# daeheepark/TrajSDE

Measured on AMD Instinct MI355X. Metric: scenes/sec (K=6, 20 SDE steps, ~256 agents) at 1/2/4/8 MI355X; minADE match, higher is better.
Workload: dtype f32 (fp16x3 split: 22-bit operands on v_mfma_f32_16x16x32_f16, f32 accumulate)

## Files before the change

trajsde_amd/csrc/aggregator_bwd.hip:

```cpp
#include <string>
#include <unordered_map>

#include "attn_common.hpp"
#include "bwd.hpp"
#include "common.hpp"
#include "dropout.hpp"
#include "kernels.hpp"
#include "layouts.hpp"
#include "tile.hpp"

namespace tsde {

static bool rows_bwd_mm();

template <int HEADS, bool NODE>
__global__ __launch_bounds__(256) void k_gattn_bwd(const float* __restrict__ img, const int32_t* __restrict__ segptr,
                                                   const int32_t* __restrict__ src, const float* __restrict__ rel,
                                                   const float* __restrict__ q, const float* __restrict__ kn,
                                                   const float* __restrict__ vn, const float* __restrict__ agg,
                                                   const float* __restrict__ dagg, const float* __restrict__ stats, int64_t N,
                                                   float* __restrict__ DQ, float* __restrict__ DKN, float* __restrict__ DVN,
                                                   float* __restrict__ RL, float* __restrict__ SS, float* __restrict__ DAGGM,
                                                   float* __restrict__ EA, float* __restrict__ ED, float* __restrict__ UZ,
                                                   const int32_t* __restrict__ asym, DropArg drop) {
// ... 776 lines not shown
      else TS_LAUNCH_TAG("k_edge_attn_rows_bwd<8>", false, (k_edge_rows_bwd_mm<false, true>), gridf, 64 * RMMF_WAVES, rows_mmf_lds_bytes(), st, img, segptr, emb, q, agg, dagg, stats, R, DQ, RL, SS, DAGGM, EA, ED, drop, wpart, wcs);
      rq->jobs.push_back(ReduceJob{wk, nullptr, base, gridf, 1, 64, 0, 0});
      rq->jobs.push_back(ReduceJob{wv, bv, base + gridf, gridf, 1, 64, 0, 0});
      *weights_done = true;
      return TRAJSDE_OK;
    }
    const int grid = int(std::min<int64_t>(256, cdiv(R, RMM_WAVES)));
    if (drop.p > 0.f) TS_LAUNCH_TAG("k_edge_attn_rows_bwd<8>", false, (k_edge_rows_bwd_mm<true, false>), grid, 64 * RMM_WAVES, rows_mm_lds_bytes(), st, img, segptr, emb, q, agg, dagg, stats, R, DQ, RL, SS, DAGGM, EA, ED, drop, nw, nw);
    else TS_LAUNCH_TAG("k_edge_attn_rows_bwd<8>", false, (k_edge_rows_bwd_mm<false, false>), grid, 64 * RMM_WAVES, rows_mm_lds_bytes(), st, img, segptr, emb, q, agg, dagg, stats, R, DQ, RL, SS, DAGGM, EA, ED, drop, nw, nw);
  } else
    TS_LAUNCH_TAG("k_edge_attn_rows_bwd<8>", false, (k_gattn_bwd<8, false>), xcd_grid(cdiv(R, 4)), 256, 0, st, img, segptr, ns, emb, q, nf, nf, agg, dagg, stats,
                  R, DQ, nw, nw, RL, SS, DAGGM, EA, ED, nw, ns, drop);
  return TRAJSDE_OK;
}

__global__ void k_reverse_edges(const int32_t* __restrict__ segptr, const int32_t* __restrict__ src, const int32_t* __restrict__ dst,
                                int64_t E, int32_t* __restrict__ REV, int32_t* __restrict__ asym) {
  const int64_t e = int64_t(blockIdx.x) * blockDim.x + threadIdx.x;
  if (e >= E) return;
  const int i = src[e], jn = dst[e];
  const int r0 = segptr[i], r1 = segptr[i + 1];
  int lo = r0, hi = r1;
  while (lo < hi) {
    const int mid = (lo + hi) >> 1;
    if (src[mid] < jn) lo = mid + 1;
    else hi = mid;
  }
  int found = lo < r1 && src[lo] == jn ? lo : -1;
  if (found < 0)
    for (int r = r0; r < r1; ++r)
      if (src[r] == jn) { found = r; break; }
  REV[e] = found;
  if (found < 0) atomicOr(asym, 1);
}

template <int HEADS>
__global__ __launch_bounds__(256) void k_gattn_src_bwd(const int32_t* __restrict__ segptr, const int32_t* __restrict__ src,
                                                       const int32_t* __restrict__ REV, const float* __restrict__ EA,
                                                       const float* __restrict__ ED, const float* __restrict__ q,
                                                       const float* __restrict__ dagg, int64_t N, float* __restrict__ DKN,
                                                       float* __restrict__ DVN, const int32_t* __restrict__ asym) {
  const int lane = threadIdx.x & 63, h = lane / (64 / HEADS);
  const int64_t node = xcd_block() * 4 + __builtin_amdgcn_readfirstlane(threadIdx.x >> 6);
  if (node >= N || *asym != 0) return;
  float dk = 0.f, dv = 0.f;
  const int beg = segptr[node], end = segptr[node + 1];
  auto idx_at = [&](int e0, int& rv, int& sv) {
    const int ec = e0 + (lane & 15) < end ? e0 + (lane & 15) : end - 1;
    rv = REV[ec];
    sv = src[ec];
  };
  int rv_n = 0, sv_n = 0;
  if (beg < end) idx_at(beg, rv_n, sv_n);
  for (int e0 = beg; e0 < end; e0 += 16) {
    const int rv = rv_n, sv = sv_n;
    idx_at(e0 + 16 < end ? e0 + 16 : e0, rv_n, sv_n);
    float a[16], d[16], qv[16], gv[16];
#pragma unroll
    for (int u = 0; u < 16; ++u) {
      const int e = __builtin_amdgcn_readlane(rv, u), i = __builtin_amdgcn_readlane(sv, u);
      a[u] = (EA + int64_t(e) * HEADS)[h];
      d[u] = (ED + int64_t(e) * HEADS)[h];
      qv[u] = (q + int64_t(i) * 64)[lane];
      gv[u] = (dagg + int64_t(i) * 64)[lane];
    }
#pragma unroll
    for (int u = 0; u < 16; ++u)
      if (e0 + u < end) {
        dk = fmaf(d[u], qv[u], dk);
        dv = fmaf(a[u], gv[u], dv);
      }
  }
  DKN[node * 64 + lane] = dk;
  DVN[node * 64 + lane] = dv;
}

struct AggBwdWs {
  float *rel, *xn[8], *q[8], *kn[8], *vn[8], *agg[8], *x1[8], *xn2[8], *out[8];
  float* stats[8];
  float *dcur, *dnext, *dagg, *dxn, *DQ, *DKN, *DVN, *DREL, *RL, *SS, *DAGGM, *XF, *part, *cs, *varena;
  float *EA[8], *ED[8], *UZ[8];
  int32_t *REV, *asym;
  NodeBlockScratch nb;
  EdgeEmbedScratch ee;
  int64_t total, parts;
  bool ok;
  AggBwdWs(int64_t N, int64_t E, int nl, int K, void* ws, int64_t bytes) {
    Carver c(ws, bytes);
    rel = c.take<float>(E * 64 + 64);
    for (int l = 0; l < nl; ++l) {
      xn[l] = c.take<float>(N * 64); q[l] = c.take<float>(N * 64); kn[l] = c.take<float>(N * 64); vn[l] = c.take<float>(N * 64);
      agg[l] = c.take<float>(N * 64); x1[l] = c.take<float>(N * 64); xn2[l] = c.take<float>(N * 64); out[l] = c.take<float>(N * 64);
      stats[l] = c.take<float>(N * 16);
    }
    float** singles[] = {&dcur, &dnext, &dagg, &dxn, &DQ, &DKN, &DVN, &DAGGM, &XF, &nb.dx1, &nb.UPD, &nb.DGP, &nb.DS};
    for (float** p : singles) *p = c.take<float>(N * 64);
    nb.H = c.take<float>(N * 256);
    nb.DH = c.take<float>(N * 256);
    RL = c.take<float>(N * 512);
    SS = c.take<float>(N * 512);
    DREL = c.take<float>(E * 64 + 64);
    for (int l = 0; l < nl; ++l) {
      EA[l] = c.take<float>(E * 8 + 64);
      ED[l] = c.take<float>(E * 8 + 64);
      UZ[l] = c.take<float>(N * 1024);
    }
    REV = c.take<int32_t>(E + 1);
    asym = c.take<int32_t>(4);
    float** edge[] = {&ee.DEP, &ee.DSP};
    for (float** p : edge) *p = c.take<float>(E * 64 + 64);
    ee.S = rel;
    nb.vpart = ee.vpart = c.take<float>(VPART_FLOATS);
    varena = c.take<float>(VPART_ARENA_SLABS * VPART_FLOATS);
    const int64_t rows = E > N ? E : N;
    parts = wgrad_max_parts(rows, 1);
    part = c.take<float>(parts * 4096);
    cs = c.take<float>(parts * 64);
    (void)K;
    total = c.off + 256;
    ok = c.ok;
  }
};

}

using namespace tsde;

template <typename DropOf>
static int aggregator_tape(const trajsde_batch* b, const trajsde_graph* g, const float* blob_fwd, int nl, int num_heads,
                           const float* local_embed, AggBwdWs& w, DropOf drop_of, hipStream_t st) {
  const int64_t N = b->N, E = g->E_g, ntiles = (N + 15) / 16, etiles = (E + 15) / 16;
#if TSDE_SPLIT_H3
  if (E > 0 && rel_embed_fused())
    TS_LAUNCH_TAG("k_edge_embed<true>", false, k_edge_embed2, tile_grid((E + 31) / 32, 1024, edge_embed2_lds(1024)), 1024, edge_embed2_lds(1024), st,
                  blob_fwd + AggBlob::REL6G, g->g_geom, EdgeCount{E, nullptr, 0}, w.rel, 0);
  else
#endif
  if (E > 0)
    TS_LAUNCH(k_edge_embed<true>, tile_grid(etiles, 1024, EdgeL6::EMB_SIZE * 4), 1024, EdgeL6::EMB_SIZE * 4, st, blob_fwd + AggBlob::REL6,
              g->g_geom, EdgeCount{E, nullptr, 0}, w.rel, 0);
  const float* x = local_embed;
  for (int l = 0; l < nl; ++l) {
    const float* lb = blob_fwd + AggBlob::layer(l);
    TS_LAUNCH(k_node_proj<3>, tile_grid(ntiles, 512, NodeProjL<3>::SIZE * 4), 512, NodeProjL<3>::SIZE * 4, st, lb + AggLayerL::QKV, x, N,
              w.xn[l], w.q[l], w.kn[l], w.vn[l]);
    {
      const DropArg dl = drop_of(l);
      TS_REQUIRE(N < (1 << 23), "aggregator_forward_train: node rows are addressed with 32-bit byte offsets (N < 2^23)");
      if (num_heads == 8 && gattn_f32mm_enabled() && g->E_g > 0) {
        if (int rc = launch_global_attn_mf(lb + AggLayerL::ATTN, g->g_segptr, g->g_src, w.rel, w.q[l], w.kn[l], w.vn[l], N, w.agg[l], w.stats[l], dl, st)) return rc;
      } else
        TS_GLOBAL_ATTN(num_heads, false, dl, xcd_grid(cdiv(N, 4)), 256, 0, st, lb + AggLayerL::ATTN, g->g_segptr, g->g_src, w.rel, w.q[l], w.kn[l], w.vn[l], N, w.agg[l], w.stats[l]);
    }
    TS_LAUNCH(k_node_update<true>, tile_grid(ntiles, 512, UpdL6::SIZE * 4), 512, UpdL6::SIZE * 4, st, lb + AggLayerL::UPD6, w.agg[l], w.xn[l], x,
              N, w.x1[l], w.xn2[l], drop_of(l), no_merge());
    TS_LAUNCH(k_ffn6, tile_grid(ntiles, 512, FfnL6::HALF * 4), 512, FfnL6::HALF * 4, st, lb + AggLayerL::FFN6, w.x1[l], w.xn2[l], N, w.out[l],
              drop_of(l));
    x = w.out[l];
  }

  return TRAJSDE_OK;
}

extern "C" {

int64_t trajsde_aggregator_backward_ws_bytes(const trajsde_batch* b, const trajsde_graph* g, int num_layers, int num_modes) {
  if (!b || !g || num_layers < 0 || num_layers > 8) return -1;
  AggBwdWs w(b->N, g->E_g, num_layers, num_modes, nullptr, 0);
  return w.total;
}

int trajsde_aggregator_backward(const trajsde_batch* b, const trajsde_graph* g, const float* blob_fwd, const float* blob_bwd,
                                int num_layers, int num_modes, const float* local_embed, const float* d_global, void* ws,
                                int64_t ws_bytes, float* const* grads, int n_grads, float* d_local, void* stream_) {
  return trajsde_aggregator_backward_heads(b, g, blob_fwd, blob_bwd, num_layers, num_modes, 8, local_embed, d_global, ws, ws_bytes, grads,
                                           n_grads, d_local, nullptr, 0, stream_);
}

int trajsde_aggregator_forward_train(const trajsde_batch* b, const trajsde_graph* g, const float* blob_fwd, int num_layers, int num_modes,
                                     int num_heads, const float* local_embed, void* ws, int64_t ws_bytes, float* global_embed,
                                     const trajsde_dropout* dropout, void* stream_) {
  if (int rc = refuse_retired_switches()) return rc;
  TS_REQUIRE(b && g && blob_fwd && local_embed && ws && global_embed, "aggregator_forward_train: null pointer");
  TS_REQUIRE(num_heads == 8 || num_heads == 4, "aggregator_forward_train: num_heads must be 8 or 4");
  TS_REQUIRE(g->g_src && g->g_segptr, "aggregator_forward_train: graph not compacted (call trajsde_graph_compact)");
  TS_REQUIRE(g->exact, "aggregator_forward_train: needs exact list lengths (trajsde_graph_prepare, not _async)");
  TS_REQUIRE(num_layers >= 1 && num_layers <= 8 && num_modes > 0, "aggregator_forward_train: bad layer/mode count");
  TS_REQUIRE(!dropout || (dropout->p >= 0.f && dropout->p < 1.f), "aggregator_forward_train: dropout p must be in [0, 1)");
  TS_REQUIRE(!state_bf16(), "aggregator_forward_train: the training tape is fp32; switch trajsde_state_storage(0)");
  auto drop_of = [&](int layer) { return dropout ? make_drop(dropout->p, dropout->seed, 2 + layer) : no_drop(); };
  AggBwdWs w(b->N, g->E_g, num_layers, num_modes, ws, ws_bytes);
  if (!w.ok) return fail(TRAJSDE_ERR_WORKSPACE, "aggregator_forward_train: workspace too small (trajsde_aggregator_backward_ws_bytes)");
  hipStream_t st = static_cast<hipStream_t>(stream_);
  if (int rc = aggregator_tape(b, g, blob_fwd, num_layers, num_heads, local_embed, w, drop_of, st)) return rc;
  const int64_t N = b->N, ntiles = (N + 15) / 16;
  const int lds = (128 + MAT64 + 64) * 4;
  dim3 grid(tile_grid(ntiles, 512, lds), num_modes);
  TS_LAUNCH(k_mode_proj, grid, 512, lds, st, blob_fwd + AggBlob::norm(num_layers), blob_fwd + AggBlob::proj(num_layers, 0), w.out[num_layers - 1], N,
            global_embed);
  return TRAJSDE_OK;
}

int trajsde_aggregator_backward_heads(const trajsde_batch* b, const trajsde_graph* g, const float* blob_fwd, const float* blob_bwd,
                                      int num_layers, int num_modes, int num_heads, const float* local_embed, const float* d_global,
                                      void* ws, int64_t ws_bytes, float* const* grads, int n_grads, float* d_local,
                                      const trajsde_dropout* dropout, int tape_valid, void* stream_) {
  if (int rc = refuse_retired_switches()) return rc;
  TS_REQUIRE(b && g && blob_fwd && blob_bwd && local_embed && d_global && ws && grads && d_local, "aggregator_backward: null pointer");
  TS_REQUIRE(!state_bf16(), "aggregator_backward: the backward pass keeps its tape in fp32; switch trajsde_state_storage(0) for training");
  TS_REQUIRE(!dropout || (dropout->p >= 0.f && dropout->p < 1.f), "aggregator_backward: dropout p must be in [0, 1)");
  auto drop_of = [&](int layer) { return dropout ? make_drop(dropout->p, dropout->seed, 2 + layer) : no_drop(); };
  TS_REQUIRE(num_heads == 8 || num_heads == 4, "aggregator_backward: num_heads must be 8 or 4");
  TS_REQUIRE(g->g_src && g->g_segptr, "aggregator_backward: graph not compacted (call trajsde_graph_compact)");
  TS_REQUIRE(g->exact, "aggregator_backward: needs exact list lengths (trajsde_graph_prepare, not _async)");
  TS_REQUIRE(num_layers >= 1 && num_layers <= 8 && num_modes > 0, "aggregator_backward: bad layer/mode count");
  const std::vector<std::string> names = stage_param_names(TRAJSDE_STAGE_AGGREGATOR_BWD, num_layers, num_modes);
  TS_REQUIRE(n_grads == int(names.size()), "aggregator_backward: gradient count does not match trajsde_param_count(AGGREGATOR_BWD)");
  std::unordered_map<std::string, float*> slot;
  for (int i = 0; i < n_grads; ++i) {
    TS_REQUIRE(grads[i] != nullptr, "aggregator_backward: null gradient buffer " + names[i]);
    slot[names[i]] = grads[i];
  }
  bool missing = false;
  auto G = [&](const std::string& n) -> float* {
    auto it = slot.find(n);
    if (it == slot.end()) { missing = true; return nullptr; }
    return it->second;
  };
  AggBwdWs w(b->N, g->E_g, num_layers, num_modes, ws, ws_bytes);
  if (!w.ok) return fail(TRAJSDE_ERR_WORKSPACE, "aggregator_backward: workspace too small");
  hipStream_t st = static_cast<hipStream_t>(stream_);
  const int64_t N = b->N, E = g->E_g, ntiles = (N + 15) / 16, etiles = (E + 15) / 16;
  const int nl = num_layers, K = num_modes;
  const WgradCtx wc{st, w.part, w.cs, nullptr, w.parts};
  DeferredSums sums(st, w.part, w.cs, w.parts, nullptr, w.varena, VPART_ARENA_SLABS * VPART_FLOATS);

  if (!tape_valid)
    if (int rc = aggregator_tape(b, g, blob_fwd, nl, num_heads, local_embed, w, drop_of, st)) return rc;
  (void)etiles;

  if (K > 0)
    TS_LAUNCH(k_lin_t_sum, unsigned(ntiles > 0 ? (ntiles + 3) / 4 : 1), 256, 2 * MAT64 * 4, st, blob_bwd + AggBwdBlob::proj(nl, 0),
              int64_t(AggBwdBlob::proj(nl, 1) - AggBwdBlob::proj(nl, 0)), d_global, N * 64, K, N, w.dxn);
  {
    const int gp = vec_grid(ntiles, 256, ProjBwdL<0>::SIZE * 4);
    float* const vp = vpart_slab(w.nb.vpart, int64_t(gp) * 4, 128);
    TS_LAUNCH(k_node_proj_bwd<0>, gp, 256, ProjBwdL<0>::SIZE * 4, st, blob_bwd + AggBwdBlob::norm(nl), w.out[nl - 1], nullptr, w.dxn,
              nullptr, nullptr, nullptr, N, w.dcur, w.XF, vp);
    {
      ColsumBatch cb(st, gp * 4, 128);
      cb.add(vp, 64, G("norm.weight"));
      cb.add(vp + 64, 64, G("norm.bias"));
      if (int rc = cb.flush()) return rc;
    }
    float* pw = G("multihead_proj.weight");
    float* pb = G("multihead_proj.bias");
    TS_REQUIRE(!missing, "aggregator_backward: parameter table lacks norm / multihead_proj");
    WgradBatch wb(wc, N, N);
    for (int k = 0; k < K; ++k)
      if (int rc = wb.add(d_global + int64_t(k) * N * 64, 64, w.XF, 64, pw + int64_t(k) * MAT64, 64, 0, pb + 64 * k, 0)) return rc;
    if (int rc = wb.flush()) return rc;
  }

  TS_HIP(hipMemsetAsync(w.asym, 0, sizeof(int32_t), st));
  if (E > 0) TS_LAUNCH(k_reverse_edges, cdiv(E, 256), 256, 0, st, g->g_segptr, g->g_src, g->g_dst, E, w.REV, w.asym);
  float* dcur = w.dcur;
  float* dnext = w.dnext;
  for (int l = nl - 1; l >= 0; --l) {
    const std::string p = "global_interactor_layers." + std::to_string(l);
    const float* lb = blob_bwd + AggBwdBlob::layer(l);
    const float* x_in = l == 0 ? local_embed : w.out[l - 1];
    NodeBlockGrads gr{G(p + ".lin_ih.weight"), G(p + ".lin_ih.bias"), G(p + ".lin_hh.weight"), G(p + ".lin_hh.bias"),
                      G(p + ".lin_self.weight"), G(p + ".lin_self.bias"), G(p + ".out_proj.weight"), G(p + ".out_proj.bias"),
                      G(p + ".norm2.weight"), G(p + ".norm2.bias"), G(p + ".mlp.0.weight"), G(p + ".mlp.0.bias"),
                      G(p + ".mlp.3.weight"), G(p + ".mlp.3.bias")};
    float* wke = G(p + ".lin_k_edge.weight");
    float* bke = G(p + ".lin_k_edge.bias");
    float* wve = G(p + ".lin_v_edge.weight");
    float* bve = G(p + ".lin_v_edge.bias");
    float* n1g = G(p + ".norm1.weight");
    float* n1b = G(p + ".norm1.bias");
    float* qkv_w[3] = {G(p + ".lin_q_node.weight"), G(p + ".lin_k_node.weight"), G(p + ".lin_v_node.weight")};
    float* qkv_b[3] = {G(p + ".lin_q_node.bias"), G(p + ".lin_k_node.bias"), G(p + ".lin_v_node.bias")};
    TS_REQUIRE(!missing, "aggregator_backward: parameter table lacks an entry of " + p);
    const NodeBlockTape tp{w.agg[l], w.xn[l], w.x1[l], w.xn2[l]};
    WgradBatch wb(wc, N, N);
    if (int rc = node_block_backward(lb + AggLayerBwdL::NODE, tp, dcur, N, w.nb, wc, gr, w.dagg, w.dxn, st, drop_of(l), &wb)) return rc;
    if (w.DVN >= w.DKN + N * 64 && w.DVN - w.DKN < N * 64 + 1024) {
      TS_HIP(hipMemsetAsync(w.DKN, 0, size_t(w.DVN - w.DKN + N * 64) * sizeof(float), st));
    } else {
      TS_HIP(hipMemsetAsync(w.DKN, 0, size_t(N) * 64 * sizeof(float), st));
      TS_HIP(hipMemsetAsync(w.DVN, 0, size_t(N) * 64 * sizeof(float), st));
    }
    if (num_heads == 4) {
      TS_LAUNCH((k_gattn_bwd<4, true>), xcd_grid(cdiv(N, 4)), 256, 0, st, lb + AggLayerBwdL::ATTN, g->g_segptr, g->g_src, w.rel, w.q[l], w.kn[l], w.vn[l],
                w.agg[l], w.dagg, w.stats[l], N, w.DQ, w.DKN, w.DVN, w.RL, w.SS, w.DAGGM, w.EA[l], w.ED[l], w.UZ[l], w.asym, drop_of(l));
      TS_LAUNCH(k_gattn_src_bwd<4>, xcd_grid(cdiv(N, 4)), 256, 0, st, g->g_segptr, g->g_src, w.REV, w.EA[l], w.ED[l], w.q[l], w.dagg, N, w.DKN, w.DVN,
                w.asym);
    } else {
      if (rows_bwd_mm()) {
        const int grid_mm = xcd_grid(std::min<int64_t>(256, cdiv(N, GBM_WAVES)));
        const DropArg dl = drop_of(l);
        if (dl.p > 0.f)
          TS_LAUNCH_TAG("(k_gattn_bwd<8, true>)", false, (k_gattn_bwd_mm<true>), grid_mm, 64 * GBM_WAVES, gattn_bwd_mm_lds_bytes(), st, lb + AggLayerBwdL::ATTN, g->g_segptr, g->g_src, w.rel, w.q[l], w.kn[l],
                        w.vn[l], w.agg[l], w.dagg, w.stats[l], N, w.DQ, w.DKN, w.DVN, w.RL, w.SS, w.DAGGM, w.EA[l], w.ED[l], w.UZ[l], w.asym, dl);
        else
          TS_LAUNCH_TAG("(k_gattn_bwd<8, true>)", false, (k_gattn_bwd_mm<false>), grid_mm, 64 * GBM_WAVES, gattn_bwd_mm_lds_bytes(), st, lb + AggLayerBwdL::ATTN, g->g_segptr, g->g_src, w.rel, w.q[l], w.kn[l],
// ... 55 lines not shown
```

trajsde_amd/csrc/attn.hip:

```cpp
#include "common.hpp"
#include "kernels.hpp"
#include "layouts.hpp"
#include "attn_common.hpp"
#include "dropout.hpp"
#include "range.hpp"
#include "tile.hpp"

#include <type_traits>

#ifndef TSDE_SKEW_SLEEPS
#define TSDE_SKEW_SLEEPS 2
#endif

namespace tsde {


__global__ __launch_bounds__(512) void k_aa_center(const float* __restrict__ img_g, const float* __restrict__ x,
                                                   const float* __restrict__ x_fake, const float* __restrict__ rot,
                                                   const uint8_t* __restrict__ bos, const int32_t* __restrict__ orig,
                                                   int N, int Nt, int H, float* __restrict__ center,
                                                   float* __restrict__ cn, float* __restrict__ q) {
  extern __shared__ __attribute__((aligned(16))) float lds[];
  stage_blob(lds, img_g, AaCenterL::SIZE);
  using A = AaCenterL;
  const Lane L;
  const int waves = blockDim.x >> 6, wave = threadIdx.x >> 6;
  const int64_t rows = int64_t(H) * Nt, ntiles = (rows + 15) / 16;
  for (int64_t tile = int64_t(blockIdx.x) * waves + wave; tile < ntiles; tile += int64_t(gridDim.x) * waves) {
    keep_lds_reads_here();
    const int64_t row = tile * 16 + L.n, r = row < rows ? row : rows - 1;
    const int t = int(r / Nt), i = int(r - int64_t(t) * Nt), o = orig[i];
    const float* xp = i < N ? x + (int64_t(i) * H + t) * 2 : x_fake + (int64_t(i - N) * H + t) * 2;
    const f4 R = *reinterpret_cast<const f4*>(rot + 4 * o);
    const float x0 = xp[0], x1 = xp[1];
    const float r0 = x0 * R[0] + x1 * R[2], r1 = x0 * R[1] + x1 * R[3];
    f4 a[4], b[4];
    linear_in2(a, r0, r1, lds + A::W0, lds + A::B0, L.g);
    layer_norm<4>(a, lds + A::G1, lds + A::E1, L.g);
    relu<4>(a);
    linear<4, 4>(b, a, lds + A::W3, lds + A::B3, L);
    layer_norm<4>(b, lds + A::G4, lds + A::E4, L.g);
    relu<4>(b);
    linear<4, 4>(a, b, lds + A::W6, lds + A::B6, L);
    layer_norm<4>(a, lds + A::G7, lds + A::E7, L.g);
    if (bos[int64_t(o) * H + t]) load_vec<4>(a, lds + A::BOS + t * 64, L.g);
    if (row < rows) store_row(a, center, row, L.g);
    layer_norm<4>(a, lds + A::N1G, lds + A::N1B, L.g);
    if (row < rows) store_row(a, cn, row, L.g);
    linear<4, 4>(b, a, lds + A::WQ, lds + A::BQ, L);
    if (row < rows) store_row(b, q, row, L.g);
  }
}

template <bool X6>
__global__ __launch_bounds__(1024) void k_edge_kv(const float* __restrict__ img_g, const float* __restrict__ geom,
                                                 const int32_t* __restrict__ dst, const float* __restrict__ q, int64_t E,
                                                 float* __restrict__ logits, float* __restrict__ v, int heads) {
  extern __shared__ __attribute__((aligned(16))) float lds[];
  using EL = typename std::conditional<X6, EdgeL6, EdgeL>::type;
  stage_blob(lds, img_g, EL::SIZE);
  const Lane L;
  const int waves = blockDim.x >> 6, wave = threadIdx.x >> 6;
  const int64_t ntiles = (E + 15) / 16;
  if ((wave >> 2) & 1) {
    for (int i = 0; i < TSDE_SKEW_SLEEPS; ++i) __builtin_amdgcn_s_sleep(32);
  }
  for (int64_t tile = int64_t(blockIdx.x) * waves + wave; tile < ntiles; tile += int64_t(gridDim.x) * waves) {
    keep_lds_reads_here();
    const int64_t e = tile * 16 + L.n, ec = e < E ? e : E - 1;
    const f4 ge = *reinterpret_cast<const f4*>(geom + 4 * ec);
    const int d = dst[ec];
    f4 emb[4], kv[8], qv[4];
    load_row(qv, q, d, L.g);
    edge_embed<X6>(emb, ge, lds, L);
    if constexpr (X6) linear_x6<8, 4>(kv, emb, lds + EL::WKV, lds + EL::BKV, L);
    else linear<8, 4>(kv, emb, lds + EL::WKV, lds + EL::BKV, L);
    f4 k[4] = {kv[0], kv[1], kv[2], kv[3]};
    f4 vv[4] = {kv[4], kv[5], kv[6], kv[7]};
    store_logits(qv, k, logits, e, e < E, L, heads);
    if (e < E) store_row(vv, v, e, L.g);
  }
}

template <int THREADS>
__global__ __launch_bounds__(THREADS) void k_edge_kv2(const float* __restrict__ img_g, const float* __restrict__ geom,
                                                      const int32_t* __restrict__ dst, const float* __restrict__ q, int64_t E,
                                                      float* __restrict__ logits, float* __restrict__ v, int heads) {
  extern __shared__ __attribute__((aligned(16))) float lds[];
  using EL = EdgeL6;
  stage_blob(lds, img_g, EL::SIZE);
  const Lane L;
  const int waves = blockDim.x >> 6, wave = threadIdx.x >> 6;
  const int64_t npairs = (E + 31) / 32;
  if ((wave >> 2) & 1) {
    for (int i = 0; i < 2 * TSDE_SKEW_SLEEPS; ++i) __builtin_amdgcn_s_sleep(32);
  }
  for (int64_t pair = int64_t(blockIdx.x) * waves + wave; pair < npairs; pair += int64_t(gridDim.x) * waves) {
    keep_lds_reads_here();
    const int64_t e0 = pair * 32 + L.n, e1 = e0 + 16;
    const int64_t c0 = e0 < E ? e0 : E - 1, c1 = e1 < E ? e1 : E - 1;
    const f4 g0 = *reinterpret_cast<const f4*>(geom + 4 * c0);
    const f4 g1 = *reinterpret_cast<const f4*>(geom + 4 * c1);
    const int d0 = dst[c0], d1 = dst[c1];
    f4 emb0[4], emb1[4], kv0[8], kv1[8], qv[4];
    edge_embed2_x6(emb0, emb1, g0, g1, lds, L);
    load_vec<8>(kv0, lds + EL::BKV, L.g);
    load_vec<8>(kv1, lds + EL::BKV, L.g);
    linear_acc_x6_2<8, 4>(kv0, kv1, emb0, emb1, lds + EL::WKV, L.lane);
    {
      load_row(qv, q, d0, L.g);
      f4 k[4] = {kv0[0], kv0[1], kv0[2], kv0[3]};
      f4 vv[4] = {kv0[4], kv0[5], kv0[6], kv0[7]};
      store_logits(qv, k, logits, e0, e0 < E, L, heads);
      if (e0 < E) store_row(vv, v, e0, L.g);
    }
    {
      load_row(qv, q, d1, L.g);
      f4 k[4] = {kv1[0], kv1[1], kv1[2], kv1[3]};
      f4 vv[4] = {kv1[4], kv1[5], kv1[6], kv1[7]};
      store_logits(qv, k, logits, e1, e1 < E, L, heads);
      if (e1 < E) store_row(vv, v, e1, L.g);
    }
  }
}
template __global__ void k_edge_kv2<512>(const float*, const float*, const int32_t*, const float*, int64_t, float*, float*, int);
template __global__ void k_edge_kv2<768>(const float*, const float*, const int32_t*, const float*, int64_t, float*, float*, int);

#if TSDE_SPLIT_H3
#ifdef TSDE_EDGE_STAMPS
__device__ unsigned long long g_edge_stamps[16];
__device__ unsigned long long g_edge_wg[4 * 512];
struct PhaseStamps {
  unsigned long long last, real0, acc[12];
  __device__ __forceinline__ void start() {
#pragma unroll
    for (int i = 0; i < 12; ++i) acc[i] = 0;
    last = __builtin_amdgcn_s_memtime();
    real0 = __builtin_amdgcn_s_memrealtime();
  }
#ifdef TSDE_EDGE_STAMPS_LIGHT
  __device__ __forceinline__ void mark(int) {}
  __device__ __forceinline__ void finish() { acc[0] = __builtin_amdgcn_s_memtime() - last; }
#else
  __device__ __forceinline__ void mark(int i) {
    const unsigned long long t = __builtin_amdgcn_s_memtime();
    acc[i] += t - last;
    last = t;
  }
  __device__ __forceinline__ void finish() {}
#endif
};
#endif
struct SegState {
  f4 acc[4], m, s;
};
__device__ __forceinline__ void seg_reset(SegState& S) {
#pragma unroll
  for (int jt = 0; jt < 4; ++jt) S.acc[jt] = f4{0.f, 0.f, 0.f, 0.f};
  S.m = f4{-INFINITY, -INFINITY, -INFINITY, -INFINITY};
  S.s = f4{0.f, 0.f, 0.f, 0.f};
}
constexpr float LOG2E_F = 1.4426950408889634f, LN2_F = 0.6931471805599453f;
__device__ __forceinline__ float logit_scale(int heads) {
  return (heads == 4 ? 0.25f : INV_SQRT_DH) * (TSDE_R6_SOFTMAX ? LOG2E_F : 1.0f);
}
__device__ __forceinline__ float head_logit1(const f4& qv, const f4& k, int heads) {
  float p = qv[0] * k[0];
#pragma unroll
  for (int c = 1; c < 4; ++c) p = fmaf(qv[c], k[c], p);
  p = xor16_sum(p);
  if (heads == 4) p = xor32_sum(p);
  return p * logit_scale(heads);
}
__device__ __forceinline__ f4 head_logits(const f4 (&qv)[4], const f4 (&k)[4], int heads) {
  f4 lg;
#pragma unroll
  for (int jt = 0; jt < 4; ++jt) lg[jt] = head_logit1(qv[jt], k[jt], heads);
  return lg;
}
#if TSDE_R6_SOFTMAX
__device__ __forceinline__ float max_plain(float a, float b) {
  float r;
  asm("v_max_f32 %0, %1, %2" : "=v"(r) : "v"(a), "v"(b));
  return r;
}
__device__ __forceinline__ void seg_front1(SegState& S, int jt, float lg, float keep, float& sc, float& exk) {
  const float mn = max_plain(S.m[jt], lg);
  sc = __builtin_amdgcn_exp2f(S.m[jt] - mn);
  const float ex = __builtin_amdgcn_exp2f(lg - mn);
  S.m[jt] = mn;
  S.s[jt] = fmaf(S.s[jt], sc, ex);
  exk = ex * keep;
}
__device__ __forceinline__ void seg_scale1(SegState& S, int jt, float sc) {
#pragma unroll
  for (int c = 0; c < 4; ++c) S.acc[jt][c] *= sc;
}
__device__ __forceinline__ void seg_add1(SegState& S, int jt, float exk, const f4& v) {
#pragma unroll
  for (int c = 0; c < 4; ++c) S.acc[jt][c] = fmaf(exk, v[c], S.acc[jt][c]);
}
// ... 603 lines not shown
  agg[node * 64 + lane] = end > beg ? acc / (s + 1e-16f) : 0.f;
}

template <int HEADS, bool ST_BF16, bool DROP, bool NODE>
__global__ __launch_bounds__(256, 4) void k_global_attn(const float* __restrict__ img, const int32_t* __restrict__ segptr,
                                                     const int32_t* __restrict__ src, const float* __restrict__ rel,
                                                     const float* __restrict__ q, const float* __restrict__ kn,
                                                     const float* __restrict__ vn, int64_t N, float* __restrict__ agg,
                                                     float* __restrict__ stats, DropArg drop) {
  constexpr int LPH = 64 / HEADS;
  constexpr int SL = 64 / LPH;
  constexpr int NV = SL / 4;
  constexpr float INV = HEADS == 4 ? 0.25f : INV_SQRT_DH;
  __shared__ __attribute__((aligned(16))) float sbuf[4][HEADS][64 + 4];
  __shared__ __attribute__((aligned(16))) float srel[4][8][64];
  const int lane = threadIdx.x & 63, wv = __builtin_amdgcn_readfirstlane(threadIdx.x >> 6);
  const int h = lane / LPH, j = lane % LPH;
  const int64_t node = xcd_block() * 4 + wv;
  const int64_t nc = node < N ? node : N - 1;
  const float* wke = img + GAttnL::WKE;
  const float* wve = img + GAttnL::WVE;
  const float ql = q[nc * 64 + lane] * INV;
  const float cb = NODE ? 0.f : head_sum_n<HEADS>(ql * img[GAttnL::BKE + lane]);
  float U[SL];
#pragma unroll
  for (int e = 0; e < SL; ++e) U[e] = 0.f;
#pragma unroll
  for (int d = 0; d < LPH; ++d) {
    const float qd = __shfl(ql, LPH * h + d);
#pragma unroll
    for (int v4 = 0; v4 < NV; ++v4) {
      const f4 w = *reinterpret_cast<const f4*>(wke + (LPH * h + d) * 64 + SL * j + 4 * v4);
#pragma unroll
      for (int e = 0; e < 4; ++e) U[4 * v4 + e] = fmaf(w[e], qd, U[4 * v4 + e]);
    }
  }
  const int beg = segptr[nc], end = node < N ? segptr[nc + 1] : beg;
  const __amdgpu_buffer_rsrc_t rs_rel = row_rsrc(rel + (ST_BF16 ? 0 : int64_t(beg) * 64));
  const __amdgpu_buffer_rsrc_t rs_kn = row_rsrc(kn), rs_vn = row_rsrc(vn);
  float m = -INFINITY, s = 0.f, sk = 0.f, accv = 0.f, accr[SL];
#pragma unroll
  for (int e = 0; e < SL; ++e) accr[e] = 0.f;
  constexpr bool dropping = DROP;
  for (int e0 = beg; e0 < end; e0 += 8) {
    f4 r[8][NV];
    float knv[8], vnv[8], lg[8], kp[8];
    if (dropping) drop_attn_chunk<8>(kp, drop, uint32_t(nc), uint32_t(e0 - beg), lane, h);
    const int sv = NODE ? src[e0 + (lane & 7) < end ? e0 + (lane & 7) : end - 1] : 0;
    float rl[8];
    f4 ra, rb;
#pragma unroll
    for (int u = 0; u < 8; ++u) {
      const int e = e0 + u < end ? e0 + u : end - 1;
      const int sidx = __builtin_amdgcn_readlane(sv, u);
      if (!ST_BF16) rl[u] = row_load(rs_rel, lane, e - beg);
      knv[u] = NODE ? row_load(rs_kn, lane, sidx) : 0.f;
      vnv[u] = NODE ? row_load(rs_vn, lane, sidx) : 0.f;
    }
    if (ST_BF16) {
      const int64_t er = e0 + (lane >> 3) < end ? e0 + (lane >> 3) : end - 1;
      const bf4* p = reinterpret_cast<const bf4*>(reinterpret_cast<const __bf16*>(rel) + er * 64 + 8 * (lane & 7));
      ra = widen4(p[0]);
      rb = widen4(p[1]);
    }
    __builtin_amdgcn_wave_barrier();
    if (ST_BF16) {
      *reinterpret_cast<f4*>(&srel[wv][lane >> 3][8 * (lane & 7)]) = ra;
      *reinterpret_cast<f4*>(&srel[wv][lane >> 3][8 * (lane & 7) + 4]) = rb;
    } else {
#pragma unroll
      for (int u = 0; u < 8; ++u) srel[wv][u][lane] = rl[u];
    }
    __builtin_amdgcn_fence(__ATOMIC_RELEASE, "wavefront");
    __builtin_amdgcn_wave_barrier();
#pragma unroll
    for (int u = 0; u < 8; ++u)
#pragma unroll
      for (int v4 = 0; v4 < NV; ++v4) r[u][v4] = *reinterpret_cast<const f4*>(&srel[wv][u][SL * j + 4 * v4]);
    float cm = -INFINITY;
#pragma unroll
    for (int u = 0; u < 8; ++u) {
      float p = ql * knv[u];
#pragma unroll
      for (int v4 = 0; v4 < NV; ++v4)
#pragma unroll
        for (int e = 0; e < 4; ++e) p = fmaf(r[u][v4][e], U[4 * v4 + e], p);
      p = head_sum_n<HEADS>(p);
      if (!NODE) p += cb;
      lg[u] = e0 + u < end ? p : -INFINITY;
      cm = fmaxf(cm, lg[u]);
    }
    const float mn = fmaxf(m, cm);
    const float sc = fast_exp(m - mn);
    m = mn;
    s *= sc;
    sk *= sc;
    accv *= sc;
#pragma unroll
    for (int e = 0; e < SL; ++e) accr[e] *= sc;
#pragma unroll
    for (int u = 0; u < 8; ++u) {
      float ex = fast_exp(lg[u] - m);
      s += ex;
      if (dropping) ex *= kp[u];
      sk += ex;
      accv = fmaf(ex, vnv[u], accv);
#pragma unroll
      for (int v4 = 0; v4 < NV; ++v4)
#pragma unroll
        for (int e = 0; e < 4; ++e) accr[4 * v4 + e] = fmaf(ex, r[u][v4][e], accr[4 * v4 + e]);
    }
  }
  const float inv = 1.0f / (s + 1e-16f);
#pragma unroll
  for (int v4 = 0; v4 < NV; ++v4)
    *reinterpret_cast<f4*>(&sbuf[wv][h][SL * j + 4 * v4]) =
        f4{accr[4 * v4] * inv, accr[4 * v4 + 1] * inv, accr[4 * v4 + 2] * inv, accr[4 * v4 + 3] * inv};
  float out = fmaf(img[GAttnL::BVE + lane], sk * inv, accv * inv);
#pragma unroll
  for (int k4 = 0; k4 < 16; ++k4) {
    const f4 wr = *reinterpret_cast<const f4*>(wve + lane * 64 + 4 * k4);
    const f4 sv = *reinterpret_cast<const f4*>(&sbuf[wv][h][4 * k4]);
#pragma unroll
    for (int e = 0; e < 4; ++e) out = fmaf(wr[e], sv[e], out);
  }
  if (node < N) agg[node * 64 + lane] = out;
  if (stats != nullptr && node < N && j == 0) *reinterpret_cast<float2*>(stats + (node * HEADS + h) * 2) = float2{m, inv};
}
template __global__ void k_global_attn<8, false, false, true>(const float*, const int32_t*, const int32_t*, const float*, const float*, const float*,
                                                       const float*, int64_t, float*, float*, DropArg);
template __global__ void k_global_attn<8, false, true, true>(const float*, const int32_t*, const int32_t*, const float*, const float*, const float*,
                                                       const float*, int64_t, float*, float*, DropArg);
template __global__ void k_global_attn<8, true, false, true>(const float*, const int32_t*, const int32_t*, const float*, const float*, const float*,
                                                       const float*, int64_t, float*, float*, DropArg);
template __global__ void k_global_attn<8, true, true, true>(const float*, const int32_t*, const int32_t*, const float*, const float*, const float*,
                                                       const float*, int64_t, float*, float*, DropArg);
template __global__ void k_global_attn<4, false, false, true>(const float*, const int32_t*, const int32_t*, const float*, const float*, const float*,
                                                       const float*, int64_t, float*, float*, DropArg);
template __global__ void k_global_attn<4, false, true, true>(const float*, const int32_t*, const int32_t*, const float*, const float*, const float*,
                                                       const float*, int64_t, float*, float*, DropArg);
template __global__ void k_global_attn<4, true, false, true>(const float*, const int32_t*, const int32_t*, const float*, const float*, const float*,
                                                       const float*, int64_t, float*, float*, DropArg);
template __global__ void k_global_attn<4, true, true, true>(const float*, const int32_t*, const int32_t*, const float*, const float*, const float*,
                                                       const float*, int64_t, float*, float*, DropArg);
template __global__ void k_global_attn<8, false, false, false>(const float*, const int32_t*, const int32_t*, const float*, const float*, const float*,
                                                       const float*, int64_t, float*, float*, DropArg);
template __global__ void k_global_attn<8, false, true, false>(const float*, const int32_t*, const int32_t*, const float*, const float*, const float*,
                                                       const float*, int64_t, float*, float*, DropArg);
template __global__ void k_global_attn<4, false, false, false>(const float*, const int32_t*, const int32_t*, const float*, const float*, const float*,
                                                       const float*, int64_t, float*, float*, DropArg);
template __global__ void k_global_attn<4, false, true, false>(const float*, const int32_t*, const int32_t*, const float*, const float*, const float*,
                                                       const float*, int64_t, float*, float*, DropArg);

template <bool X6>
__global__ __launch_bounds__(512) void k_node_update(const float* __restrict__ img_g, const float* __restrict__ agg,
                                                     const float* __restrict__ xn, const float* __restrict__ x, int64_t R,
                                                     float* __restrict__ x1, float* __restrict__ xn2, DropArg drop, SegMerge mg) {
  extern __shared__ __attribute__((aligned(16))) float lds[];
  using U = typename std::conditional<X6, UpdL6, UpdL>::type;
  stage_blob(lds, img_g, U::SIZE);
  const Lane L_;
  auto lin = [&](f4 (&out)[4], const f4 (&in)[4], int wo, int bo) {
    if constexpr (X6) linear_x6<4, 4>(out, in, lds + wo, lds + bo, L_);
    else linear<4, 4>(out, in, lds + wo, lds + bo, L_);
  };
  const Lane L;
  const int waves = blockDim.x >> 6, wave = threadIdx.x >> 6;
  const int64_t ntiles = (R + 15) / 16;
  for (int64_t tile = int64_t(blockIdx.x) * waves + wave; tile < ntiles; tile += int64_t(gridDim.x) * waves) {
    keep_lds_reads_here();
    const int64_t row = tile * 16 + L.n, r = row < R ? row : R - 1;
    f4 a[4], n[4], g[4], s[4];
    if (mg.rec != nullptr) {
      const int C = stream_len(mg.ec, edge_count(mg.ec), mg.C_host);
      const int beg = mg.segptr[r], end = mg.segptr[r + 1];
#pragma unroll
      for (int jt = 0; jt < 4; ++jt) a[jt] = f4{0.f, 0.f, 0.f, 0.f};
      if (end > beg) {
        const StreamMap smap = stream_map(C);
        const int c0 = int(stream_of(smap, beg)), c1 = int(stream_of(smap, end - 1));
        const float* rr = mg.rec + (r + c0) * SEG_REC;
#pragma unroll
        for (int jt = 0; jt < 4; ++jt) a[jt] = *reinterpret_cast<const f4*>(rr + 16 * jt + 4 * L.g);
        f4 m = *reinterpret_cast<const f4*>(rr + 64 + 4 * L.g), sm = *reinterpret_cast<const f4*>(rr + 80 + 4 * L.g);
        for (int c = c0 + 1; c <= c1; ++c) {
          rr += SEG_REC;
          const f4 mp = *reinterpret_cast<const f4*>(rr + 64 + 4 * L.g), sp = *reinterpret_cast<const f4*>(rr + 80 + 4 * L.g);
#pragma unroll
          for (int jt = 0; jt < 4; ++jt) {
            const f4 ap = *reinterpret_cast<const f4*>(rr + 16 * jt + 4 * L.g);
            const float mn = fmaxf(m[jt], mp[jt]);
            const float wa = fast_exp(m[jt] - mn), wb = fast_exp(mp[jt] - mn);
            sm[jt] = sm[jt] * wa + sp[jt] * wb;
            a[jt] = a[jt] * wa + ap * wb;
            m[jt] = mn;
          }
        }
#pragma unroll
        for (int jt = 0; jt < 4; ++jt) {
          const f4 cv = *reinterpret_cast<const f4*>(mg.cv + 16 * jt + 4 * L.g);
#pragma unroll
          for (int c = 0; c < 4; ++c) a[jt][c] = a[jt][c] / (sm[jt] + 1e-16f) + cv[c];
        }
      }
    } else {
      load_row(a, agg, r, L.g);
    }
    load_row(n, xn, r, L.g);
    f4 xr[4];
    load_row(xr, x, r, L.g);
    range_note(absmax<4>(a), RS_NODE_AGG);
    lin(g, a, U::WIH, U::BIH);
    {
      f4 h[4];
      lin(h, n, U::WHH, U::BHH);
#pragma unroll
      for (int jt = 0; jt < 4; ++jt) g[jt] += h[jt];
    }
    sigmoid_<4>(g);
    lin(s, n, U::WSELF, U::BSELF);
#pragma unroll
    for (int jt = 0; jt < 4; ++jt)
#pragma unroll
      for (int c = 0; c < 4; ++c) a[jt][c] = a[jt][c] + g[jt][c] * (s[jt][c] - a[jt][c]);
    range_note(absmax<4>(a), RS_NODE_AGG);
    lin(s, a, U::WOUT, U::BOUT);
    if (drop.p > 0.f) {
      f4 mk[4];
      drop_feat16(mk, drop, DK_PROJ, uint32_t(r), 0, L.g);
#pragma unroll
      for (int jt = 0; jt < 4; ++jt) s[jt] *= mk[jt];
    }
#pragma unroll
    for (int jt = 0; jt < 4; ++jt) n[jt] = xr[jt] + s[jt];
    if (row < R) store_row(n, x1, row, L.g);
    layer_norm<4>(n, lds + U::N2G, lds + U::N2B, L.g);
    if (row < R) store_row(n, xn2, row, L.g);
  }
}

__global__ __launch_bounds__(512) void k_ffn(const float* __restrict__ img_g, const float* __restrict__ x1,
                                             const float* __restrict__ xn2, int64_t R, float* __restrict__ out, DropArg drop, int out_bf16) {
  extern __shared__ __attribute__((aligned(16))) float lds[];
  stage_blob(lds, img_g, FfnL::SIZE);
  const Lane L;
  const int waves = blockDim.x >> 6, wave = threadIdx.x >> 6;
  const int64_t ntiles = (R + 15) / 16;
  for (int64_t tile = int64_t(blockIdx.x) * waves + wave; tile < ntiles; tile += int64_t(gridDim.x) * waves) {
    keep_lds_reads_here();
    const int64_t row = tile * 16 + L.n, r = row < R ? row : R - 1;
    f4 n[4], hid[16], o[4], xr[4];
    load_row(n, xn2, r, L.g);
    load_row(xr, x1, r, L.g);
    linear<16, 4>(hid, n, lds + FfnL::W1, lds + FfnL::B1, L);
    relu<16>(hid);
    if (drop.p > 0.f) {
#pragma unroll
      for (int blk = 0; blk < 4; ++blk) {
        f4 mk[4];
        drop_feat16(mk, drop, DK_HIDDEN, uint32_t(r), blk, L.g);
#pragma unroll
        for (int jt = 0; jt < 4; ++jt) hid[4 * blk + jt] *= mk[jt];
      }
    }
    range_note(absmax<16>(hid), RS_FFN_HIDDEN);
    linear<4, 16>(o, hid, lds + FfnL::W2, lds + FfnL::B2, L);
    if (drop.p > 0.f) {
      f4 mk[4];
      drop_feat16(mk, drop, DK_OUT, uint32_t(r), 0, L.g);
#pragma unroll
      for (int jt = 0; jt < 4; ++jt) o[jt] *= mk[jt];
    }
#pragma unroll
    for (int jt = 0; jt < 4; ++jt) o[jt] += xr[jt];
    if (row < R) store_row_st(o, out, row, L.g, out_bf16 != 0);
  }
}

__global__ __launch_bounds__(512) void k_ffn6(const float* __restrict__ img_g, const float* __restrict__ x1,
                                              const float* __restrict__ xn2, int64_t R, float* __restrict__ out, DropArg drop) {
  extern __shared__ __attribute__((aligned(16))) float lds[];
  const Lane L;
  const int waves = blockDim.x >> 6, wave = threadIdx.x >> 6;
  const int64_t ntiles = (R + 15) / 16;
  for (int hf = 0; hf < 2; ++hf) {
    if (hf) __syncthreads();
    stage_blob(lds, img_g + hf * FfnL6::HALF, FfnL6::HALF);
    for (int64_t tile = int64_t(blockIdx.x) * waves + wave; tile < ntiles; tile += int64_t(gridDim.x) * waves) {
      keep_lds_reads_here();
      const int64_t row = tile * 16 + L.n, r = row < R ? row : R - 1;
      f4 n[4], hid[8], o[4];
      load_row(n, xn2, r, L.g);
      linear_x6<8, 4>(hid, n, lds + FfnL6::W1, lds + FfnL6::B1, L);
      relu<8>(hid);
      f4 mo[4];
      if (drop.p > 0.f) {
#pragma unroll
        for (int b2 = 0; b2 < 2; ++b2) {
          f4 mk[4];
          drop_feat16(mk, drop, DK_HIDDEN, uint32_t(r), 2 * hf + b2, L.g);
#pragma unroll
          for (int jt = 0; jt < 4; ++jt) hid[4 * b2 + jt] *= mk[jt];
        }
        drop_feat16(mo, drop, DK_OUT, uint32_t(r), 0, L.g);
      }
      range_note(absmax<8>(hid), RS_FFN_HIDDEN);
      if (hf == 0) {
        load_vec<4>(o, lds + FfnL6::B2, L.g);
        load_row(n, x1, r, L.g);
      } else {
#pragma unroll
        for (int jt = 0; jt < 4; ++jt) o[jt] = f4{0.f, 0.f, 0.f, 0.f};
        load_row(n, out, r, L.g);
      }
      linear_acc_x6<4, 8>(o, hid, lds + FfnL6::W2, L.lane);
      if (drop.p > 0.f) {
#pragma unroll
        for (int jt = 0; jt < 4; ++jt) o[jt] *= mo[jt];
      }
#pragma unroll
      for (int jt = 0; jt < 4; ++jt) o[jt] += n[jt];
      if (row < R) store_row(o, out, row, L.g);
    }
  }
}

template <int NQ, bool SPLITKV>
__global__ __launch_bounds__(512) void k_node_proj(const float* __restrict__ img_g, const float* __restrict__ x, int64_t R,
                                                   float* __restrict__ xn_out, float* __restrict__ p0, float* __restrict__ p1,
                                                   float* __restrict__ p2) {
  extern __shared__ __attribute__((aligned(16))) float lds[];
  using P = NodeProjL<NQ>;
  stage_blob(lds, img_g, P::SIZE);
  const Lane L;
  const int waves = blockDim.x >> 6, wave = threadIdx.x >> 6;
  const int64_t ntiles = (R + 15) / 16;
  for (int64_t tile = int64_t(blockIdx.x) * waves + wave; tile < ntiles; tile += int64_t(gridDim.x) * waves) {
    keep_lds_reads_here();
    const int64_t row = tile * 16 + L.n, r = row < R ? row : R - 1;
    f4 a[4], pr[4 * NQ];
    load_row(a, x, r, L.g);
    layer_norm<4>(a, lds + P::N1G, lds + P::N1B, L.g);
    if (row < R) store_row(a, xn_out, row, L.g);
    linear<4 * NQ, 4>(pr, a, lds + P::W, lds + P::B, L);
    float* outs[3] = {p0, p1, p2};
#pragma unroll
    for (int j = 0; j < NQ; ++j) {
      f4 t4[4] = {pr[4 * j], pr[4 * j + 1], pr[4 * j + 2], pr[4 * j + 3]};
#if TSDE_SPLIT_H3
      if (SPLITKV && j > 0) {
        if (row < R) {
          char* o = reinterpret_cast<char*>(outs[j] + row * 64);
#pragma unroll
          for (int jt = 0; jt < 4; ++jt) {
            unsigned h0, l0, h1, l1;
            split_pair(t4[jt][0], t4[jt][1], h0, l0);
            split_pair(t4[jt][2], t4[jt][3], h1, l1);
            *reinterpret_cast<uint2*>(o + 32 * jt + 8 * L.g) = uint2{h0, h1};
            *reinterpret_cast<uint2*>(o + 128 + 32 * jt + 8 * L.g) = uint2{l0, l1};
          }
        }
        continue;
      }
#endif
      if (row < R) store_row(t4, outs[j], row, L.g);
    }
  }
}

__global__ __launch_bounds__(512) void k_mode_proj(const float* __restrict__ norm_g, const float* __restrict__ proj_g,
                                                   const float* __restrict__ x, int64_t N, float* __restrict__ out) {
  extern __shared__ __attribute__((aligned(16))) float lds[];
  const int k = blockIdx.y;
  for (int i = threadIdx.x; i < 128; i += blockDim.x) lds[i] = norm_g[i];
  stage_blob(lds + 128, proj_g + int64_t(k) * (MAT64 + 64), MAT64 + 64);
  const Lane L;
  const int waves = blockDim.x >> 6, wave = threadIdx.x >> 6;
  const int64_t ntiles = (N + 15) / 16;
  for (int64_t tile = int64_t(blockIdx.x) * waves + wave; tile < ntiles; tile += int64_t(gridDim.x) * waves) {
    keep_lds_reads_here();
    const int64_t row = tile * 16 + L.n, r = row < N ? row : N - 1;
    f4 a[4], o[4];
    load_row(a, x, r, L.g);
    layer_norm<4>(a, lds, lds + 64, L.g);
    linear<4, 4>(o, a, lds + 128, lds + 128 + MAT64, L);
    if (row < N) store_row(o, out + int64_t(k) * N * 64, row, L.g);
  }
}

template __global__ void k_edge_kv<false>(const float*, const float*, const int32_t*, const float*, int64_t, float*, float*, int);
template __global__ void k_edge_kv<true>(const float*, const float*, const int32_t*, const float*, int64_t, float*, float*, int);
template __global__ void k_edge_embed<false>(const float*, const float*, EdgeCount, float*, int);
template __global__ void k_edge_embed<true>(const float*, const float*, EdgeCount, float*, int);
template __global__ void k_global_edge<false>(const float*, const float*, const int32_t*, const int32_t*, const float*, const float*, const float*, int64_t, float*, float*);
template __global__ void k_global_edge<true>(const float*, const float*, const int32_t*, const int32_t*, const float*, const float*, const float*, int64_t, float*, float*);
template __global__ void k_node_update<false>(const float*, const float*, const float*, const float*, int64_t, float*, float*, DropArg, SegMerge);
template __global__ void k_node_update<true>(const float*, const float*, const float*, const float*, int64_t, float*, float*, DropArg, SegMerge);
template __global__ void k_node_proj<1, false>(const float*, const float*, int64_t, float*, float*, float*, float*);
template __global__ void k_node_proj<3, false>(const float*, const float*, int64_t, float*, float*, float*, float*);
template __global__ void k_node_proj<3, true>(const float*, const float*, int64_t, float*, float*, float*, float*);

}
```

trajsde_amd/csrc/encoder_bwd.hip:

```cpp
#include <string>
#include <unordered_map>

#include "attn_common.hpp"
#include "bwd.hpp"
#include "common.hpp"
#include "encoder_bwd_host.hpp"
#include "kernels.hpp"
#include "layouts.hpp"
#include "philox.hpp"
#include "range.hpp"
#include "sde_funcs.hpp"
#include "tile.hpp"
#include "tile_bwd.hpp"

namespace tsde {

__global__ __launch_bounds__(256) void k_aa_center_bwd_tail(const float* __restrict__ img, const float* __restrict__ x,
                                                            const float* __restrict__ x_fake, const float* __restrict__ rot,
                                                            const uint8_t* __restrict__ bos, const int32_t* __restrict__ orig, int N,
                                                            int Nt, int H, const float* __restrict__ dcenter,
                                                            float* __restrict__ A1, float* __restrict__ A2, float* __restrict__ DA3P,
                                                            float* __restrict__ DA2P, float* __restrict__ XR,
                                                            float* __restrict__ vpart) {
  extern __shared__ __attribute__((aligned(16))) float lds[];
// ... 592 lines not shown
struct AttnChain {
  const float *img_node, *img_proj, *img_attn, *img_emb;
  const float *geom, *q, *emb, *stats, *x;
  const int32_t *dst, *segptr;
  NodeBlockTape tp;
  int64_t R, E;
  std::string prefix, embed;
  int heads = 8;
  DropArg drop = no_drop();
  const float* img_kvt = nullptr;
};

}

using namespace tsde;

namespace {

struct GradTable {
  std::unordered_map<std::string, float*> slot;
  bool missing = false;
  std::string missing_name;
  float* operator()(const std::string& n) {
    auto it = slot.find(n);
    if (it == slot.end()) {
      if (!missing) missing_name = n;
      missing = true;
      return nullptr;
    }
    return it->second;
  }
};

int run_attn_chain(const AttnChain& c, const float* dout, EncBwdWs& w, const WgradCtx& wc, GradTable& G, float* dx_out,
                   hipStream_t st) {
  const std::string& p = c.prefix;
  NodeBlockGrads gr{G(p + ".lin_ih.weight"), G(p + ".lin_ih.bias"), G(p + ".lin_hh.weight"), G(p + ".lin_hh.bias"),
                    G(p + ".lin_self.weight"), G(p + ".lin_self.bias"), G(p + ".out_proj.weight"), G(p + ".out_proj.bias"),
                    G(p + ".norm2.weight"), G(p + ".norm2.bias"), G(p + ".mlp.0.weight"), G(p + ".mlp.0.bias"),
                    G(p + ".mlp.3.weight"), G(p + ".mlp.3.bias")};
  const std::string e = p + "." + c.embed;
  EdgeEmbedGrads eg{G(e + ".module_list.0.0.weight"), G(e + ".module_list.0.0.bias"), G(e + ".module_list.0.1.weight"),
                    G(e + ".module_list.0.1.bias"), G(e + ".module_list.1.0.weight"), G(e + ".module_list.1.0.bias"),
                    G(e + ".module_list.1.1.weight"), G(e + ".module_list.1.1.bias"), G(e + ".module_list.0.3.weight"),
                    G(e + ".module_list.0.3.bias"), G(e + ".module_list.1.3.weight"), G(e + ".module_list.1.3.bias"),
                    G(e + ".aggr_embed.0.weight"), G(e + ".aggr_embed.0.bias"), G(e + ".aggr_embed.2.weight"),
                    G(e + ".aggr_embed.2.bias"), G(e + ".aggr_embed.3.weight"), G(e + ".aggr_embed.3.bias")};
  float *wk = G(p + ".lin_k.weight"), *bk = G(p + ".lin_k.bias"), *wv = G(p + ".lin_v.weight"), *bv = G(p + ".lin_v.bias");
  float *wq = G(p + ".lin_q.weight"), *bq = G(p + ".lin_q.bias"), *n1g = G(p + ".norm1.weight"), *n1b = G(p + ".norm1.bias");
  TS_REQUIRE(!G.missing, "encoder_backward: parameter table lacks " + G.missing_name);
  const int64_t R = c.R, E = c.E;
  if (int rc = node_block_backward(c.img_node, c.tp, dout, R, w.nb, wc, gr, w.dagg, w.dxn, st, c.drop)) return rc;
  bool weights_done = false;
  if (int rc = run_edge_attn_bwd(st, c.heads, c.img_attn, c.segptr, c.emb, c.q, c.tp.agg, w.dagg, c.stats, R, w.DQ, w.RL, w.SS, w.DAGGM,
                                 w.EA, w.ED, c.drop, &wc, wk, wv, bv, &weights_done))
    return rc;
  if (!weights_done) {
    if (int rc = run_headwise_outer(wc, c.q, w.RL, R, wk, c.heads)) return rc;
    if (int rc = run_headwise_outer(wc, w.dagg, w.SS, R, wv, c.heads)) return rc;
  }
  TS_HIP(hipMemsetAsync(bk, 0, 64 * sizeof(float), st));
  if (!weights_done)
    if (int rc = run_colsum_tall(st, w.DAGGM, R, 64, 64, bv, w.nb.vpart)) return rc;
  if (E > 0) {
    const EdgeAttnGrad ag{c.dst, c.q, w.dagg, w.EA, w.ED, c.img_kvt, c.heads};
    EdgeEmbedScratch ee = w.ee;
    ee.S = const_cast<float*>(c.emb);
    if (int rc = edge_embed_backward(c.img_emb, c.geom, nullptr, E, ee, wc, eg, st, &ag)) return rc;
  }
  const int gp = vec_grid((R + 15) / 16, 256, ProjBwdL<1>::SIZE * 4);
  float* const vp = vpart_slab(w.nb.vpart, int64_t(gp) * 4, 128);
  TS_LAUNCH(k_node_proj_bwd<1>, gp, 256, ProjBwdL<1>::SIZE * 4, st, c.img_proj, c.x, w.nb.dx1, w.dxn, w.DQ, nullptr, nullptr, R, dx_out,
            nullptr, vp);
  {
    ColsumBatch cb(st, gp * 4, 128);
    cb.add(vp, 64, n1g);
    cb.add(vp + 64, 64, n1b);
    if (int rc = cb.flush()) return rc;
  }
  return run_wgrad(wc, w.DQ, 64, c.tp.xn, 64, R, R, wq, 64, 0, bq, 0);
}

int aa_encoder_backward(const trajsde_batch* b, const trajsde_graph* g, const float* rot, const float* blob_fwd, const float* blob_bwd, EncBwdWs& w,
                        const WgradCtx& wc, GradTable& G, int heads, hipStream_t st, const DropArg& drop = no_drop()) {
  using BB = EncBwdBlob;
  const int N = b->N, Nt = g->Nt, H = b->H;
  const int64_t R = int64_t(H) * Nt, Eaa = g->E_aa;
  AttnChain c{blob_bwd + BB::AA_NODE, blob_bwd + BB::AA_PROJ, blob_fwd + EncBlob::AA_ATTN, blob_bwd + BB::AA_EDGEEMB,
              g->aa_geom, w.q, w.emb, w.stats, w.center, g->aa_dst, g->aa_segptr, NodeBlockTape{w.agg, w.cn, w.x1, w.xn2}, R, Eaa,
              "aa_encoder", "nbr_embed", heads};
  c.drop = drop;
  c.img_kvt = blob_bwd + BB::AA_EDGEKV + EdgeKvBwdL::WKT;
  if (int rc = run_attn_chain(c, w.DAA, w, wc, G, w.DCENTER, st)) return rc;
  const std::string ce = "aa_encoder.center_embed.embed.";
  float *w0 = G(ce + "0.weight"), *b0 = G(ce + "0.bias"), *g1 = G(ce + "1.weight"), *e1 = G(ce + "1.bias");
  float *w3 = G(ce + "3.weight"), *b3 = G(ce + "3.bias"), *g4 = G(ce + "4.weight"), *e4 = G(ce + "4.bias");
  float *w6 = G(ce + "6.weight"), *b6 = G(ce + "6.bias"), *g7 = G(ce + "7.weight"), *e7 = G(ce + "7.bias");
  float* tok = G("aa_encoder.bos_token");
  TS_REQUIRE(!G.missing, "encoder_backward: parameter table lacks " + G.missing_name);
  const int gt = vec_grid((R + 15) / 16, 256, CenterTailL::SIZE * 4);
  float* vp = vpart_slab(w.nb.vpart, int64_t(gt) * 4, 256);
  TS_LAUNCH(k_aa_center_bwd_tail, gt, 256, CenterTailL::SIZE * 4, st, blob_bwd + BB::AA_CTAIL, b->x, g->x_fake, rot, b->bos_mask, g->orig, N,
            Nt, H, w.DCENTER, w.A1, w.A2, w.DA3P, w.DA2P, w.XR, vp);
  float* const tv[4] = {g7, e7, g4, e4};
  {
    ColsumBatch cb(st, gt * 4, 256);
    for (int i = 0; i < 4; ++i) cb.add(vp + 64 * i, 64, tv[i]);
    if (int rc = cb.flush()) return rc;
  }
  if (int rc = run_wgrad(wc, w.DA3P, 64, w.A2, 64, R, R, w6, 64, 0, b6, 0)) return rc;
  if (int rc = run_wgrad(wc, w.DA2P, 64, w.A1, 64, R, R, w3, 64, 0, b3, 0)) return rc;
  const int lds_br = (EdgeL::WA3 + MAT64) * 4;
  const int gb = vec_grid((R + 15) / 16, 256, lds_br);
  vp = vpart_slab(w.nb.vpart, int64_t(gb) * 4, 320);
  TS_LAUNCH(k_edge_embed_bwd_branch<0>, gb, 256, lds_br, st, blob_bwd + BB::AA_CHEAD, w.XR, w.DA2P, R, vp);
  {
    ColsumBatch cb(st, gb * 4, 320);
    cb.add(vp, 64, g1);
    cb.add(vp + 64, 64, e1);
    cb.add(vp + 128, 64, w0, 2);
    cb.add(vp + 192, 64, w0 + 1, 2);
    cb.add(vp + 256, 64, b0);
    if (int rc = cb.flush()) return rc;
  }
  TS_LAUNCH(k_bos_grad, dim3(H, BOS_SLICES), 1024, 0, st, w.DCENTER, b->bos_mask, g->orig, Nt, H, w.nb.vpart);
  return run_colsum(st, w.nb.vpart, BOS_SLICES, H * 64, H * 64, tok);
}

}

static int edge_attention_tape(const char* tag, const float* img_fused, const float* img_edge6, const float* img_attn, const float* geom, const int32_t* dst, int64_t E,
                               const int32_t* segptr, const float* q, int64_t R, float* emb, float* stats, float* agg, float* rec, int heads,
                               const DropArg& drop, hipStream_t st) {
  if (attn_fused_enabled())
    return fused_edge_attention(tag, false, img_fused, geom, dst, q, EdgeCount{E, nullptr, 0}, segptr, R, rec, agg, heads, st, drop, emb, stats);
  if (E > 0)
    TS_LAUNCH(k_edge_embed<true>, tile_grid((E + 15) / 16, 1024, EdgeL6::EMB_SIZE * 4), 1024, EdgeL6::EMB_SIZE * 4, st, img_edge6, geom,
              EdgeCount{E, nullptr, 0}, emb, 0);
  TS_EDGE_ATTN(heads, drop, xcd_grid(cdiv(R, 4)), 256, 0, st, img_attn, segptr, emb, q, R, agg, stats);
  return TRAJSDE_OK;
}

static int encoder_tape(const trajsde_batch* b, const trajsde_graph* g, const float* rot, const float* blob_fwd, const float* step_tab,
                        const NoiseArg& na, EncBwdWs& w, const DropArg& drop_aa, const DropArg& drop_al, hipStream_t st) {
  const int N = b->N, Nt = g->Nt, H = b->H;
  const int64_t R = int64_t(H) * Nt, Eaa = g->E_aa, Ela = g->E_la;
  const int64_t rtiles = (int64_t(Nt) + 15) / 16;
  using FB = EncBlob;
  TS_LAUNCH(k_aa_center, tile_grid((R + 15) / 16, 512, AaCenterL::SIZE * 4), 512, AaCenterL::SIZE * 4, st, blob_fwd + FB::AA_CENTER, b->x,
            g->x_fake, rot, b->bos_mask, g->orig, N, Nt, H, w.center, w.cn, w.q);
  if (int rc = edge_attention_tape("k_edge_kv[aa]+emb", blob_fwd + FB::AA_EDGE6F, blob_fwd + FB::AA_EDGE6, blob_fwd + FB::AA_ATTN, g->aa_geom, g->aa_dst, Eaa, g->aa_segptr, w.q, R,
                                   w.emb, w.stats, w.agg, w.rec, 8, drop_aa, st))
    return rc;
  TS_LAUNCH(k_node_update<true>, tile_grid((R + 15) / 16, 512, UpdL6::SIZE * 4), 512, UpdL6::SIZE * 4, st, blob_fwd + FB::AA_UPD6, w.agg, w.cn,
            w.center, R, w.x1, w.xn2, drop_aa, no_merge());
  TS_LAUNCH(k_ffn6, tile_grid((R + 15) / 16, 512, FfnL6::HALF * 4), 512, FfnL6::HALF * 4, st, blob_fwd + FB::AA_FFN6, w.x1, w.xn2, R, w.aa_out, drop_aa);
  {
    RecurTab tab;
    for (int idx = 0; idx < H; ++idx) {
      const float* e = step_tab + 8 * idx;
      tab.v[idx][0] = e[1]; tab.v[idx][1] = e[2]; tab.v[idx][2] = e[3]; tab.v[idx][3] = e[4];
    }
    static const bool legacy = []() { const char* e = getenv("TRAJSDE_RECUR_LEGACY"); return e && atoi(e) != 0; }();
    static const int force_tw = []() { const char* e = getenv("TRAJSDE_RECUR_TW"); return e ? atoi(e) : 0; }();
    const int tiles_per_wg = force_tw > 0 ? force_tw : int((rtiles + 255) / 256);
    if (TSDE_SPLIT_H3 && !legacy && tiles_per_wg <= COOP_TMAX && H <= 32) {
      StepTab stab;
      for (int i = 0; i < H; ++i) {
        stab.dt[i] = step_tab[8 * i + 1]; stab.sq[i] = step_tab[8 * i + 2]; stab.sn[i] = step_tab[8 * i + 3]; stab.cs[i] = step_tab[8 * i + 4];
      }
      const RecurTape tp{w.HIN, w.H1, w.H2, w.G1, w.G2, w.GS, w.HODE, w.XS, w.U1, w.R1, w.UU, w.RR, w.RH, w.N1, w.NW};
      const int grid = int((rtiles + tiles_per_wg - 1) / tiles_per_wg);
      const int lds = coop_lds_floats(tiles_per_wg) * 4;
#define TS_COOP_SAVE(TW) TS_LAUNCH_TAG("k_enc_recur_coop<save>", false, (k_enc_recur_coop<TW, true>), grid, 256, lds, st, blob_fwd + FB::SDE, blob_fwd + FB::GRU, \
              blob_fwd + FB::COOP6, blob_fwd + FB::HIDDEN, w.aa_out, Nt, N, H, b->TT, tiles_per_wg, stab, 0, na, g->nus_mask, b->padding_mask, g->orig, g->eos_idx,     \
              g->pick_slot, w.lat, nullptr, nullptr, 0, tp)
      switch (tiles_per_wg) {
        case 1: TS_COOP_SAVE(1); break;
        case 2: TS_COOP_SAVE(2); break;
        case 3: TS_COOP_SAVE(3); break;
        default: TS_COOP_SAVE(4); break;
      }
#undef TS_COOP_SAVE
    } else {
      const RecurSaveArgs ra{blob_fwd + FB::SDE, blob_fwd + FB::GRU, blob_fwd + FB::HIDDEN, w.aa_out, Nt, H, b->TT, na, g->nus_mask, b->padding_mask,
                             g->orig, w.HIN, w.H1, w.H2, w.G1, w.G2, w.GS, w.HODE, w.XS, w.U1, w.R1, w.UU, w.RR, w.RH, w.N1, w.NW, w.hcur};
      const int lds_r = (EncSdeL::SIZE > EncGruL::SIZE ? EncSdeL::SIZE : EncGruL::SIZE) * 4;
      TS_LAUNCH(k_enc_recur_save, tile_grid(rtiles, 256, lds_r), 256, lds_r, st, ra, tab);
    }
  }
  k_gather_latent<<<cdiv(int64_t(N) * 64, 256), 256, 0, st>>>(w.HODE, w.UU, w.NW, g->eos_idx, b->padding_mask, g->orig, N, Nt, H, b->TT, w.lat);
  TS_LAUNCH_CHECK("k_gather_latent");
  TS_LAUNCH(k_node_proj<1>, tile_grid((int64_t(N) + 15) / 16, 512, NodeProjL<1>::SIZE * 4), 512, NodeProjL<1>::SIZE * 4, st,
            blob_fwd + FB::AL_Q, w.lat, int64_t(N), w.al_xn, w.al_q, nullptr, nullptr);
  if (int rc = edge_attention_tape("k_edge_kv[al]+emb", blob_fwd + FB::AL_EDGE6F, blob_fwd + FB::AL_EDGE6, blob_fwd + FB::AL_ATTN, g->la_geom, g->la_dst, Ela, g->la_segptr, w.al_q,
                                   int64_t(N), w.al_emb, w.al_stats, w.al_agg, w.rec, 8, drop_al, st))
    return rc;
  TS_LAUNCH(k_node_update<true>, tile_grid((int64_t(N) + 15) / 16, 512, UpdL6::SIZE * 4), 512, UpdL6::SIZE * 4, st, blob_fwd + FB::AL_UPD6,
            w.al_agg, w.al_xn, w.lat, int64_t(N), w.al_x1, w.al_xn2, drop_al, no_merge());

  return TRAJSDE_OK;
}

__global__ void k_pick_diff(const float* __restrict__ GS, const int32_t* __restrict__ eos, const int32_t* __restrict__ pick_slot, int Nt,
                            float* __restrict__ diff_pick) {
  const int r = blockIdx.x, lane = threadIdx.x;
  const int slot = pick_slot[r];
  if (slot >= 0) diff_pick[int64_t(slot) * 64 + lane] = GS[int64_t(eos[r]) * Nt + r];
}

extern "C" {

int64_t trajsde_encoder_backward_ws_bytes(const trajsde_batch* b, const trajsde_graph* g) {
  if (!b || !g) return -1;
  EncBwdWs w(b, g, nullptr, 0);
  return w.total;
}
int64_t trajsde_encoder_tape_bytes(const trajsde_batch* b, const trajsde_graph* g) {
  if (!b || !g) return -1;
  EncBwdWs w(b, g, nullptr, 0);
  return w.tape_total;
}
int64_t trajsde_encoder_backward_scratch_bytes(const trajsde_batch* b, const trajsde_graph* g) {
  if (!b || !g) return -1;
  EncBwdWs w(b, g, nullptr, 0);
  return w.scratch_total;
}

int trajsde_encoder_forward_train(const trajsde_batch* b, const trajsde_graph* g, const float* rot, const float* blob_fwd,
                                  const float* step_tab , const trajsde_noise* noise, void* ws, int64_t ws_bytes,
                                  float* local_embed, float* diff_pick, const trajsde_dropout* dropout, void* stream_) {
  if (int rc = refuse_retired_switches()) return rc;
  TS_REQUIRE(b && g && rot && blob_fwd && step_tab && ws && local_embed && diff_pick, "encoder_forward_train: null pointer");
  TS_REQUIRE(g->aa_dst && g->la_dst && g->orig, "encoder_forward_train: graph not compacted (call trajsde_graph_compact)");
  TS_REQUIRE(g->exact, "encoder_forward_train: needs exact list lengths (trajsde_graph_prepare, not _async)");
  TS_REQUIRE(b->A > 0 && g->Nt == b->N + b->A, "encoder_forward_train: graph was prepared without the fake-agent rows");
  TS_REQUIRE(!dropout || (dropout->p >= 0.f && dropout->p < 1.f), "encoder_forward_train: dropout p must be in [0, 1)");
  TS_REQUIRE(!state_bf16(), "encoder_forward_train: the training tape is fp32; switch trajsde_state_storage(0)");
  const DropArg drop_aa = dropout ? make_drop(dropout->p, dropout->seed, 0) : no_drop();
  const DropArg drop_al = dropout ? make_drop(dropout->p, dropout->seed, 1) : no_drop();
  EncBwdWs w(b, g, ws, int64_t(1) << 60);
  if (ws_bytes < w.tape_total) return fail(TRAJSDE_ERR_WORKSPACE, "encoder_forward_train: workspace too small (trajsde_encoder_tape_bytes)");
  hipStream_t st = static_cast<hipStream_t>(stream_);
  NoiseArg na{0, nullptr, nullptr};
  if (noise) { na.seed = noise->seed; na.z = noise->z; na.row_ids = noise->row_ids; na.seed_dev = noise->seed_dev; }
  if (int rc = encoder_tape(b, g, rot, blob_fwd, step_tab, na, w, drop_aa, drop_al, st)) return rc;
  const int N = b->N;
  TS_LAUNCH(k_ffn6, tile_grid((int64_t(N) + 15) / 16, 512, FfnL6::HALF * 4), 512, FfnL6::HALF * 4, st, blob_fwd + EncBlob::AL_FFN6, w.al_x1, w.al_xn2,
            int64_t(N), local_embed, drop_al);
  TS_HIP(hipMemsetAsync(diff_pick, 0, size_t(2) * b->A * 64 * sizeof(float), st));
  k_pick_diff<<<g->Nt, 64, 0, st>>>(w.GS, g->eos_idx, g->pick_slot, g->Nt, diff_pick);
  TS_LAUNCH_CHECK("k_pick_diff");
  return TRAJSDE_OK;
}

}

int tsde::encoder_backward_run(const char* who_, const trajsde_batch* b, const trajsde_graph* g, const float* rot, const float* blob_fwd,
                               const float* blob_bwd, const float* step_tab , const float* step_tab_dev,
                               const trajsde_noise* noise, const float* d_local, void* ws, int64_t ws_bytes, float* const* grads, int n_grads,
                               float* d_latent, float* d_aa_out, const trajsde_dropout* dropout, int tape_valid, void* scratch,
                               int64_t scratch_bytes, void* stream_, const DldgProducer& dldg) {
  const std::string who = who_;
  TS_REQUIRE(!dropout || (dropout->p >= 0.f && dropout->p < 1.f), who + ": dropout p must be in [0, 1)");
  TS_REQUIRE(!state_bf16(), who + ": the backward pass keeps its tape in fp32; switch trajsde_state_storage(0) for training");
  const DropArg drop_aa = dropout ? make_drop(dropout->p, dropout->seed, 0) : no_drop();
  const DropArg drop_al = dropout ? make_drop(dropout->p, dropout->seed, 1) : no_drop();
  TS_REQUIRE(g->aa_dst && g->la_dst && g->orig, who + ": graph not compacted (call trajsde_graph_compact)");
  TS_REQUIRE(g->exact, who + ": needs exact list lengths (trajsde_graph_prepare, not _async)");
  TS_REQUIRE(b->A > 0 && g->Nt == b->N + b->A, who + ": graph was prepared without the fake-agent rows");
  const std::vector<std::string> names = stage_param_names(TRAJSDE_STAGE_ENCODER_BWD, 0, 0);
  TS_REQUIRE(n_grads == int(names.size()), who + ": gradient count does not match trajsde_param_count(ENCODER_BWD)");
  GradTable G;
  for (int i = 0; i < n_grads; ++i) {
    TS_REQUIRE(grads[i] != nullptr, who + ": null gradient buffer " + names[i]);
    G.slot[names[i]] = grads[i];
  }
  EncBwdWs w(b, g, ws, ws_bytes, scratch, scratch_bytes);
  if (!w.ok) return fail(TRAJSDE_ERR_WORKSPACE, who + ": workspace too small");
  hipStream_t st = static_cast<hipStream_t>(stream_);
  const int N = b->N, Nt = g->Nt, H = b->H;
  const int64_t R = int64_t(H) * Nt, Ela = g->E_la;
  const int64_t rtiles = (int64_t(Nt) + 15) / 16;
  NoiseArg na{0, nullptr, nullptr};
  if (noise) { na.seed = noise->seed; na.z = noise->z; na.row_ids = noise->row_ids; na.seed_dev = noise->seed_dev; }
  const WgradCtx wc{st, w.part, w.cs, step_tab_dev, w.parts};
  DeferredSums sums(st, w.part, w.cs, w.parts, step_tab_dev, w.varena, VPART_ARENA_SLABS * VPART_FLOATS);
  using BB = EncBwdBlob;

  if (!tape_valid)
    if (int rc = encoder_tape(b, g, rot, blob_fwd, step_tab, na, w, drop_aa, drop_al, st)) return rc;

  {
    AttnChain c{blob_bwd + BB::AL_NODE, blob_bwd + BB::AL_PROJ, blob_fwd + EncBlob::AL_ATTN, blob_bwd + BB::AL_EDGEEMB,
                g->la_geom, w.al_q, w.al_emb, w.al_stats, w.lat, g->la_dst, g->la_segptr,
                NodeBlockTape{w.al_agg, w.al_xn, w.al_x1, w.al_xn2}, int64_t(N), Ela, "al_encoder", "lane_embed"};
    c.drop = drop_al;
    c.img_kvt = blob_bwd + BB::AL_EDGEKV + EdgeKvBwdL::WKT;
    if (int rc = run_attn_chain(c, d_local, w, wc, G, w.DLAT, st)) return rc;
    if (d_latent) TS_HIP(hipMemcpyAsync(d_latent, w.DLAT, size_t(N) * 64 * sizeof(float), hipMemcpyDeviceToDevice, st));
  }
  if (int rc = dldg(w.GS, w.DLDG, w.scal, st)) return rc;
  {
    RecurTab tab;
    for (int idx = 0; idx < H; ++idx) {
      const float* e = step_tab + 8 * idx;
      tab.v[idx][0] = e[1]; tab.v[idx][1] = e[2]; tab.v[idx][2] = e[3]; tab.v[idx][3] = e[4];
    }
    const RecurBwdArgs rb{blob_bwd + BB::GRU, blob_bwd + BB::SDE, Nt, N, H, b->TT, na, b->padding_mask, g->nus_mask, g->orig, g->eos_idx,
                          w.DLAT, w.DLDG, w.HODE, w.U1, w.R1, w.UU, w.RR, w.N1, w.NW, w.H1, w.H2, w.G1, w.G2, w.GS,
                          w.DNW, w.DN1P, w.DUP, w.DRP, w.DU1, w.DR1, w.DHO, w.DAA, w.DF, w.DH2, w.DH1, w.DG2N, w.DG1N, w.DG2A, w.DG1A,
                          w.DGPN, w.DGPA, w.dhA};
    const int lds_r = (GruBwdL::SIZE > EncSdeBwdL::SIZE ? GruBwdL::SIZE : EncSdeBwdL::SIZE) * 4;
    static const bool legacy_bwd = []() { const char* e = getenv("TRAJSDE_RECUR_LEGACY"); return e && atoi(e) != 0; }();
    static const int force_tw = []() { const char* e = getenv("TRAJSDE_RECUR_BWD_TW"); return e ? atoi(e) : 0; }();
    const int64_t rounds1 = (rtiles + 255) / 256, rounds2 = (rtiles + 511) / 512;
    const int tiles_per_wg = force_tw > 0 ? force_tw : (rounds2 * 185 < rounds1 * 100 ? 2 : 1);
    if (TSDE_SPLIT_H3 && !legacy_bwd && tiles_per_wg <= COOP_TMAX && H <= 32) {
      RecurBwdCoopArgs ca{};
      ca.gru_t = blob_bwd + BB::GRU; ca.sde_t = blob_bwd + BB::SDE;
      ca.Nt = Nt; ca.N = N; ca.H = H; ca.TT = b->TT; ca.na = na;
      ca.pad = b->padding_mask; ca.nus = g->nus_mask; ca.orig = g->orig; ca.eos = g->eos_idx;
      ca.dlat = w.DLAT; ca.DLDG = w.DLDG;
      ca.tp = RecurTape{w.HIN, w.H1, w.H2, w.G1, w.G2, w.GS, w.HODE, w.XS, w.U1, w.R1, w.UU, w.RR, w.RH, w.N1, w.NW};
      ca.DNW = w.DNW; ca.DN1P = w.DN1P; ca.DUP = w.DUP; ca.DRP = w.DRP; ca.DU1 = w.DU1; ca.DR1 = w.DR1; ca.DAA = w.DAA;
      ca.DF = w.DF; ca.DH2 = w.DH2; ca.DH1 = w.DH1; ca.DG2N = w.DG2N; ca.DG1N = w.DG1N; ca.DG2A = w.DG2A; ca.DG1A = w.DG1A;
      ca.DGPN = w.DGPN; ca.DGPA = w.DGPA; ca.dh_out = w.dhA;
      for (int i = 0; i < H; ++i) { ca.dt[i] = step_tab[8 * i + 1]; ca.sq[i] = step_tab[8 * i + 2]; }
      const int grid = int((rtiles + tiles_per_wg - 1) / tiles_per_wg);
      const int lds = coop_bwd_lds_floats(tiles_per_wg) * 4;
      switch (tiles_per_wg) {
        case 1: TS_LAUNCH(k_enc_recur_bwd_coop<1>, grid, 256, lds, st, ca); break;
        case 2: TS_LAUNCH(k_enc_recur_bwd_coop<2>, grid, 256, lds, st, ca); break;
        case 3: TS_LAUNCH(k_enc_recur_bwd_coop<3>, grid, 256, lds, st, ca); break;
        default: TS_LAUNCH(k_enc_recur_bwd_coop<4>, grid, 256, lds, st, ca); break;
      }
    } else {
      TS_LAUNCH(k_enc_recur_bwd, tile_grid(rtiles, 256, lds_r), 256, lds_r, st, rb, tab);
    }
    const float* dh = w.dhA;
    if (int rc = run_colsum_tall(st, dh, Nt, 64, 64, G("hidden"), w.nb.vpart)) return rc;
    const std::string lf = "lsde_func.", gu = "gru_unit.";
    struct WG { const float* d; const float* a; const char* w; const char* bias; int ldw, col0, tc; };
    const WG jobs[] = {
        {w.DH1, w.HIN, "lsde_func.f_func.net.0.weight", "lsde_func.f_func.net.0.bias", 66, 0, 1},
        {w.DH2, w.H1, "lsde_func.f_func.net.2.weight", "lsde_func.f_func.net.2.bias", 64, 0, 0},
        {w.DF, w.H2, "lsde_func.f_func.net.4.weight", "lsde_func.f_func.net.4.bias", 64, 0, 0},
        {w.DG1N, w.HIN, "lsde_func.g_nus.net.0.weight", "lsde_func.g_nus.net.0.bias", 66, 0, 1},
        {w.DG2N, w.G1, "lsde_func.g_nus.net.2.weight", "lsde_func.g_nus.net.2.bias", 64, 0, 0},
        {w.DG1A, w.HIN, "lsde_func.g_argo.net.0.weight", "lsde_func.g_argo.net.0.bias", 66, 0, 1},
        {w.DG2A, w.G1, "lsde_func.g_argo.net.2.weight", "lsde_func.g_argo.net.2.bias", 64, 0, 0},
        {w.DNW, w.N1, "gru_unit.new_state_net.2.weight", "gru_unit.new_state_net.2.bias", 64, 0, 0},
        {w.DN1P, w.XS, "gru_unit.new_state_net.0.weight", "gru_unit.new_state_net.0.bias", 128, 0, 0},
        {w.DN1P, w.RH, "gru_unit.new_state_net.0.weight", nullptr, 128, 64, 0},
        {w.DUP, w.U1, "gru_unit.update_gate.2.weight", "gru_unit.update_gate.2.bias", 64, 0, 0},
        {w.DRP, w.R1, "gru_unit.reset_gate.2.weight", "gru_unit.reset_gate.2.bias", 64, 0, 0},
        {w.DU1, w.HODE, "gru_unit.update_gate.0.weight", "gru_unit.update_gate.0.bias", 128, 0, 0},
        {w.DU1, w.XS, "gru_unit.update_gate.0.weight", nullptr, 128, 64, 0},
        {w.DR1, w.HODE, "gru_unit.reset_gate.0.weight", "gru_unit.reset_gate.0.bias", 128, 0, 0},
        {w.DR1, w.XS, "gru_unit.reset_gate.0.weight", nullptr, 128, 64, 0},
    };
    WgradBatch wb(wc, R, Nt);
    for (const WG& j : jobs) {
      float* W = G(j.w);
      float* bias = j.bias ? G(j.bias) : nullptr;
      TS_REQUIRE(!G.missing, "encoder_backward: parameter table lacks " + G.missing_name);
      if (int rc = wb.add(j.d, 64, j.a, 64, W, j.ldw, j.col0, bias, j.tc)) return rc;
    }
    if (int rc = wb.flush()) return rc;
    float *n4w = G("lsde_func.g_nus.net.4.weight"), *n4b = G("lsde_func.g_nus.net.4.bias");
    float *a4w = G("lsde_func.g_argo.net.4.weight"), *a4b = G("lsde_func.g_argo.net.4.bias");
    TS_REQUIRE(!G.missing, "encoder_backward: parameter table lacks " + G.missing_name);
    for (int net = 0; net < 2; ++net) {
      const int blocks = R >= 65536 ? 128 : 8;
      float* const vp = vpart_slab(w.nb.vpart, blocks, 128);
      TS_LAUNCH(k_rowscale_colsum, blocks, 1024, 0, st, w.G2, net == 0 ? w.DGPN : w.DGPA, R, vp);
      {
        ColsumBatch cb(st, blocks, 128);
        cb.add(vp, 64, net == 0 ? n4w : a4w);
        cb.add(vp + 64, 1, net == 0 ? n4b : a4b);
        if (int rc = cb.flush()) return rc;
      }
    }
  }
  if (d_aa_out) TS_HIP(hipMemcpyAsync(d_aa_out, w.DAA, size_t(R) * 64 * sizeof(float), hipMemcpyDeviceToDevice, st));
  if (int rc = aa_encoder_backward(b, g, rot, blob_fwd, blob_bwd, w, wc, G, 8, st, drop_aa)) return rc;
  return sums.finish();
}

extern "C" {

int trajsde_encoder_backward(const trajsde_batch* b, const trajsde_graph* g, const float* rot, const float* blob_fwd,
                             const float* blob_bwd, const float* step_tab , const float* step_tab_dev,
                             const trajsde_noise* noise, const float* d_local, float diff_weight, void* ws, int64_t ws_bytes,
                             float* diff_loss, float* const* grads, int n_grads, float* d_latent, float* d_aa_out,
                             const trajsde_dropout* dropout, int tape_valid, void* scratch, int64_t scratch_bytes, void* stream_) {
  if (int rc = refuse_retired_switches()) return rc;
  TS_REQUIRE(b && g && rot && blob_fwd && blob_bwd && step_tab && step_tab_dev && d_local && ws && diff_loss && grads,
             "encoder_backward: null pointer");
  const DldgProducer bce = [&](const float* GS, float* DLDG, float* scal, hipStream_t st) -> int {
    TS_LAUNCH(k_diffbce, 1, 1024, 0, st, GS, g->eos_idx, g->pick_slot, g->Nt, b->A, diff_weight, DLDG, scal);
    TS_HIP(hipMemcpyAsync(diff_loss, scal, sizeof(float), hipMemcpyDeviceToDevice, st));
    return TRAJSDE_OK;
  };
  return encoder_backward_run("encoder_backward", b, g, rot, blob_fwd, blob_bwd, step_tab, step_tab_dev, noise, d_local, ws, ws_bytes, grads,
                              n_grads, d_latent, d_aa_out, dropout, tape_valid, scratch, scratch_bytes, stream_, bce);
}

namespace {
struct TrLayerTape { float *xn, *q, *k, *v, *o, *x1, *xn2, *out; };
struct GridBwdExtra {
  float *x0, *dxa, *dxb, *dq, *dk, *dv, *dO, *tout, *dtout, *H, *DH, *dx1;
  std::vector<TrLayerTape> tp;
  int64_t bytes;
  bool ok;
  GridBwdExtra(void* base, int64_t size, int64_t N, int nl) : tp(nl) {
    Carver ex(base, size);
    const int64_t RT = N * 22;
    x0 = ex.take<float>(RT * 64);
    for (auto& l : tp) {
      l.xn = ex.take<float>(RT * 64); l.q = ex.take<float>(RT * 64); l.k = ex.take<float>(RT * 64); l.v = ex.take<float>(RT * 64);
      l.o = ex.take<float>(RT * 64); l.x1 = ex.take<float>(RT * 64); l.xn2 = ex.take<float>(RT * 64); l.out = ex.take<float>(RT * 64);
    }
    float** slabs[] = {&dxa, &dxb, &dq, &dk, &dv, &dO, &dx1};
    for (float** p : slabs) *p = ex.take<float>(RT * 64);
    tout = ex.take<float>(N * 64);
    dtout = ex.take<float>(N * 64);
    H = ex.take<float>(RT * 256);
    DH = ex.take<float>(RT * 256);
    bytes = ex.off + 256;
    ok = ex.ok;
  }
};
}

int64_t trajsde_encoder_grid_backward_ws_bytes(const trajsde_batch* b, const trajsde_graph* g, int num_temporal_layers) {
  if (!b || !g || num_temporal_layers < 1 || num_temporal_layers > 16) return -1;
  EncBwdWs w(b, g, nullptr, 0);
  return align_up(w.total, 256) + GridBwdExtra(nullptr, 0, b->N, num_temporal_layers).bytes;
}

int trajsde_encoder_grid_backward(const trajsde_batch* b, const trajsde_graph* g, const float* rot, const float* blob_fwd,
                                  const float* blob_bwd, int num_heads, int num_temporal_layers, const float* d_local, void* ws,
                                  int64_t ws_bytes, float* const* grads, int n_grads, void* stream_) {
  return trajsde_encoder_grid_backward_train(b, g, rot, blob_fwd, blob_bwd, num_heads, num_temporal_layers, d_local, ws, ws_bytes, grads, n_grads,
                                             nullptr, stream_);
}

int trajsde_encoder_grid_backward_train(const trajsde_batch* b, const trajsde_graph* g, const float* rot, const float* blob_fwd,
                                        const float* blob_bwd, int num_heads, int num_temporal_layers, const float* d_local, void* ws,
                                        int64_t ws_bytes, float* const* grads, int n_grads, const trajsde_dropout* dropout, void* stream_) {
  if (int rc = refuse_retired_switches()) return rc;
  TS_REQUIRE(b && g && rot && blob_fwd && blob_bwd && d_local && ws && grads, "encoder_grid_backward: null pointer");
  TS_REQUIRE(!dropout || (dropout->p >= 0.f && dropout->p < 1.f), "encoder_grid_backward: dropout p must be in [0, 1)");
  const bool dropping = dropout && dropout->p > 0.f;
  auto drop_of = [&](int block) { return dropping ? make_drop(dropout->p, dropout->seed, block) : no_drop(); };
  const DropArg drop_aa = drop_of(0), drop_al = drop_of(1);
  TS_REQUIRE(g->aa_dst && g->la_dst && g->orig, "encoder_grid_backward: graph not compacted");
  TS_REQUIRE(g->exact, "encoder_grid_backward: needs exact list lengths (trajsde_graph_prepare, not _async)");
  TS_REQUIRE(b->A == 0 && g->Nt == b->N && b->H == 21, "encoder_grid_backward: graph with A = 0 and 21 history steps expected");
  TS_REQUIRE(num_heads == 8 || num_heads == 4, "encoder_grid_backward: num_heads must be 8 or 4");
  const int nl = num_temporal_layers;
  TS_REQUIRE(nl >= 1 && nl <= 16, "encoder_grid_backward: 1..16 temporal layers");
  const std::vector<std::string> names = stage_param_names(TRAJSDE_STAGE_ENCODER_GRID_BWD, nl, 0);
  TS_REQUIRE(n_grads == int(names.size()), "encoder_grid_backward: gradient count does not match trajsde_param_count(ENCODER_GRID_BWD)");
  GradTable G;
  for (int i = 0; i < n_grads; ++i) {
    TS_REQUIRE(grads[i] != nullptr, "encoder_grid_backward: null gradient buffer " + names[i]);
    G.slot[names[i]] = grads[i];
  }
  if (ws_bytes < trajsde_encoder_grid_backward_ws_bytes(b, g, nl)) return fail(TRAJSDE_ERR_WORKSPACE, "encoder_grid_backward: workspace too small");
  EncBwdWs w(b, g, ws, ws_bytes);
  GridBwdExtra ex(static_cast<char*>(ws) + align_up(w.total, 256), ws_bytes - align_up(w.total, 256), b->N, nl);
  TS_REQUIRE(w.ok && ex.ok, "encoder_grid_backward: workspace too small");
  hipStream_t st = static_cast<hipStream_t>(stream_);
  const int N = b->N, H = b->H;
  const int64_t R = int64_t(H) * N, RT = int64_t(N) * 22, Eaa = g->E_aa, Ela = g->E_la, rtiles = (RT + 15) / 16;
  std::vector<TrLayerTape>& tp = ex.tp;
  float *x0 = ex.x0, *dxa = ex.dxa, *dxb = ex.dxb, *dq = ex.dq, *dk = ex.dk, *dv = ex.dv, *dO = ex.dO, *tout = ex.tout, *dtout = ex.dtout;
  const WgradCtx wc{st, w.part, w.cs, nullptr, w.parts};
  using FB = EncBlob;
  using BB = EncBwdBlob;
  TS_LAUNCH(k_aa_center, tile_grid((R + 15) / 16, 512, AaCenterL::SIZE * 4), 512, AaCenterL::SIZE * 4, st, blob_fwd + FB::AA_CENTER, b->x,
            g->x_fake, rot, b->bos_mask, g->orig, N, N, H, w.center, w.cn, w.q);
  if (int rc = edge_attention_tape("k_edge_kv[aa]+emb", blob_fwd + FB::AA_EDGE6F, blob_fwd + FB::AA_EDGE6, blob_fwd + FB::AA_ATTN, g->aa_geom, g->aa_dst, Eaa, g->aa_segptr, w.q, R,
                                   w.emb, w.stats, w.agg, w.rec, num_heads, drop_aa, st))
    return rc;
  TS_LAUNCH(k_node_update<true>, tile_grid((R + 15) / 16, 512, UpdL6::SIZE * 4), 512, UpdL6::SIZE * 4, st, blob_fwd + FB::AA_UPD6, w.agg, w.cn,
            w.center, R, w.x1, w.xn2, drop_aa, no_merge());
  TS_LAUNCH(k_ffn6, tile_grid((R + 15) / 16, 512, FfnL6::HALF * 4), 512, FfnL6::HALF * 4, st, blob_fwd + FB::AA_FFN6, w.x1, w.xn2, R, w.aa_out, drop_aa);
  TS_LAUNCH(k_tr_prep, cdiv(RT * 64, 256), 256, 0, st, w.aa_out, b->padding_mask, blob_fwd + EncGridBlob::TOK, N, b->TT, x0);
  const float* x = x0;
  for (int l = 0; l < nl; ++l) {
    const float* lb = blob_fwd + EncGridBlob::layer(l);
    TS_LAUNCH(k_node_proj<3>, tile_grid(rtiles, 512, NodeProjL<3>::SIZE * 4), 512, NodeProjL<3>::SIZE * 4, st, lb + TrLayerL::QKV, x, RT,
              tp[l].xn, tp[l].q, tp[l].k, tp[l].v);
    const DropArg dl = drop_of(DROP_TEMPORAL_BLOCK0 + l);
    if (int rc = launch_tr_attention(num_heads, tp[l].q, tp[l].k, tp[l].v, N, tp[l].o, dl, st)) return rc;
    TS_LAUNCH(k_tr_outproj, tile_grid(rtiles, 512, TrOutL::SIZE * 4), 512, TrOutL::SIZE * 4, st, lb + TrLayerL::OUT, tp[l].o, x, RT, tp[l].x1,
              tp[l].xn2, dl);
    TS_LAUNCH(k_ffn, tile_grid(rtiles, 512, FfnL::SIZE * 4), 512, FfnL::SIZE * 4, st, lb + TrLayerL::FFN, tp[l].x1, tp[l].xn2, RT, tp[l].out, dl, 0);
    x = tp[l].out;
  }
  TS_LAUNCH(k_tr_final, tile_grid((int64_t(N) + 15) / 16, 256, 0), 256, 0, st, blob_fwd + EncGridBlob::norm(nl), x, N, tout);
  TS_LAUNCH(k_node_proj<1>, tile_grid((int64_t(N) + 15) / 16, 512, NodeProjL<1>::SIZE * 4), 512, NodeProjL<1>::SIZE * 4, st,
            blob_fwd + FB::AL_Q, tout, int64_t(N), w.al_xn, w.al_q, nullptr, nullptr);
  if (int rc = edge_attention_tape("k_edge_kv[al]+emb", blob_fwd + FB::AL_EDGE6F, blob_fwd + FB::AL_EDGE6, blob_fwd + FB::AL_ATTN, g->la_geom, g->la_dst, Ela, g->la_segptr, w.al_q,
                                   int64_t(N), w.al_emb, w.al_stats, w.al_agg, w.rec, num_heads, drop_al, st))
    return rc;
  TS_LAUNCH(k_node_update<true>, tile_grid((int64_t(N) + 15) / 16, 512, UpdL6::SIZE * 4), 512, UpdL6::SIZE * 4, st, blob_fwd + FB::AL_UPD6,
            w.al_agg, w.al_xn, tout, int64_t(N), w.al_x1, w.al_xn2, drop_al, no_merge());
  {
    AttnChain c{blob_bwd + BB::AL_NODE, blob_bwd + BB::AL_PROJ, blob_fwd + EncBlob::AL_ATTN, blob_bwd + BB::AL_EDGEEMB,
                g->la_geom, w.al_q, w.al_emb, w.al_stats, tout, g->la_dst, g->la_segptr,
                NodeBlockTape{w.al_agg, w.al_xn, w.al_x1, w.al_xn2}, int64_t(N), Ela, "al_encoder", "lane_embed", num_heads};
    c.img_kvt = blob_bwd + BB::AL_EDGEKV + EdgeKvBwdL::WKT;
    c.drop = drop_al;
    if (int rc = run_attn_chain(c, d_local, w, wc, G, dtout, st)) return rc;
  }
  const std::string te = "temporal_encoder.";
  float* dcur = dxa;
  float* dnext = dxb;
  TS_HIP(hipMemsetAsync(dcur, 0, size_t(RT) * 64 * sizeof(float), st));
  {
    const int gf = vec_grid((int64_t(N) + 15) / 16, 256, 0);
    float *ng = G(te + "transformer_encoder.norm.weight"), *nb = G(te + "transformer_encoder.norm.bias");
    TS_REQUIRE(!G.missing, "encoder_grid_backward: parameter table lacks " + G.missing_name);
    TS_LAUNCH(k_tr_final_bwd, gf, 256, 0, st, blob_bwd + EncGridBwdBlob::norm(nl), x, dtout, N, dcur, w.nb.vpart);
    {
      ColsumBatch cb(st, gf * 4, 128);
      cb.add(w.nb.vpart, 64, ng);
      cb.add(w.nb.vpart + 64, 64, nb);
      if (int rc = cb.flush()) return rc;
    }
  }
  NodeBlockScratch sc = w.nb;
  sc.H = ex.H;
  sc.DH = ex.DH;
  sc.dx1 = ex.dx1;
  for (int l = nl - 1; l >= 0; --l) {
    const std::string p = te + "transformer_encoder.layers." + std::to_string(l);
    const float* lb = blob_bwd + EncGridBwdBlob::layer(l);
    const float* x_in = l == 0 ? x0 : tp[l - 1].out;
    NodeBlockGrads gr{};
    gr.w1 = G(p + ".linear1.weight"); gr.b1 = G(p + ".linear1.bias"); gr.w2 = G(p + ".linear2.weight"); gr.b2 = G(p + ".linear2.bias");
    gr.n2g = G(p + ".norm2.weight"); gr.n2b = G(p + ".norm2.bias");
    float *wo = G(p + ".self_attn.out_proj.weight"), *bo = G(p + ".self_attn.out_proj.bias");
    float *wi = G(p + ".self_attn.in_proj_weight"), *bi = G(p + ".self_attn.in_proj_bias");
    float *n1g = G(p + ".norm1.weight"), *n1b = G(p + ".norm1.bias");
    TS_REQUIRE(!G.missing, "encoder_grid_backward: parameter table lacks " + G.missing_name);
    const DropArg dl = drop_of(DROP_TEMPORAL_BLOCK0 + l);
    if (int rc = ffn_block_backward(lb + TrLayerBwdL::FFN_A, lb + TrLayerBwdL::FFN_B, tp[l].xn2, tp[l].x1, dcur, RT, sc, wc, gr, st, dl)) return rc;
    const float* dx1m = sc.dx1;
    if (dropping) {
      TS_LAUNCH(k_drop_rows, tile_grid(rtiles, 256, 0), 256, 0, st, sc.dx1, RT, dq, dl, int(DK_PROJ));
      dx1m = dq;
    }
    TS_LAUNCH(k_lin_t_acc, tile_grid(rtiles, 256, MAT64 * 4), 256, MAT64 * 4, st, lb + TrLayerBwdL::WOUT_T, dx1m, RT, dO, 0);
    if (int rc = run_wgrad(wc, dx1m, 64, tp[l].o, 64, RT, RT, wo, 64, 0, bo, 0)) return rc;
    if (num_heads == 4) {
      if (dropping) TS_LAUNCH_TAG("k_tr_attention_bwd<drop>", false, (k_tr_attention_bwd<4, true>), cdiv(N, 4), 256, 0, st, tp[l].q, tp[l].k, tp[l].v, dO, N, dq, dk, dv, dl);
      else TS_LAUNCH_TAG("k_tr_attention_bwd", false, (k_tr_attention_bwd<4, false>), cdiv(N, 4), 256, 0, st, tp[l].q, tp[l].k, tp[l].v, dO, N, dq, dk, dv, dl);
    } else {
      if (dropping) TS_LAUNCH_TAG("k_tr_attention_bwd<drop>", false, (k_tr_attention_bwd<8, true>), cdiv(N, 4), 256, 0, st, tp[l].q, tp[l].k, tp[l].v, dO, N, dq, dk, dv, dl);
      else TS_LAUNCH_TAG("k_tr_attention_bwd", false, (k_tr_attention_bwd<8, false>), cdiv(N, 4), 256, 0, st, tp[l].q, tp[l].k, tp[l].v, dO, N, dq, dk, dv, dl);
    }
    const int gp = vec_grid(rtiles, 256, ProjBwdL<3>::SIZE * 4);
    TS_LAUNCH(k_node_proj_bwd<3>, gp, 256, ProjBwdL<3>::SIZE * 4, st, lb + TrLayerBwdL::PROJ, x_in, sc.dx1, nullptr, dq, dk, dv, RT, dnext,
              nullptr, w.nb.vpart);
    {
      ColsumBatch cb(st, gp * 4, 128);
      cb.add(w.nb.vpart, 64, n1g);
      cb.add(w.nb.vpart + 64, 64, n1b);
      if (int rc = cb.flush()) return rc;
    }
    const float* dps[3] = {dq, dk, dv};
    WgradBatch wb(wc, RT, RT);
    for (int j = 0; j < 3; ++j)
      if (int rc = wb.add(dps[j], 64, tp[l].xn, 64, wi + int64_t(j) * MAT64, 64, 0, bi + 64 * j, 0)) return rc;
    if (int rc = wb.flush()) return rc;
    float* t = dcur; dcur = dnext; dnext = t;
  }
  {
    float *gpad = G(te + "padding_token"), *gcls = G(te + "cls_token"), *gpos = G(te + "pos_embed");
    TS_REQUIRE(!G.missing, "encoder_grid_backward: parameter table lacks " + G.missing_name);
    TS_LAUNCH(k_tr_tok_grad, 22, 1024, 0, st, dcur, b->padding_mask, N, b->TT, gpad, gcls, gpos);
    TS_LAUNCH(k_tr_prep_bwd, cdiv(R * 64, 256), 256, 0, st, dcur, b->padding_mask, N, b->TT, w.DAA);
  }
  return aa_encoder_backward(b, g, rot, blob_fwd, blob_bwd, w, wc, G, num_heads, st, drop_aa);
}

}
```

trajsde_amd/csrc/kernels.hpp:

```cpp
#pragma once
#include <hip/hip_runtime.h>
#include <stdint.h>

#include "dropout.hpp"
#include "layouts.hpp"
#include "philox.hpp"

namespace tsde {

__global__ void k_aa_center(const float* img, const float* x, const float* x_fake, const float* rot, const uint8_t* bos,
                            const int32_t* orig, int N, int Nt, int H, float* center, float* cn, float* q);
template <bool X6>
__global__ void k_edge_kv(const float* img, const float* geom, const int32_t* dst, const float* q, int64_t E, float* logits, float* v,
                          int heads);
template <int THREADS>
__global__ void k_edge_kv2(const float* img, const float* geom, const int32_t* dst, const float* q, int64_t E, float* logits, float* v,
                           int heads);
constexpr int SEG_REC = 96;
constexpr int SEG_STREAMS_512 = 256 * 8 * 32;
struct AttnPlan {
  int C;
  int64_t nstreams;
  int64_t rec_slots(int64_t targets) const { return targets + nstreams + 1; }
};
struct EdgeCount {
  int64_t E;
  const int32_t* dev;
  int streams_target;
};
__device__ __forceinline__ int64_t edge_count(const EdgeCount& c) { return c.dev ? int64_t(*c.dev) : c.E; }
__device__ __forceinline__ int stream_len(const EdgeCount& c, int64_t E, int C_host) {
  if (!c.dev) return C_host;
  const int C = int((E + c.streams_target - 1) / c.streams_target);
  return C < 1 ? 1 : C;
}
struct StreamMap {
  int C, Co, Cy;
};
__host__ __device__ __forceinline__ StreamMap stream_map(int C) {
#ifdef TSDE_EQUAL_STREAMS
  return StreamMap{C, C, C};
#else
#ifndef TSDE_STREAM_SHORT_PCT
#define TSDE_STREAM_SHORT_PCT 70
#endif
  int Cy = (TSDE_STREAM_SHORT_PCT * C + 50) / 100;
  Cy = Cy < 1 ? 1 : (Cy > C ? C : Cy);
  return StreamMap{C, 2 * C - Cy, Cy};
#endif
}
__host__ __device__ __forceinline__ int64_t stream_count(int64_t E, int C) {
  const int64_t per_block = int64_t(256) * C;
  return (E + per_block - 1) / per_block * 256;
}
__device__ __forceinline__ int64_t stream_base(const StreamMap& m, int64_t s) {
  const int r = int(s & 255);
  return (s >> 8) * (int64_t(256) * m.C) + (r < 128 ? int64_t(r) * m.Co : int64_t(128) * m.Co + int64_t(r - 128) * m.Cy);
}
__device__ __forceinline__ int stream_length(const StreamMap& m, int64_t s) { return (s & 255) < 128 ? m.Co : m.Cy; }
__device__ __forceinline__ int64_t stream_of(const StreamMap& m, int64_t e) {
  const int64_t per_block = int64_t(256) * m.C, blk = e / per_block, r = e - blk * per_block, half = int64_t(128) * m.Co;
  return blk * 256 + (r < half ? r / m.Co : 128 + (r - half) / m.Cy);
}
struct SegMerge {
  const float* rec;
  const int32_t* segptr;
  EdgeCount ec;
  int C_host;
  const float* cv;
};
inline SegMerge no_merge() { return SegMerge{nullptr, nullptr, EdgeCount{0, nullptr, 0}, 0, nullptr}; }
inline AttnPlan attn_plan(int64_t E, int streams_target = SEG_STREAMS_512) {
  AttnPlan p;
  p.C = int((E + streams_target - 1) / streams_target);
  if (p.C < 1) p.C = 1;
  p.nstreams = stream_count(E, p.C);
  return p;
}
template <int NT, bool DROP, bool SAVE, int LIST, bool H8>
__global__ void k_edge_attn2(const float* img, const float* geom, const int32_t* dst, const float* q, EdgeCount ec, int C, float* rec, int heads,
                             const int32_t* segptr, DropArg drop, float* emb_out);
bool attn_fused_enabled();
int64_t fused_rec_floats(int64_t E, bool exact, int64_t targets);
int fused_edge_attention(const char* tag, bool dominant, const float* img, const float* geom, const int32_t* dst, const float* q,
                         const EdgeCount& ec, const int32_t* segptr, int64_t R, float* rec, float* agg, int heads, hipStream_t st,
                         const DropArg& drop, float* emb_out = nullptr, float* stats = nullptr, SegMerge* defer = nullptr);
bool rel_split_enabled();
int launch_global_attn_h3(const float* img, const int32_t* segptr, const int32_t* src, const float* rel, const float* q, const float* kn,
                          const float* vn, int64_t N, float* agg, hipStream_t st);
bool rel_split_scene_cache();
int launch_scene_ptr(const int64_t* scene_of, int N, int A, const int32_t* esrc, const int32_t* edst, const int32_t* segptr, int64_t E_bound,
                     int32_t* scene_ptr, hipStream_t st);
int launch_global_attn_sc(const float* img, const int32_t* segptr, const int32_t* src, const float* rel, const float* q, const float* kn,
                          const float* vn, int64_t N, int A, const int64_t* scene_of, const int32_t* scene_ptr, float* agg, hipStream_t st);
bool gattn_f32mm_enabled();
int launch_global_attn_mf(const float* img, const int32_t* segptr, const int32_t* src, const float* rel, const float* q, const float* kn,
                          const float* vn, int64_t N, float* agg, float* stats, const DropArg& drop, hipStream_t st);
#define TS_GLOBAL_ATTN(heads, bf16, drop, ...)                                                                       \
  do {                                                                                                              \
    const bool _d = (drop).p > 0.f;                                                                                 \
    if ((heads) == 4) {                                                                                             \
      if (bf16) { if (_d) TS_LAUNCH_TAG("k_global_attn<4>", false, (k_global_attn<4, true, true, true>), __VA_ARGS__, drop); else TS_LAUNCH_TAG("k_global_attn<4>", false, (k_global_attn<4, true, false, true>), __VA_ARGS__, drop); } \
      else { if (_d) TS_LAUNCH_TAG("k_global_attn<4>", false, (k_global_attn<4, false, true, true>), __VA_ARGS__, drop); else TS_LAUNCH_TAG("k_global_attn<4>", false, (k_global_attn<4, false, false, true>), __VA_ARGS__, drop); } \
    } else {                                                                                                        \
      if (bf16) { if (_d) TS_LAUNCH_TAG("k_global_attn<8>", false, (k_global_attn<8, true, true, true>), __VA_ARGS__, drop); else TS_LAUNCH_TAG("k_global_attn<8>", false, (k_global_attn<8, true, false, true>), __VA_ARGS__, drop); } \
      else { if (_d) TS_LAUNCH_TAG("k_global_attn<8>", false, (k_global_attn<8, false, true, true>), __VA_ARGS__, drop); else TS_LAUNCH_TAG("k_global_attn<8>", false, (k_global_attn<8, false, false, true>), __VA_ARGS__, drop); } \
    }                                                                                                               \
  } while (0)
#define TS_EDGE_ATTN(heads, drop, grid, block, lds, st, img, segptr, emb, q, R, agg, stats)                          \
  do {                                                                                                              \
    const bool _d = (drop).p > 0.f;                                                                                 \
    const int32_t* _ns = nullptr;                                                                                   \
    const float* _nf = nullptr;                                                                                     \
    if ((heads) == 4) {                                                                                             \
      if (_d) TS_LAUNCH_TAG("k_edge_attn_rows<4>", false, (k_global_attn<4, false, true, false>), grid, block, lds, st, img, segptr, _ns, emb, q, _nf, _nf, R, agg, stats, drop); \
      else TS_LAUNCH_TAG("k_edge_attn_rows<4>", false, (k_global_attn<4, false, false, false>), grid, block, lds, st, img, segptr, _ns, emb, q, _nf, _nf, R, agg, stats, drop); \
    } else {                                                                                                        \
      if (_d) TS_LAUNCH_TAG("k_edge_attn_rows<8>", false, (k_global_attn<8, false, true, false>), grid, block, lds, st, img, segptr, _ns, emb, q, _nf, _nf, R, agg, stats, drop); \
      else TS_LAUNCH_TAG("k_edge_attn_rows<8>", false, (k_global_attn<8, false, false, false>), grid, block, lds, st, img, segptr, _ns, emb, q, _nf, _nf, R, agg, stats, drop); \
    }                                                                                                               \
  } while (0)
__global__ void k_seg_merge(const int32_t* segptr, const float* rec, EdgeCount ec, int C, int64_t R, float* agg, float* stats, int heads,
                            const float* img, const float* q, int add_cv);
template <bool X6>
__global__ void k_edge_embed(const float* img, const float* geom, EdgeCount ec, float* emb_out, int st_bf16);
bool rel_embed_fused();
constexpr int edge_embed2_lds(int threads) { return (EdgeL6G::SIZE + (threads / 64) * ROWSTAGE) * 4; }
__global__ void k_edge_embed2(const float* img, const float* geom, EdgeCount ec, float* emb_out, int st_bf16);
template <bool X6>
__global__ void k_global_edge(const float* img, const float* rel, const int32_t* src, const int32_t* dst, const float* q,
                              const float* kn, const float* vn, int64_t E, float* logits, float* v);
template <int HEADS, bool ST_BF16, bool DROP, bool NODE>
__global__ void k_global_attn(const float* img, const int32_t* segptr, const int32_t* src, const float* rel, const float* q, const float* kn,
                              const float* vn, int64_t N, float* agg, float* stats, DropArg drop);
__global__ void k_seg_softmax_agg(const int32_t* segptr, const float* logits, const float* v, int64_t R, float* agg, int heads, DropArg drop);
template <bool X6>
__global__ void k_node_update(const float* img, const float* agg, const float* xn, const float* x, int64_t R, float* x1, float* xn2, DropArg drop,
                              SegMerge mg);
__global__ void k_ffn6(const float* img, const float* x1, const float* xn2, int64_t R, float* out, DropArg drop);
__global__ void k_ffn(const float* img, const float* x1, const float* xn2, int64_t R, float* out, DropArg drop, int out_bf16);
template <int NQ, bool SPLITKV = false>
__global__ void k_node_proj(const float* img, const float* x, int64_t R, float* xn_out, float* p0, float* p1, float* p2);
__global__ void k_mode_proj(const float* norm_g, const float* proj_g, const float* x, int64_t N, float* out);

__global__ void k_enc_sde_step(const float* img, const float* h_in, const float* hidden0, int Nt, float dt, float sq, float sn, float cs,
                               int idx, int noise_step0, NoiseArg na, const uint8_t* nus, const int32_t* eos, const int32_t* pick_slot, float* h_ode,
                               float* diff_pick);
__global__ void k_enc_gru_step(const float* img, const float* h_ode, const float* x_t, int Nt, int N, int t, int TT, int idx,
                               const uint8_t* pad, const int32_t* orig, const int32_t* eos, float* h_out, float* local_out,
                               float* latent_t);

constexpr int COOP_TMAX = 4;
constexpr int COOP_RS = 68;
constexpr int COOP_TILE = 16 * COOP_RS;
constexpr int COOP_BIAS_VECS = 21;
constexpr int coop_lds_floats(int tiles) {
  return tiles * (COOP_TILE + 5 * (TSDE_SPLIT_H3 ? 1024 : COOP_TILE)) + tiles * 64 + COOP_BIAS_VECS * 64 + 32 * 3 * 64;
}
struct StepTab {
  float dt[32], sq[32], sn[32], cs[32];
};
struct RecurTape {
  float *HIN, *H1, *H2, *G1, *G2, *GS, *HODE, *XS, *U1, *R1, *UU, *RR, *RH, *N1, *NW;
};
template <int TW, bool SAVE>
__global__ void k_enc_recur_coop(const float* sde_img, const float* gru_img, const float* coop6, const float* h0, const float* aa_out, int Nt, int N, int H,
                                 int TT, int tiles_per_wg, StepTab tab, int noise_step0, NoiseArg na, const uint8_t* nus, const uint8_t* pad,
                                 const int32_t* orig, const int32_t* eos, const int32_t* pick_slot, float* kept, float* diff_pick,
                                 float* latent_ys, int aa_bf16, RecurTape tp);
struct RecurBwdCoopArgs {
  const float *gru_t, *sde_t;
  int Nt, N, H, TT;
  NoiseArg na;
  const uint8_t *pad, *nus;
  const int32_t *orig, *eos;
  const float *dlat, *DLDG;
  RecurTape tp;
  float *DNW, *DN1P, *DUP, *DRP, *DU1, *DR1, *DAA, *DF, *DH2, *DH1, *DG2N, *DG1N, *DG2A, *DG1A, *DGPN, *DGPA, *dh_out;
  float dt[32], sq[32];
};
constexpr int COOP_BWD_TILES = 6;
constexpr int coop_bwd_lds_floats(int tiles) { return tiles * (COOP_BWD_TILES * (TSDE_SPLIT_H3 ? 1024 : COOP_TILE) + 128); }
template <int TW>
__global__ void k_enc_recur_bwd_coop(RecurBwdCoopArgs a);
constexpr int SDE_REPLAY_COOP_LDS_BYTES = (4 * 1024 + 64) * 4;
__global__ void k_sde_replay_coop(const float* img, const int32_t* best, int N, int K, int n_euler, const float* step_tab, NoiseArg na,
                                  float* states, float* H1, float* H2, float* G1, float* G2, float* GS);
constexpr int SDE_SWEEP_V_FLOATS = 68;
constexpr int SDE_BWD_COOP_LDS_BYTES = (5 * 1024 + 128) * 4;
struct SdeBwdCoopArgs {
  const float* img;
  const int32_t* best;
  int N, K, T, n_euler;
  const float *step_tab, *out_tab;
  NoiseArg na;
  const float *H1, *H2, *G1, *G2, *GS, *DS;
  float *DH1, *DH2, *DF, *DG1, *DG2, *DY0, *vpart;
};
__global__ void k_sde_bwd_coop(SdeBwdCoopArgs a);
struct MilRows { float *g2b, *h1t, *g1b, *u; };
__global__ void k_sde_replay_mil(const float* img, const float* mil_img, const int32_t* best, int N, int K, int n_euler, const float* step_tab,
                                 NoiseArg na, float* states, float* H1, float* H2, float* G1, float* G2, float* GS);
__global__ void k_sde_bwd_mil(const float* img, const float* tan_img, const int32_t* best, int N, int K, int T, int n_euler, const float* step_tab,
                              const float* out_tab, NoiseArg na, const float* H1, const float* H2, const float* G1, const float* G2,
                              const float* GS, const float* DS, float* DH1, float* DH2, float* DF, float* DG1, float* DG2, float* DY0,
                              float* vpart, MilRows mr);
__global__ void k_add_mil_wgrad(float* w2, float* w0, const float* m2, const float* m0);
struct MlpPiV { enum : int { DGAM1 = 0, DBET1 = 64, DGAM4 = 128, DBET4 = 192, DW6 = 256, DB6 = 320, SIZE = 324 }; };
template <bool SCALE>
__global__ void k_mlp_heads_bwd_cot(const float* img, const float* out, const float* loc, const float* d_loc, float min_scale, int NN, int T,
                                    float* H, float* DL, float* DU, float* DOUT, float* vpart, const float* DOUT_LOC);
__global__ void k_mlp_pi_bwd(const float* img, const float* local, const float* global, const float* d_pi, int N, int K, float* DP0,
                             float* DPS, float* H1, float* DP3, float* d_local, float* d_global, float* vpart);
__global__ void k_tr_prep(const float* aa_out, const uint8_t* pad, const float* tok, int N, int TT, float* X);
template <int HEADS, bool DROP>
__global__ void k_tr_attention(const float* q, const float* k, const float* v, int N, float* o, DropArg drop);
__global__ void k_tr_outproj(const float* img, const float* o, const float* x, int64_t R, float* x1, float* xn2, DropArg drop);
int launch_tr_attention(int heads, const float* q, const float* k, const float* v, int N, float* o, const DropArg& drop, hipStream_t st);
__global__ void k_tr_final(const float* norm, const float* x, int N, float* out);

__global__ void k_ood_stats(const float* samples, int S, int N, float* mean, float* stds);

}
```

trajsde_amd/csrc/stages.hip:

```cpp
#include "common.hpp"
#include "kernels.hpp"
#include "layouts.hpp"

#include <algorithm>
#include <cstdlib>

namespace tsde {

static bool edge_x6() { static bool v = []() { const char* e = getenv("TRAJSDE_EDGE_FP32"); return !(e && atoi(e) != 0); }(); return v; }
static bool edge_pair() { static bool v = []() { const char* e = getenv("TRAJSDE_EDGE_PAIR"); return !(e && atoi(e) == 0); }(); return v; }
static int pair_threads() { static int t = []() { const char* e = getenv("TRAJSDE_PAIR_THREADS"); const int v = e ? atoi(e) : 768; return v == 512 ? 512 : 768; }(); return t; }
static bool attn_fused() { static bool v = []() { const char* e = getenv("TRAJSDE_ATTN_FUSED"); return !(e && atoi(e) == 0); }(); return v && edge_x6() && edge_pair() && TSDE_SPLIT_H3; }
static int fused_threads() {
  static const int t = [] { const char* e = getenv("TRAJSDE_FUSED_THREADS"); const int v = e ? atoi(e) : 512; return v == 256 ? 256 : 512; }();
  return t;
}
static bool merge_in_update() { static const bool v = []() { const char* e = getenv("TRAJSDE_MERGE_KERNEL"); return !(e && atoi(e) != 0); }(); return v; }
int refuse_retired_switches() {
  struct Retired { const char* name; int value; };
  static const Retired table[] = {{"TRAJSDE_EDGE_TILE", 32}, {"TRAJSDE_EDGE_PIPE", 1}, {"TRAJSDE_FUSED_TILES", 1},
                                  {"TRAJSDE_GATTN_MM", 0},   {"TRAJSDE_GMF_TILES", 2}, {"TRAJSDE_BRANCH_FUSED", 1}};
  static const char* const asked = []() -> const char* {
    for (const Retired& r : table) {
      const char* e = getenv(r.name);
      if (e && (r.value ? atoi(e) == r.value : atoi(e) != 0)) return r.name;
    }
    return nullptr;
  }();
  if (asked) return fail(TRAJSDE_ERR_UNSUPPORTED, std::string(asked) + " selects a kernel form that was removed from the library: unset it");
  return TRAJSDE_OK;
}
static bool global_fused_env() { static const bool v = []() { const char* e = getenv("TRAJSDE_GLOBAL_UNFUSED"); return !(e && atoi(e) != 0); }(); return v; }
static int fused_streams() { return 256 * 256; }
static AttnPlan fused_plan(int64_t E) { return attn_plan(E, fused_streams()); }
static int64_t fused_rec_slots(int64_t E, bool exact, int64_t targets) {
  return exact ? fused_plan(E).rec_slots(targets) : targets + std::min<int64_t>(E, fused_streams()) + 1;
}
static EdgeCount count_of(const trajsde_graph* g, int which, int64_t E) {
  return EdgeCount{E, g->exact ? nullptr : g->counts + which, fused_streams()};
}
static int threads_edge() { static int t = env_threads("TRAJSDE_THREADS_EDGE", 1024); return t; }
static int threads_node() { static int t = env_threads("TRAJSDE_THREADS_NODE", 512); return t; }
static int threads_recur() { static int t = env_threads("TRAJSDE_THREADS_RECUR", 256); return t; }

struct EncWs {
  float *center, *cn, *q, *logits, *v, *agg, *x1, *xn2, *aa_out, *hA, *hB, *lat, *al_xn, *al_q, *al_logits, *al_v, *al_agg, *al_x1,
      *al_xn2;
  float *rec, *al_rec;
  int64_t total;
  bool ok;
  EncWs(const trajsde_batch* b, const trajsde_graph* g, void* ws, int64_t bytes) {
    Carver c(ws, bytes);
    const int64_t R = int64_t(b->H) * g->Nt, N = b->N;
    const bool fused = attn_fused();
    center = c.take<float>(R * 64); cn = c.take<float>(R * 64); q = c.take<float>(R * 64);
    rec = c.take<float>(fused ? fused_rec_slots(g->E_aa, g->exact != 0, R) * SEG_REC : 4);
    al_rec = c.take<float>(fused ? fused_rec_slots(g->E_la, g->exact != 0, N) * SEG_REC : 4);
    logits = c.take<float>(fused ? 8 : int64_t(g->E_aa) * 8 + 8); v = c.take<float>(fused ? 64 : int64_t(g->E_aa) * 64 + 64);
    agg = c.take<float>(R * 64); x1 = c.take<float>(R * 64); xn2 = c.take<float>(R * 64); aa_out = c.take<float>(R * 64);
    hA = c.take<float>(int64_t(g->Nt) * 64); hB = c.take<float>(int64_t(g->Nt) * 64); lat = c.take<float>(N * 64);
    al_xn = c.take<float>(N * 64); al_q = c.take<float>(N * 64);
    al_logits = c.take<float>(fused ? 8 : int64_t(g->E_la) * 8 + 8); al_v = c.take<float>(fused ? 64 : int64_t(g->E_la) * 64 + 64);
    al_agg = c.take<float>(N * 64); al_x1 = c.take<float>(N * 64); al_xn2 = c.take<float>(N * 64);
    total = c.off + 256;
    ok = c.ok;
  }
};

struct AggWs {
  float *rel, *xn, *q, *kn, *vn, *logits, *v, *agg, *x1, *xn2, *xa, *xb;
  int64_t total;
  bool ok;
  AggWs(const trajsde_batch* b, const trajsde_graph* g, void* ws, int64_t bytes) {
    Carver c(ws, bytes);
    const int64_t N = b->N, E = g->E_g;
    rel = c.take<float>(E * 64 + 64);
    xn = c.take<float>(N * 64); q = c.take<float>(N * 64); kn = c.take<float>(N * 64); vn = c.take<float>(N * 64);
    logits = c.take<float>(E * 8 + 8); v = c.take<float>(E * 64 + 64);
    agg = c.take<float>(N * 64); x1 = c.take<float>(N * 64); xn2 = c.take<float>(N * 64); xa = c.take<float>(N * 64); xb = c.take<float>(N * 64);
    total = c.off + 256;
    ok = c.ok;
  }
};

static bool node_x6() {
  static bool v = []() {
    const char* e = getenv("TRAJSDE_NODE_FP32");
    return e ? atoi(e) == 0 : !TSDE_SPLIT_H3;
  }();
  return v;
}

struct NodeImgs {
  const float *upd, *ffn, *upd6, *ffn6;
};
static int update_ffn(const NodeImgs& im, const float* agg, const float* xn, const float* x, int64_t R, float* x1, float* xn2, float* out,
                      hipStream_t st, const DropArg& drop = no_drop(), bool out_bf16 = false, const SegMerge& mg = no_merge()) {
  const int64_t ntiles = (R + 15) / 16;
  TS_REQUIRE(!(out_bf16 && node_x6()), "bf16 state storage needs the one-pass FFN kernel (default fp16x3 build, TRAJSDE_NODE_FP32 unset)");
  if (node_x6()) {
    TS_LAUNCH(k_node_update<true>, tile_grid(ntiles, threads_node(), UpdL6::SIZE * 4), threads_node(), UpdL6::SIZE * 4, st, im.upd6, agg, xn, x,
              R, x1, xn2, drop, mg);
    TS_LAUNCH(k_ffn6, tile_grid(ntiles, threads_node(), FfnL6::HALF * 4), threads_node(), FfnL6::HALF * 4, st, im.ffn6, x1, xn2, R, out, drop);
  } else {
    TS_LAUNCH(k_node_update<false>, tile_grid(ntiles, threads_node(), UpdL::SIZE * 4), threads_node(), UpdL::SIZE * 4, st, im.upd, agg, xn, x, R,
              x1, xn2, drop, mg);
    TS_LAUNCH(k_ffn, tile_grid(ntiles, threads_node(), FfnL::SIZE * 4), threads_node(), FfnL::SIZE * 4, st, im.ffn, x1, xn2, R, out, drop, out_bf16 ? 1 : 0);
  }
  return TRAJSDE_OK;
}
static int attention_tail(const NodeImgs& im, const int32_t* segptr, const float* logits, const float* v, const float* xn, const float* x,
                          int64_t R, float* agg, float* x1, float* xn2, float* out, hipStream_t st, int heads = 8,
                          const DropArg& drop = no_drop()) {
  TS_LAUNCH(k_seg_softmax_agg, cdiv(R, 4), 256, 0, st, segptr, logits, v, R, agg, heads, drop);
  return update_ffn(im, agg, xn, x, R, x1, xn2, out, st, drop);
}

int fused_edge_attention(const char* tag, bool dominant, const float* img, const float* geom, const int32_t* dst, const float* q,
                         const EdgeCount& ec, const int32_t* segptr, int64_t R, float* rec, float* agg, int heads, hipStream_t st,
                         const DropArg& drop, float* emb_out, float* stats, SegMerge* defer) {
  const int64_t E = ec.E;
  const AttnPlan pl = fused_plan(E);
  TS_REQUIRE(E < (int64_t(1) << 28), "fused edge attention: an edge list of 2^28 or more entries exceeds its 32-bit byte offsets; split the batch");
  if (E > 0) {
    const int threads = fused_threads();
    const int64_t streams = ec.dev ? std::min<int64_t>(E, fused_streams()) : pl.nstreams;
    const int per_wg = threads / 64 * 32;
    const int grid = xcd_grid((streams + per_wg - 1) / per_wg);
    const int lds = (EdgeL6F::LDS_SIZE + 256 * 64) * 4;
    const bool d = drop.p > 0.f, sv = emb_out != nullptr;
#define TS_EA2H(N_, D_, S_, L_, H_) TS_LAUNCH_TAG(tag, dominant, (k_edge_attn2<N_, D_, S_, L_, H_>), grid, threads, lds, st, img, geom, dst, q, ec, pl.C, rec, heads, segptr, drop, emb_out)
#define TS_EA2L(N_, D_, S_, L_) do { if (heads == 8) TS_EA2H(N_, D_, S_, L_, true); else TS_EA2H(N_, D_, S_, L_, false); } while (0)
#define TS_EA2(N_, D_, S_) do { if (dominant) TS_EA2L(N_, D_, S_, 0); else TS_EA2L(N_, D_, S_, 1); } while (0)
#if !TSDE_SPLIT_H3
    (void)grid; (void)lds; (void)threads;
    return fail(TRAJSDE_ERR_UNSUPPORTED, "the fused edge attention (and with it the training forward) exists in the fp16x3 build only");
#else
    if (d && sv) TS_EA2(2, true, true);
    else if (d) TS_EA2(2, true, false);
    else if (sv) TS_EA2(2, false, true);
    else TS_EA2(2, false, false);
#endif
#undef TS_EA2
#undef TS_EA2L
#undef TS_EA2H
  }
  if (defer != nullptr && stats == nullptr && emb_out == nullptr && drop.p == 0.f && merge_in_update()) {
    *defer = SegMerge{rec, segptr, ec, pl.C, img + EdgeL6F::CV};
    return TRAJSDE_OK;
  }
  if (defer != nullptr) *defer = no_merge();
  TS_LAUNCH(k_seg_merge, cdiv(R, 4), 256, 0, st, segptr, rec, ec, pl.C, R, agg, stats, heads, img, q, drop.p > 0.f ? 0 : 1);
  return TRAJSDE_OK;
}
bool attn_fused_enabled() { return attn_fused(); }
bool rel_embed_fused() {
  static const bool v = []() { const char* e = getenv("TRAJSDE_REL_EMBED_FUSED"); return !(e && atoi(e) == 0); }();
  return v;
}
int64_t fused_rec_floats(int64_t E, bool exact, int64_t targets) { return fused_rec_slots(E, exact, targets) * SEG_REC; }

}

using namespace tsde;

static thread_local hipStream_t t_fork_stream = nullptr;
static thread_local hipEvent_t t_fork_event = nullptr;


extern "C" {

int trajsde_sync_free_supported(void) { return attn_fused() && global_fused_env() ? 1 : 0; }

int64_t trajsde_encoder_ws_bytes(const trajsde_batch* b, const trajsde_graph* g) {
  if (!b || !g) return -1;
  EncWs w(b, g, nullptr, 0);
  return w.total;
}

static int run_aa_encoder(const trajsde_batch* b, const trajsde_graph* g, const float* rot, const float* blob, EncWs& w, float* aa_out,
                          hipStream_t st, int heads = 8, const DropArg& drop = no_drop()) {
  const int N = b->N, Nt = g->Nt, H = b->H;
  const int64_t R = int64_t(H) * Nt;
  TS_LAUNCH(k_aa_center, tile_grid((R + 15) / 16, 512, AaCenterL::SIZE * 4), 512, AaCenterL::SIZE * 4, st, blob + EncBlob::AA_CENTER,
            b->x, g->x_fake, rot, b->bos_mask, g->orig, N, Nt, H, w.center, w.cn, w.q);
  const NodeImgs im{blob + EncBlob::AA_UPD, blob + EncBlob::AA_FFN, blob + EncBlob::AA_UPD6, blob + EncBlob::AA_FFN6};
  if (attn_fused()) {
    SegMerge mg = no_merge();
    if (int rc = fused_edge_attention("k_edge_kv[aa]", true, blob + EncBlob::AA_EDGE6F, g->aa_geom, g->aa_dst, w.q, count_of(g, 1, g->E_aa), g->aa_segptr, R,
                                      w.rec, w.agg, heads, st, drop, nullptr, nullptr, &mg))
      return rc;
    return update_ffn(im, w.agg, w.cn, w.center, R, w.x1, w.xn2, aa_out, st, drop, state_bf16(), mg);
  }
  if (g->E_aa > 0) {
    if (edge_x6() && edge_pair())
    {
      if (pair_threads() == 768)
        TS_LAUNCH_TAG("k_edge_kv[aa]", true, k_edge_kv2<768>, tile_grid((int64_t(g->E_aa) + 31) / 32, 768, EdgeL6::SIZE * 4), 768, EdgeL6::SIZE * 4,
                      st, blob + EncBlob::AA_EDGE6, g->aa_geom, g->aa_dst, w.q, int64_t(g->E_aa), w.logits, w.v, heads);
      else
        TS_LAUNCH_TAG("k_edge_kv[aa]", true, k_edge_kv2<512>, tile_grid((int64_t(g->E_aa) + 31) / 32, 512, EdgeL6::SIZE * 4), 512, EdgeL6::SIZE * 4,
                      st, blob + EncBlob::AA_EDGE6, g->aa_geom, g->aa_dst, w.q, int64_t(g->E_aa), w.logits, w.v, heads);
    }
    else if (edge_x6())
      TS_LAUNCH_TAG("k_edge_kv[aa]", true, k_edge_kv<true>, tile_grid((int64_t(g->E_aa) + 15) / 16, threads_edge(), EdgeL6::SIZE * 4), threads_edge(),
                    EdgeL6::SIZE * 4, st, blob + EncBlob::AA_EDGE6, g->aa_geom, g->aa_dst, w.q, int64_t(g->E_aa), w.logits, w.v, heads);
    else
      TS_LAUNCH_TAG("k_edge_kv[aa]", true, k_edge_kv<false>, tile_grid((int64_t(g->E_aa) + 15) / 16, threads_edge(), EdgeL::SIZE * 4), threads_edge(),
                    EdgeL::SIZE * 4, st, blob + EncBlob::AA_EDGE, g->aa_geom, g->aa_dst, w.q, int64_t(g->E_aa), w.logits, w.v, heads);
  }
  TS_REQUIRE(!state_bf16(), "bf16 state storage needs the fused edge attention (default)");
  return attention_tail(im, g->aa_segptr, w.logits, w.v, w.cn, w.center, R, w.agg, w.x1, w.xn2, aa_out, st, heads, drop);
}

static int run_recurrence(const trajsde_batch* b, const trajsde_graph* g, const float* blob, const float* step_tab, const float* h0,
                          int noise_step0, NoiseArg na, EncWs& w, const float* aa_out, float* kept, float* diff_pick,
                          float* latent_ys, hipStream_t st) {
  const int N = b->N, Nt = g->Nt, H = b->H;
  const int64_t rtiles = (int64_t(Nt) + 15) / 16;
  static const bool legacy = []() { const char* e = getenv("TRAJSDE_RECUR_LEGACY"); return e && atoi(e) != 0; }();
  static const int force_tw = []() { const char* e = getenv("TRAJSDE_RECUR_TW"); return e ? atoi(e) : 0; }();
  const int tiles_per_wg = force_tw > 0 ? force_tw : int((rtiles + 255) / 256);
  TS_REQUIRE(!state_bf16() || (!legacy && tiles_per_wg <= COOP_TMAX && H <= 32),
             "bf16 state storage needs the cooperative recurrence kernel (at most 16384 extended rows)");
  if (!legacy && tiles_per_wg <= COOP_TMAX && H <= 32) {
    StepTab tab;
    for (int i = 0; i < H; ++i) {
      tab.dt[i] = step_tab[8 * i + 1]; tab.sq[i] = step_tab[8 * i + 2]; tab.sn[i] = step_tab[8 * i + 3]; tab.cs[i] = step_tab[8 * i + 4];
    }
    const int grid = int((rtiles + tiles_per_wg - 1) / tiles_per_wg);
    const int lds = coop_lds_floats(tiles_per_wg) * 4;
#define TS_COOP(TW) TS_LAUNCH_TAG("k_enc_recur_coop", false, (k_enc_recur_coop<TW, false>), grid, 256, lds, st, blob + EncBlob::SDE, blob + EncBlob::GRU, blob + EncBlob::COOP6, h0, aa_out, Nt, N, H, b->TT, tiles_per_wg, tab, \
              noise_step0, na, g->nus_mask, b->padding_mask, g->orig, g->eos_idx, g->pick_slot, kept, diff_pick, latent_ys, state_bf16() ? 1 : 0, RecurTape{})
    switch (tiles_per_wg) {
      case 1: TS_COOP(1); break;
      case 2: TS_COOP(2); break;
      case 3: TS_COOP(3); break;
      default: TS_COOP(4); break;
    }
#undef TS_COOP
    return TRAJSDE_OK;
  }
  for (int idx = 0; idx < H; ++idx) {
    const int t = H - 1 - idx;
    const float* e = step_tab + 8 * idx;
    TS_LAUNCH(k_enc_sde_step, tile_grid(rtiles, threads_recur(), EncSdeL::SIZE * 4), threads_recur(), EncSdeL::SIZE * 4, st, blob + EncBlob::SDE,
              idx == 0 ? nullptr : w.hA, h0, Nt, e[1], e[2], e[3], e[4], idx, noise_step0, na, g->nus_mask, g->eos_idx,
              g->pick_slot, w.hB, diff_pick);
    TS_LAUNCH(k_enc_gru_step, tile_grid(rtiles, threads_recur(), EncGruL::SIZE * 4), threads_recur(), EncGruL::SIZE * 4, st, blob + EncBlob::GRU, w.hB,
              aa_out + int64_t(t) * Nt * 64, Nt, N, t, b->TT, idx, b->padding_mask, g->orig, g->eos_idx, w.hA, kept,
              latent_ys ? latent_ys + int64_t(idx) * N * 64 : nullptr);
  }
  return TRAJSDE_OK;
}

static int run_al_encoder(const trajsde_batch* b, const trajsde_graph* g, const float* blob, EncWs& w, const float* lat,
                          float* local_embed, hipStream_t st, int heads = 8, const DropArg& drop = no_drop()) {
  const int N = b->N;
  TS_LAUNCH(k_node_proj<1>, tile_grid((int64_t(N) + 15) / 16, 512, NodeProjL<1>::SIZE * 4), 512, NodeProjL<1>::SIZE * 4, st,
            blob + EncBlob::AL_Q, lat, int64_t(N), w.al_xn, w.al_q, nullptr, nullptr);
  const NodeImgs im{blob + EncBlob::AL_UPD, blob + EncBlob::AL_FFN, blob + EncBlob::AL_UPD6, blob + EncBlob::AL_FFN6};
  if (attn_fused()) {
    SegMerge mg = no_merge();
    if (int rc = fused_edge_attention("k_edge_kv[al]", false, blob + EncBlob::AL_EDGE6F, g->la_geom, g->la_dst, w.al_q, count_of(g, 3, g->E_la), g->la_segptr,
                                      int64_t(N), w.al_rec, w.al_agg, heads, st, drop, nullptr, nullptr, &mg))
      return rc;
    return update_ffn(im, w.al_agg, w.al_xn, lat, N, w.al_x1, w.al_xn2, local_embed, st, drop, false, mg);
  }
  if (g->E_la > 0) {
    if (edge_x6() && edge_pair())
      TS_LAUNCH_TAG("k_edge_kv[al]", false, k_edge_kv2<512>, tile_grid((int64_t(g->E_la) + 31) / 32, 512, EdgeL6::SIZE * 4), 512, EdgeL6::SIZE * 4, st,
                    blob + EncBlob::AL_EDGE6, g->la_geom, g->la_dst, w.al_q, int64_t(g->E_la), w.al_logits, w.al_v, heads);
    else if (edge_x6())
      TS_LAUNCH_TAG("k_edge_kv[al]", false, k_edge_kv<true>, tile_grid((int64_t(g->E_la) + 15) / 16, threads_edge(), EdgeL6::SIZE * 4), threads_edge(),
                    EdgeL6::SIZE * 4, st, blob + EncBlob::AL_EDGE6, g->la_geom, g->la_dst, w.al_q, int64_t(g->E_la), w.al_logits, w.al_v, heads);
    else
      TS_LAUNCH_TAG("k_edge_kv[al]", false, k_edge_kv<false>, tile_grid((int64_t(g->E_la) + 15) / 16, threads_edge(), EdgeL::SIZE * 4), threads_edge(),
                    EdgeL::SIZE * 4, st, blob + EncBlob::AL_EDGE, g->la_geom, g->la_dst, w.al_q, int64_t(g->E_la), w.al_logits, w.al_v, heads);
  }
  return attention_tail(im, g->la_segptr, w.al_logits, w.al_v, w.al_xn, lat, N, w.al_agg, w.al_x1, w.al_xn2, local_embed, st, heads, drop);
}

int trajsde_encoder_forward(const trajsde_batch* b, const trajsde_graph* g, const float* rot, const float* blob,
                            const float* step_tab , const trajsde_noise* noise, void* ws, int64_t ws_bytes,
                            float* local_embed, float* diff_pick, float* aa_out_user, float* latent_ys, const trajsde_dropout* dropout,
                            void* stream_) {
  if (int rc = refuse_retired_switches()) return rc;
  TS_REQUIRE(b && g && rot && blob && step_tab && ws && local_embed && diff_pick, "encoder_forward: null pointer");
  TS_REQUIRE(!dropout || (dropout->p >= 0.f && dropout->p < 1.f), "encoder_forward: dropout p must be in [0, 1)");
  const DropArg drop_aa = dropout ? make_drop(dropout->p, dropout->seed, 0) : no_drop();
  const DropArg drop_al = dropout ? make_drop(dropout->p, dropout->seed, 1) : no_drop();
  TS_REQUIRE(g->aa_dst && g->la_dst && g->orig, "encoder_forward: graph not compacted (call trajsde_graph_compact)");
  TS_REQUIRE(g->exact || (attn_fused() && g->counts), "encoder_forward: a graph from trajsde_graph_prepare_async needs the fused edge attention");
  TS_REQUIRE(b->A > 0 && g->Nt == b->N + b->A, "encoder_forward: graph was prepared without the fake-agent rows");
  EncWs w(b, g, ws, ws_bytes);
  if (!w.ok) return fail(TRAJSDE_ERR_WORKSPACE, "encoder_forward: workspace too small");
  hipStream_t st = static_cast<hipStream_t>(stream_);
  float* aa_out = aa_out_user ? aa_out_user : w.aa_out;
  NoiseArg na{0, nullptr, nullptr};
  if (noise) { na.seed = noise->seed; na.z = noise->z; na.row_ids = noise->row_ids; na.seed_dev = noise->seed_dev; }
  if (int rc = run_aa_encoder(b, g, rot, blob, w, aa_out, st, 8, drop_aa)) return rc;
  TS_HIP(hipMemsetAsync(diff_pick, 0, size_t(2) * b->A * 64 * sizeof(float), st));
  if (t_fork_stream != nullptr) {
    if (t_fork_event == nullptr) TS_HIP(hipEventCreateWithFlags(&t_fork_event, hipEventDisableTiming));
    TS_HIP(hipEventRecord(t_fork_event, st));
    TS_HIP(hipStreamWaitEvent(t_fork_stream, t_fork_event, 0));
    t_fork_stream = nullptr;
  }
  if (int rc = run_recurrence(b, g, blob, step_tab, blob + EncBlob::HIDDEN, 0, na, w, aa_out, w.lat, diff_pick, latent_ys, st)) return rc;
  return run_al_encoder(b, g, blob, w, w.lat, local_embed, st, 8, drop_al);
}

int64_t trajsde_encoder_ood_ws_bytes(const trajsde_batch* b, const trajsde_graph* g, int n_samples) {
  if (!b || !g || n_samples < 1) return -1;
  EncWs w(b, g, nullptr, 0);
  return w.total + align_up(int64_t(n_samples) * b->N * 64 * 4, 256) + align_up(int64_t(b->N) * 64 * 4, 256) + 1024;
}

int trajsde_encoder_forward_ood(const trajsde_batch* b, const trajsde_graph* g, const float* rot, const float* blob,
                                const float* step_tab , const trajsde_noise* noise, int n_samples, void* ws,
                                int64_t ws_bytes, float* local_embed, float* stds, void* stream_) {
  if (int rc = refuse_retired_switches()) return rc;
  TS_REQUIRE(b && g && rot && blob && step_tab && ws && local_embed && stds, "encoder_forward_ood: null pointer");
  TS_REQUIRE(g->aa_dst && g->la_dst && g->orig, "encoder_forward_ood: graph not compacted");
  TS_REQUIRE(g->exact || (attn_fused() && g->counts), "encoder_forward_ood: a graph from trajsde_graph_prepare_async needs the fused edge attention");
  TS_REQUIRE(b->A == 0 && g->Nt == b->N, "encoder_forward_ood: prepare the graph with A = 0 (no fake agents)");
  TS_REQUIRE(n_samples >= 1, "encoder_forward_ood: n_samples < 1");
  if (ws_bytes < trajsde_encoder_ood_ws_bytes(b, g, n_samples)) return fail(TRAJSDE_ERR_WORKSPACE, "encoder_forward_ood: workspace too small");
  EncWs w(b, g, ws, ws_bytes);
  Carver extra(static_cast<char*>(ws) + align_up(w.total, 256), ws_bytes - align_up(w.total, 256));
  float* samples = extra.take<float>(int64_t(n_samples) * b->N * 64);
  float* mean = extra.take<float>(int64_t(b->N) * 64);
  float* zero = extra.take<float>(64);
  hipStream_t st = static_cast<hipStream_t>(stream_);
  NoiseArg na{0, nullptr, nullptr};
  if (noise) { na.seed = noise->seed; na.z = noise->z; na.row_ids = noise->row_ids; na.seed_dev = noise->seed_dev; }
  if (int rc = run_aa_encoder(b, g, rot, blob, w, w.aa_out, st)) return rc;
  TS_HIP(hipMemsetAsync(zero, 0, 64 * sizeof(float), st));
  for (int j = 0; j < n_samples; ++j)
    if (int rc = run_recurrence(b, g, blob, step_tab, zero, j * b->H, na, w, w.aa_out, samples + int64_t(j) * b->N * 64, nullptr,
                                nullptr, st))
      return rc;
  TS_LAUNCH(k_ood_stats, cdiv(b->N, 4), 256, 0, st, samples, n_samples, b->N, mean, stds);
  return run_al_encoder(b, g, blob, w, mean, local_embed, st);
}

int64_t trajsde_encoder_grid_ws_bytes(const trajsde_batch* b, const trajsde_graph* g) {
  if (!b || !g) return -1;
  EncWs w(b, g, nullptr, 0);
  return w.total + 9 * align_up(int64_t(b->N) * 22 * 64 * 4, 256) + align_up(int64_t(b->N) * 64 * 4, 256) + 1024;
}

int trajsde_encoder_grid_forward(const trajsde_batch* b, const trajsde_graph* g, const float* rot, const float* blob, int num_heads,
                                 int num_temporal_layers, void* ws, int64_t ws_bytes, float* local_embed, void* stream_) {
  return trajsde_encoder_grid_forward_train(b, g, rot, blob, num_heads, num_temporal_layers, ws, ws_bytes, local_embed, nullptr, stream_);
}

int trajsde_encoder_grid_forward_train(const trajsde_batch* b, const trajsde_graph* g, const float* rot, const float* blob, int num_heads,
                                       int num_temporal_layers, void* ws, int64_t ws_bytes, float* local_embed,
                                       const trajsde_dropout* dropout, void* stream_) {
  if (int rc = refuse_retired_switches()) return rc;
  TS_REQUIRE(b && g && rot && blob && ws && local_embed, "encoder_grid_forward: null pointer");
  TS_REQUIRE(!dropout || (dropout->p >= 0.f && dropout->p < 1.f), "encoder_grid_forward: dropout p must be in [0, 1)");
  const bool dropping = dropout && dropout->p > 0.f;
  auto drop_of = [&](int block) { return dropping ? make_drop(dropout->p, dropout->seed, block) : no_drop(); };
  TS_REQUIRE(g->aa_dst && g->la_dst && g->orig, "encoder_grid_forward: graph not compacted");
  TS_REQUIRE(g->exact || (attn_fused() && g->counts), "encoder_grid_forward: a graph from trajsde_graph_prepare_async needs the fused edge attention");
  TS_REQUIRE(b->A == 0 && g->Nt == b->N, "encoder_grid_forward: prepare the graph with A = 0 (no fake agents)");
  TS_REQUIRE(b->H == 21, "encoder_grid_forward: the temporal kernels are built for historical_steps = 21");
  TS_REQUIRE(num_heads == 8 || num_heads == 4, "encoder_grid_forward: num_heads must be 8 or 4");
  TS_REQUIRE(num_temporal_layers >= 1, "encoder_grid_forward: no temporal layers");
  if (ws_bytes < trajsde_encoder_grid_ws_bytes(b, g)) return fail(TRAJSDE_ERR_WORKSPACE, "encoder_grid_forward: workspace too small");
  EncWs w(b, g, ws, ws_bytes);
  Carver extra(static_cast<char*>(ws) + align_up(w.total, 256), ws_bytes - align_up(w.total, 256));
  const int N = b->N;
  const int64_t R = int64_t(N) * 22, rtiles = (R + 15) / 16;
  float *xa = extra.take<float>(R * 64), *xb = extra.take<float>(R * 64), *xn = extra.take<float>(R * 64), *q = extra.take<float>(R * 64),
        *k = extra.take<float>(R * 64), *v = extra.take<float>(R * 64), *o = extra.take<float>(R * 64), *x1 = extra.take<float>(R * 64),
        *xn2 = extra.take<float>(R * 64), *tout = extra.take<float>(int64_t(N) * 64);
  hipStream_t st = static_cast<hipStream_t>(stream_);
  if (int rc = run_aa_encoder(b, g, rot, blob, w, w.aa_out, st, num_heads, drop_of(0))) return rc;
  TS_LAUNCH(k_tr_prep, cdiv(R * 64, 256), 256, 0, st, w.aa_out, b->padding_mask, blob + EncGridBlob::TOK, N, b->TT, xa);
  float* x = xa;
  float* nx = xb;
  for (int l = 0; l < num_temporal_layers; ++l) {
    const float* lb = blob + EncGridBlob::layer(l);
    TS_LAUNCH(k_node_proj<3>, tile_grid(rtiles, 512, NodeProjL<3>::SIZE * 4), 512, NodeProjL<3>::SIZE * 4, st, lb + TrLayerL::QKV, x, R, xn, q, k,
              v);
    const DropArg dl = drop_of(DROP_TEMPORAL_BLOCK0 + l);
    if (int rc = launch_tr_attention(num_heads, q, k, v, N, o, dl, st)) return rc;
    TS_LAUNCH(k_tr_outproj, tile_grid(rtiles, 512, TrOutL::SIZE * 4), 512, TrOutL::SIZE * 4, st, lb + TrLayerL::OUT, o, x, R, x1, xn2, dl);
    TS_LAUNCH(k_ffn, tile_grid(rtiles, 512, FfnL::SIZE * 4), 512, FfnL::SIZE * 4, st, lb + TrLayerL::FFN, x1, xn2, R, nx, dl, 0);
    float* t = x; x = nx; nx = t;
  }
  TS_LAUNCH(k_tr_final, tile_grid((int64_t(N) + 15) / 16, 256, 0), 256, 0, st, blob + EncGridBlob::norm(num_temporal_layers), x, N, tout);
  return run_al_encoder(b, g, blob, w, tout, local_embed, st, num_heads, drop_of(1));
}

int64_t trajsde_aggregator_ws_bytes(const trajsde_batch* b, const trajsde_graph* g, int num_modes) {
  if (!b || !g) return -1;
  (void)num_modes;
  AggWs w(b, g, nullptr, 0);
  return w.total;
}

int trajsde_aggregator_forward(const trajsde_batch* b, const trajsde_graph* g, const float* blob, int num_layers, int num_modes,
                               const float* local_embed, void* ws, int64_t ws_bytes, float* global_embed, void* stream_) {
  return trajsde_aggregator_forward_heads(b, g, blob, num_layers, num_modes, 8, local_embed, ws, ws_bytes, global_embed, nullptr, stream_);
}

static bool rel_split_possible() {
#if TSDE_SPLIT_H3
  return rel_split_enabled() && !state_bf16() && edge_x6() && rel_embed_fused() && global_fused_env();
#else
  return false;
#endif
}
static int aggregator_rel_embed(const trajsde_batch* b, const trajsde_graph* g, const float* blob, AggWs& w, hipStream_t st, bool split) {
  const int64_t E = g->E_g, etiles = (E + 15) / 16;
  if (E > 0) {
#if TSDE_SPLIT_H3
    if (edge_x6() && rel_embed_fused())
      TS_LAUNCH_TAG("k_edge_embed<true>", false, k_edge_embed2, tile_grid((E + 31) / 32, 1024, edge_embed2_lds(1024)), 1024, edge_embed2_lds(1024), st,
                    blob + AggBlob::REL6G, g->g_geom, count_of(g, 2, E), w.rel, split ? 2 : (state_bf16() ? 1 : 0));
    else
#endif
    if (edge_x6())
      TS_LAUNCH(k_edge_embed<true>, tile_grid(etiles, threads_edge(), EdgeL6::EMB_SIZE * 4), threads_edge(), EdgeL6::EMB_SIZE * 4, st,
                blob + AggBlob::REL6, g->g_geom, count_of(g, 2, E), w.rel, state_bf16() ? 1 : 0);
    else
      TS_LAUNCH(k_edge_embed<false>, tile_grid(etiles, threads_edge(), EdgeL::EMB_SIZE * 4), threads_edge(), EdgeL::EMB_SIZE * 4, st,
                blob + AggBlob::REL, g->g_geom, count_of(g, 2, E), w.rel, state_bf16() ? 1 : 0);
  }
  return TRAJSDE_OK;
}

int trajsde_encoder_fork_stream(void* side_stream) {
  t_fork_stream = static_cast<hipStream_t>(side_stream);
  return TRAJSDE_OK;
}

int trajsde_aggregator_prepare(const trajsde_batch* b, const trajsde_graph* g, const float* blob, void* ws, int64_t ws_bytes, void* stream_) {
  if (int rc = refuse_retired_switches()) return rc;
  TS_REQUIRE(b && g && blob && ws, "aggregator_prepare: null pointer");
  TS_REQUIRE(g->g_src && g->g_segptr, "aggregator_prepare: graph not compacted (call trajsde_graph_compact)");
  AggWs w(b, g, ws, ws_bytes);
  if (!w.ok) return fail(TRAJSDE_ERR_WORKSPACE, "aggregator_prepare: workspace too small");
  return aggregator_rel_embed(b, g, blob, w, static_cast<hipStream_t>(stream_), rel_split_possible());
}

static int aggregator_forward_impl(const trajsde_batch* b, const trajsde_graph* g, const float* blob, int num_layers, int num_modes,
                                   int num_heads, const float* local_embed, void* ws, int64_t ws_bytes, float* global_embed,
                                   const trajsde_dropout* dropout, void* stream_, bool rel_ready);

int trajsde_aggregator_forward_heads(const trajsde_batch* b, const trajsde_graph* g, const float* blob, int num_layers, int num_modes,
                                     int num_heads, const float* local_embed, void* ws, int64_t ws_bytes, float* global_embed,
                                     const trajsde_dropout* dropout, void* stream_) {
  return aggregator_forward_impl(b, g, blob, num_layers, num_modes, num_heads, local_embed, ws, ws_bytes, global_embed, dropout, stream_, false);
}

int trajsde_aggregator_forward_prepared(const trajsde_batch* b, const trajsde_graph* g, const float* blob, int num_layers, int num_modes,
                                        int num_heads, const float* local_embed, void* ws, int64_t ws_bytes, float* global_embed,
                                        const trajsde_dropout* dropout, void* stream_) {
  return aggregator_forward_impl(b, g, blob, num_layers, num_modes, num_heads, local_embed, ws, ws_bytes, global_embed, dropout, stream_, true);
}

static int aggregator_forward_impl(const trajsde_batch* b, const trajsde_graph* g, const float* blob, int num_layers, int num_modes,
                                   int num_heads, const float* local_embed, void* ws, int64_t ws_bytes, float* global_embed,
                                   const trajsde_dropout* dropout, void* stream_, bool rel_ready) {
  if (int rc = refuse_retired_switches()) return rc;
  TS_REQUIRE(b && g && blob && local_embed && ws && global_embed, "aggregator_forward: null pointer");
  TS_REQUIRE(!dropout || (dropout->p >= 0.f && dropout->p < 1.f), "aggregator_forward: dropout p must be in [0, 1)");
  TS_REQUIRE(num_heads == 8 || num_heads == 4, "aggregator_forward: num_heads must be 8 or 4");
  TS_REQUIRE(g->g_src && g->g_segptr, "aggregator_forward: graph not compacted (call trajsde_graph_compact)");
  TS_REQUIRE(num_layers >= 0 && num_modes > 0, "aggregator_forward: bad layer/mode count");
  AggWs w(b, g, ws, ws_bytes);
  if (!w.ok) return fail(TRAJSDE_ERR_WORKSPACE, "aggregator_forward: workspace too small");
  hipStream_t st = static_cast<hipStream_t>(stream_);
  const int64_t N = b->N, E = g->E_g, ntiles = (N + 15) / 16, etiles = (E + 15) / 16;
  const bool split = rel_split_possible() && num_heads == 8 && (!dropout || dropout->p == 0.f) && E > 0;
  if (!rel_ready || split != rel_split_possible())
    if (int rc = aggregator_rel_embed(b, g, blob, w, st, split)) return rc;
  const float* x = local_embed;
  float* bufs[2] = {w.xa, w.xb};
  for (int i = 0; i < num_layers; ++i) {
    const float* lb = blob + AggBlob::layer(i);
    if (split)
      TS_LAUNCH((k_node_proj<3, true>), tile_grid(ntiles, 512, NodeProjL<3>::SIZE * 4), 512, NodeProjL<3>::SIZE * 4, st, lb + AggLayerL::QKV, x, N,
                w.xn, w.q, w.kn, w.vn);
    else
      TS_LAUNCH(k_node_proj<3>, tile_grid(ntiles, 512, NodeProjL<3>::SIZE * 4), 512, NodeProjL<3>::SIZE * 4, st, lb + AggLayerL::QKV, x, N,
                w.xn, w.q, w.kn, w.vn);
    float* out = bufs[i & 1];
    const NodeImgs im{lb + AggLayerL::UPD, lb + AggLayerL::FFN, lb + AggLayerL::UPD6, lb + AggLayerL::FFN6};
    const bool fused = global_fused_env() || num_heads != 8;
    const DropArg drop = dropout ? make_drop(dropout->p, dropout->seed, 2 + i) : no_drop();
    TS_REQUIRE(fused || drop.p == 0.f, "aggregator_forward: dropout needs the fused global attention (unset TRAJSDE_GLOBAL_UNFUSED)");
    TS_REQUIRE(fused || !state_bf16(), "aggregator_forward: bf16 state storage needs the fused global attention");
    TS_REQUIRE(fused || g->exact, "aggregator_forward: a graph from trajsde_graph_prepare_async needs the fused global attention");
    if (fused) {
      TS_REQUIRE(N < (1 << 23), "aggregator_forward: node rows are addressed with 32-bit byte offsets (N < 2^23)");
      if (split && rel_split_scene_cache() && b->batch != nullptr && b->A > 0 && b->A + 2 <= E * 8 + 8) {
        int32_t* scene_ptr = reinterpret_cast<int32_t*>(w.logits);
        if (i == 0)
          if (int rc = launch_scene_ptr(b->batch, b->N, b->A, g->g_src, g->g_dst, g->g_segptr, E, scene_ptr, st)) return rc;
        if (int rc = launch_global_attn_sc(lb + AggLayerL::ATTN, g->g_segptr, g->g_src, w.rel, w.q, w.kn, w.vn, N, b->A, b->batch, scene_ptr, w.agg, st))
          return rc;
      } else if (split) {
        if (int rc = launch_global_attn_h3(lb + AggLayerL::ATTN, g->g_segptr, g->g_src, w.rel, w.q, w.kn, w.vn, N, w.agg, st)) return rc;
      } else if (num_heads == 8 && !state_bf16() && gattn_f32mm_enabled() && E > 0) {
        if (int rc = launch_global_attn_mf(lb + AggLayerL::ATTN, g->g_segptr, g->g_src, w.rel, w.q, w.kn, w.vn, N, w.agg, nullptr, drop, st)) return rc;
      } else {
        TS_GLOBAL_ATTN(num_heads, state_bf16(), drop, xcd_grid(cdiv(N, 4)), 256, 0, st, lb + AggLayerL::ATTN, g->g_segptr, g->g_src, w.rel, w.q, w.kn, w.vn, N, w.agg, static_cast<float*>(nullptr));
      }
      if (int rc = update_ffn(im, w.agg, w.xn, x, N, w.x1, w.xn2, out, st, drop)) return rc;
      x = out;
      continue;
    }
    if (E > 0) {
      if (edge_x6())
        TS_LAUNCH(k_global_edge<true>, tile_grid(etiles, 512, GEdgeL6::SIZE * 4), 512, GEdgeL6::SIZE * 4, st,
                  lb + AggLayerL::EDGE6, w.rel, g->g_src, g->g_dst, w.q, w.kn, w.vn, E, w.logits, w.v);
      else
        TS_LAUNCH(k_global_edge<false>, tile_grid(etiles, 512, GEdgeL::SIZE * 4), 512, GEdgeL::SIZE * 4, st,
                  lb + AggLayerL::EDGE, w.rel, g->g_src, g->g_dst, w.q, w.kn, w.vn, E, w.logits, w.v);
    }
    if (int rc = attention_tail(im, g->g_segptr, w.logits, w.v, w.xn, x, N, w.agg, w.x1, w.xn2, out, st)) return rc;
    x = out;
  }
  const int lds = (128 + MAT64 + 64) * 4;
  dim3 grid(tile_grid(ntiles, 512, lds), num_modes);
  TS_LAUNCH(k_mode_proj, grid, 512, lds, st, blob + AggBlob::norm(num_layers), blob + AggBlob::proj(num_layers, 0), x, N, global_embed);
  return TRAJSDE_OK;
}

}
```

Baseline: 16690.

## Recompute layer norms in node update and FFN instead of storing normed twins

In the fused paths, the node projection and centre kernels no longer write the LayerNorm'd copies (xn/cn, xn2). The downstream node-update and FFN kernels recompute those norms from the residual rows, using gamma/beta parked in extra LDS or read directly from global memory. This cuts a global write and read of a 64-wide row per node per layer, at the cost of redundant LayerNorm arithmetic. It also adds a software prefetch of the next tile's x1 row in k_ffn and an env-capped grid helper.

```diff
diff --git a/trajsde_amd/csrc/aggregator_bwd.hip b/trajsde_amd/csrc/aggregator_bwd.hip
--- a/trajsde_amd/csrc/aggregator_bwd.hip
+++ b/trajsde_amd/csrc/aggregator_bwd.hip
@@ -952,7 +952,7 @@
       } else
         TS_GLOBAL_ATTN(num_heads, false, dl, xcd_grid(cdiv(N, 4)), 256, 0, st, lb + AggLayerL::ATTN, g->g_segptr, g->g_src, w.rel, w.q[l], w.kn[l], w.vn[l], N, w.agg[l], w.stats[l]);
     }
-    TS_LAUNCH(k_node_update<true>, tile_grid(ntiles, 512, UpdL6::SIZE * 4), 512, UpdL6::SIZE * 4, st, lb + AggLayerL::UPD6, w.agg[l], w.xn[l], x,
+    TS_LAUNCH(k_node_update<true>, tile_grid(ntiles, 512, node_update_lds(true)), 512, node_update_lds(true), st, lb + AggLayerL::UPD6, w.agg[l], w.xn[l], x,
               N, w.x1[l], w.xn2[l], drop_of(l), no_merge());
     TS_LAUNCH(k_ffn6, tile_grid(ntiles, 512, FfnL6::HALF * 4), 512, FfnL6::HALF * 4, st, lb + AggLayerL::FFN6, w.x1[l], w.xn2[l], N, w.out[l],
               drop_of(l));
diff --git a/trajsde_amd/csrc/attn.hip b/trajsde_amd/csrc/attn.hip
--- a/trajsde_amd/csrc/attn.hip
+++ b/trajsde_amd/csrc/attn.hip
@@ -46,7 +46,7 @@
     if (bos[int64_t(o) * H + t]) load_vec<4>(a, lds + A::BOS + t * 64, L.g);
     if (row < rows) store_row(a, center, row, L.g);
     layer_norm<4>(a, lds + A::N1G, lds + A::N1B, L.g);
-    if (row < rows) store_row(a, cn, row, L.g);
+    if (cn != nullptr && row < rows) store_row(a, cn, row, L.g);
     linear<4, 4>(b, a, lds + A::WQ, lds + A::BQ, L);
     if (row < rows) store_row(b, q, row, L.g);
   }
@@ -956,13 +956,25 @@
 template __global__ void k_global_attn<4, false, true, false>(const float*, const int32_t*, const int32_t*, const float*, const float*, const float*,
                                                        const float*, int64_t, float*, float*, DropArg);
 
+__device__ __forceinline__ void rows_are_requested() { asm volatile("" ::: "memory"); }
+__device__ __forceinline__ void rows_have_arrived(f4 (&a)[4]) { asm volatile("" : "+v"(a[0]), "+v"(a[1]), "+v"(a[2]), "+v"(a[3])); }
+
 template <bool X6>
 __global__ __launch_bounds__(512) void k_node_update(const float* __restrict__ img_g, const float* __restrict__ agg,
                                                      const float* __restrict__ xn, const float* __restrict__ x, int64_t R,
-                                                     float* __restrict__ x1, float* __restrict__ xn2, DropArg drop, SegMerge mg) {
+                                                     float* __restrict__ x1, float* __restrict__ xn2, DropArg drop, SegMerge mg,
+                                                     const float* __restrict__ n1g, const float* __restrict__ n1b) {
   extern __shared__ __attribute__((aligned(16))) float lds[];
   using U = typename std::conditional<X6, UpdL6, UpdL>::type;
-  stage_blob(lds, img_g, U::SIZE);
+  const bool merge = mg.rec != nullptr;
+  float* const vec = lds + U::SIZE;
+  {
+    const bool norm = xn == nullptr && threadIdx.x < 64;
+    const float vg = norm ? n1g[threadIdx.x] : 0.f, vb = norm ? n1b[threadIdx.x] : 0.f;
+    stage_copy(lds, img_g, U::SIZE);
+    if (norm) vec[threadIdx.x] = vg, vec[64 + threadIdx.x] = vb;
+    __syncthreads();
+  }
   const Lane L_;
   auto lin = [&](f4 (&out)[4], const f4 (&in)[4], int wo, int bo) {
     if constexpr (X6) linear_x6<4, 4>(out, in, lds + wo, lds + bo, L_);
@@ -975,7 +987,7 @@
     keep_lds_reads_here();
     const int64_t row = tile * 16 + L.n, r = row < R ? row : R - 1;
     f4 a[4], n[4], g[4], s[4];
-    if (mg.rec != nullptr) {
+    if (merge) {
       const int C = stream_len(mg.ec, edge_count(mg.ec), mg.C_host);
       const int beg = mg.segptr[r], end = mg.segptr[r + 1];
 #pragma unroll
@@ -1010,9 +1022,15 @@
     } else {
       load_row(a, agg, r, L.g);
     }
-    load_row(n, xn, r, L.g);
     f4 xr[4];
     load_row(xr, x, r, L.g);
+    if (xn != nullptr) {
+      load_row(n, xn, r, L.g);
+    } else {
+#pragma unroll
+      for (int jt = 0; jt < 4; ++jt) n[jt] = xr[jt];
+      layer_norm<4>(n, vec, vec + 64, L.g);
+    }
     range_note(absmax<4>(a), RS_NODE_AGG);
     lin(g, a, U::WIH, U::BIH);
     {
@@ -1038,24 +1056,48 @@
 #pragma unroll
     for (int jt = 0; jt < 4; ++jt) n[jt] = xr[jt] + s[jt];
     if (row < R) store_row(n, x1, row, L.g);
-    layer_norm<4>(n, lds + U::N2G, lds + U::N2B, L.g);
-    if (row < R) store_row(n, xn2, row, L.g);
+    if (xn2 != nullptr) {
+      layer_norm<4>(n, lds + U::N2G, lds + U::N2B, L.g);
+      if (row < R) store_row(n, xn2, row, L.g);
+    }
   }
 }
 
 __global__ __launch_bounds__(512) void k_ffn(const float* __restrict__ img_g, const float* __restrict__ x1,
-                                             const float* __restrict__ xn2, int64_t R, float* __restrict__ out, DropArg drop, int out_bf16) {
+                                             const float* __restrict__ xn2, int64_t R, float* __restrict__ out, DropArg drop, int out_bf16,
+                                             const float* __restrict__ n2g, const float* __restrict__ n2b) {
   extern __shared__ __attribute__((aligned(16))) float lds[];
-  stage_blob(lds, img_g, FfnL::SIZE);
+  float* const vec = lds + FfnL::SIZE;
+  {
+    const bool norm = xn2 == nullptr && threadIdx.x < 64;
+    const float vg = norm ? n2g[threadIdx.x] : 0.f, vb = norm ? n2b[threadIdx.x] : 0.f;
+    stage_copy(lds, img_g, FfnL::SIZE);
+    if (norm) vec[threadIdx.x] = vg, vec[64 + threadIdx.x] = vb;
+    __syncthreads();
+  }
   const Lane L;
   const int waves = blockDim.x >> 6, wave = threadIdx.x >> 6;
-  const int64_t ntiles = (R + 15) / 16;
-  for (int64_t tile = int64_t(blockIdx.x) * waves + wave; tile < ntiles; tile += int64_t(gridDim.x) * waves) {
+  const int64_t ntiles = (R + 15) / 16, stride = int64_t(gridDim.x) * waves;
+  int64_t tile = int64_t(blockIdx.x) * waves + wave;
+  if (tile >= ntiles) return;
+  auto request_row = [&](int64_t t, f4 (&px)[4]) __attribute__((always_inline)) {
+    const int64_t row = t * 16 + L.n;
+    load_row(px, x1, row < R ? row : R - 1, L.g);
+  };
+  f4 cx[4];
+  request_row(tile, cx);
+  for (; tile < ntiles; tile += stride) {
     keep_lds_reads_here();
     const int64_t row = tile * 16 + L.n, r = row < R ? row : R - 1;
-    f4 n[4], hid[16], o[4], xr[4];
-    load_row(n, xn2, r, L.g);
-    load_row(xr, x1, r, L.g);
+    f4 n[4], hid[16], o[4], nx[4];
+    if (xn2 != nullptr) load_row(n, xn2, r, L.g);
+    request_row(tile + stride < ntiles ? tile + stride : tile, nx);
+    rows_are_requested();
+    if (xn2 == nullptr) {
+#pragma unroll
+      for (int jt = 0; jt < 4; ++jt) n[jt] = cx[jt];
+      layer_norm<4>(n, vec, vec + 64, L.g);
+    }
     linear<16, 4>(hid, n, lds + FfnL::W1, lds + FfnL::B1, L);
     relu<16>(hid);
     if (drop.p > 0.f) {
@@ -1076,13 +1118,17 @@
       for (int jt = 0; jt < 4; ++jt) o[jt] *= mk[jt];
     }
 #pragma unroll
-    for (int jt = 0; jt < 4; ++jt) o[jt] += xr[jt];
+    for (int jt = 0; jt < 4; ++jt) o[jt] += cx[jt];
+    rows_have_arrived(nx);
     if (row < R) store_row_st(o, out, row, L.g, out_bf16 != 0);
+#pragma unroll
+    for (int jt = 0; jt < 4; ++jt) cx[jt] = nx[jt];
   }
 }
 
 __global__ __launch_bounds__(512) void k_ffn6(const float* __restrict__ img_g, const float* __restrict__ x1,
-                                              const float* __restrict__ xn2, int64_t R, float* __restrict__ out, DropArg drop) {
+                                              const float* __restrict__ xn2, int64_t R, float* __restrict__ out, DropArg drop,
+                                              const float* __restrict__ n2g, const float* __restrict__ n2b) {
   extern __shared__ __attribute__((aligned(16))) float lds[];
   const Lane L;
   const int waves = blockDim.x >> 6, wave = threadIdx.x >> 6;
@@ -1094,7 +1140,12 @@
       keep_lds_reads_here();
       const int64_t row = tile * 16 + L.n, r = row < R ? row : R - 1;
       f4 n[4], hid[8], o[4];
-      load_row(n, xn2, r, L.g);
+      if (xn2 != nullptr) {
+        load_row(n, xn2, r, L.g);
+      } else {
+        load_row(n, x1, r, L.g);
+        layer_norm<4>(n, n2g, n2b, L.g);
+      }
       linear_x6<8, 4>(hid, n, lds + FfnL6::W1, lds + FfnL6::B1, L);
       relu<8>(hid);
       f4 mo[4];
@@ -1145,7 +1196,7 @@
     f4 a[4], pr[4 * NQ];
     load_row(a, x, r, L.g);
     layer_norm<4>(a, lds + P::N1G, lds + P::N1B, L.g);
-    if (row < R) store_row(a, xn_out, row, L.g);
+    if (xn_out != nullptr && row < R) store_row(a, xn_out, row, L.g);
     linear<4 * NQ, 4>(pr, a, lds + P::W, lds + P::B, L);
     float* outs[3] = {p0, p1, p2};
 #pragma unroll
@@ -1198,8 +1249,10 @@
 template __global__ void k_edge_embed<true>(const float*, const float*, EdgeCount, float*, int);
 template __global__ void k_global_edge<false>(const float*, const float*, const int32_t*, const int32_t*, const float*, const float*, const float*, int64_t, float*, float*);
 template __global__ void k_global_edge<true>(const float*, const float*, const int32_t*, const int32_t*, const float*, const float*, const float*, int64_t, float*, float*);
-template __global__ void k_node_update<false>(const float*, const float*, const float*, const float*, int64_t, float*, float*, DropArg, SegMerge);
-template __global__ void k_node_update<true>(const float*, const float*, const float*, const float*, int64_t, float*, float*, DropArg, SegMerge);
+template __global__ void k_node_update<false>(const float*, const float*, const float*, const float*, int64_t, float*, float*, DropArg, SegMerge,
+                                              const float*, const float*);
+template __global__ void k_node_update<true>(const float*, const float*, const float*, const float*, int64_t, float*, float*, DropArg, SegMerge,
+                                             const float*, const float*);
 template __global__ void k_node_proj<1, false>(const float*, const float*, int64_t, float*, float*, float*, float*);
 template __global__ void k_node_proj<3, false>(const float*, const float*, int64_t, float*, float*, float*, float*);
 template __global__ void k_node_proj<3, true>(const float*, const float*, int64_t, float*, float*, float*, float*);
diff --git a/trajsde_amd/csrc/encoder_bwd.hip b/trajsde_amd/csrc/encoder_bwd.hip
--- a/trajsde_amd/csrc/encoder_bwd.hip
+++ b/trajsde_amd/csrc/encoder_bwd.hip
@@ -768,7 +768,7 @@
   if (int rc = edge_attention_tape("k_edge_kv[aa]+emb", blob_fwd + FB::AA_EDGE6F, blob_fwd + FB::AA_EDGE6, blob_fwd + FB::AA_ATTN, g->aa_geom, g->aa_dst, Eaa, g->aa_segptr, w.q, R,
                                    w.emb, w.stats, w.agg, w.rec, 8, drop_aa, st))
     return rc;
-  TS_LAUNCH(k_node_update<true>, tile_grid((R + 15) / 16, 512, UpdL6::SIZE * 4), 512, UpdL6::SIZE * 4, st, blob_fwd + FB::AA_UPD6, w.agg, w.cn,
+  TS_LAUNCH(k_node_update<true>, tile_grid((R + 15) / 16, 512, node_update_lds(true)), 512, node_update_lds(true), st, blob_fwd + FB::AA_UPD6, w.agg, w.cn,
             w.center, R, w.x1, w.xn2, drop_aa, no_merge());
   TS_LAUNCH(k_ffn6, tile_grid((R + 15) / 16, 512, FfnL6::HALF * 4), 512, FfnL6::HALF * 4, st, blob_fwd + FB::AA_FFN6, w.x1, w.xn2, R, w.aa_out, drop_aa);
   {
@@ -812,7 +812,7 @@
   if (int rc = edge_attention_tape("k_edge_kv[al]+emb", blob_fwd + FB::AL_EDGE6F, blob_fwd + FB::AL_EDGE6, blob_fwd + FB::AL_ATTN, g->la_geom, g->la_dst, Ela, g->la_segptr, w.al_q,
                                    int64_t(N), w.al_emb, w.al_stats, w.al_agg, w.rec, 8, drop_al, st))
     return rc;
-  TS_LAUNCH(k_node_update<true>, tile_grid((int64_t(N) + 15) / 16, 512, UpdL6::SIZE * 4), 512, UpdL6::SIZE * 4, st, blob_fwd + FB::AL_UPD6,
+  TS_LAUNCH(k_node_update<true>, tile_grid((int64_t(N) + 15) / 16, 512, node_update_lds(true)), 512, node_update_lds(true), st, blob_fwd + FB::AL_UPD6,
             w.al_agg, w.al_xn, w.lat, int64_t(N), w.al_x1, w.al_xn2, drop_al, no_merge());
 
   return TRAJSDE_OK;
@@ -1102,7 +1102,7 @@
   if (int rc = edge_attention_tape("k_edge_kv[aa]+emb", blob_fwd + FB::AA_EDGE6F, blob_fwd + FB::AA_EDGE6, blob_fwd + FB::AA_ATTN, g->aa_geom, g->aa_dst, Eaa, g->aa_segptr, w.q, R,
                                    w.emb, w.stats, w.agg, w.rec, num_heads, drop_aa, st))
     return rc;
-  TS_LAUNCH(k_node_update<true>, tile_grid((R + 15) / 16, 512, UpdL6::SIZE * 4), 512, UpdL6::SIZE * 4, st, blob_fwd + FB::AA_UPD6, w.agg, w.cn,
+  TS_LAUNCH(k_node_update<true>, tile_grid((R + 15) / 16, 512, node_update_lds(true)), 512, node_update_lds(true), st, blob_fwd + FB::AA_UPD6, w.agg, w.cn,
             w.center, R, w.x1, w.xn2, drop_aa, no_merge());
   TS_LAUNCH(k_ffn6, tile_grid((R + 15) / 16, 512, FfnL6::HALF * 4), 512, FfnL6::HALF * 4, st, blob_fwd + FB::AA_FFN6, w.x1, w.xn2, R, w.aa_out, drop_aa);
   TS_LAUNCH(k_tr_prep, cdiv(RT * 64, 256), 256, 0, st, w.aa_out, b->padding_mask, blob_fwd + EncGridBlob::TOK, N, b->TT, x0);
@@ -1115,7 +1115,7 @@
     if (int rc = launch_tr_attention(num_heads, tp[l].q, tp[l].k, tp[l].v, N, tp[l].o, dl, st)) return rc;
     TS_LAUNCH(k_tr_outproj, tile_grid(rtiles, 512, TrOutL::SIZE * 4), 512, TrOutL::SIZE * 4, st, lb + TrLayerL::OUT, tp[l].o, x, RT, tp[l].x1,
               tp[l].xn2, dl);
-    TS_LAUNCH(k_ffn, tile_grid(rtiles, 512, FfnL::SIZE * 4), 512, FfnL::SIZE * 4, st, lb + TrLayerL::FFN, tp[l].x1, tp[l].xn2, RT, tp[l].out, dl, 0);
+    TS_LAUNCH(k_ffn, tile_grid(rtiles, 512, ffn_lds()), 512, ffn_lds(), st, lb + TrLayerL::FFN, tp[l].x1, tp[l].xn2, RT, tp[l].out, dl, 0);
     x = tp[l].out;
   }
   TS_LAUNCH(k_tr_final, tile_grid((int64_t(N) + 15) / 16, 256, 0), 256, 0, st, blob_fwd + EncGridBlob::norm(nl), x, N, tout);
@@ -1124,7 +1124,7 @@
   if (int rc = edge_attention_tape("k_edge_kv[al]+emb", blob_fwd + FB::AL_EDGE6F, blob_fwd + FB::AL_EDGE6, blob_fwd + FB::AL_ATTN, g->la_geom, g->la_dst, Ela, g->la_segptr, w.al_q,
                                    int64_t(N), w.al_emb, w.al_stats, w.al_agg, w.rec, num_heads, drop_al, st))
     return rc;
-  TS_LAUNCH(k_node_update<true>, tile_grid((int64_t(N) + 15) / 16, 512, UpdL6::SIZE * 4), 512, UpdL6::SIZE * 4, st, blob_fwd + FB::AL_UPD6,
+  TS_LAUNCH(k_node_update<true>, tile_grid((int64_t(N) + 15) / 16, 512, node_update_lds(true)), 512, node_update_lds(true), st, blob_fwd + FB::AL_UPD6,
             w.al_agg, w.al_xn, tout, int64_t(N), w.al_x1, w.al_xn2, drop_al, no_merge());
   {
     AttnChain c{blob_bwd + BB::AL_NODE, blob_bwd + BB::AL_PROJ, blob_fwd + EncBlob::AL_ATTN, blob_bwd + BB::AL_EDGEEMB,
diff --git a/trajsde_amd/csrc/kernels.hpp b/trajsde_amd/csrc/kernels.hpp
--- a/trajsde_amd/csrc/kernels.hpp
+++ b/trajsde_amd/csrc/kernels.hpp
@@ -134,11 +134,18 @@
 __global__ void k_global_attn(const float* img, const int32_t* segptr, const int32_t* src, const float* rel, const float* q, const float* kn,
                               const float* vn, int64_t N, float* agg, float* stats, DropArg drop);
 __global__ void k_seg_softmax_agg(const int32_t* segptr, const float* logits, const float* v, int64_t R, float* agg, int heads, DropArg drop);
+constexpr int NODE_VEC_BYTES = 128 * 4;
+constexpr int node_update_lds(bool x6) { return (x6 ? UpdL6::SIZE : UpdL::SIZE) * 4 + NODE_VEC_BYTES; }
+constexpr int ffn_lds() { return FfnL::SIZE * 4 + NODE_VEC_BYTES; }
+static_assert(node_update_lds(true) <= 160 * 1024 && node_update_lds(false) <= 160 * 1024 && ffn_lds() <= 160 * 1024,
+              "node images + their parked vectors must fit LDS");
 template <bool X6>
 __global__ void k_node_update(const float* img, const float* agg, const float* xn, const float* x, int64_t R, float* x1, float* xn2, DropArg drop,
-                              SegMerge mg);
-__global__ void k_ffn6(const float* img, const float* x1, const float* xn2, int64_t R, float* out, DropArg drop);
-__global__ void k_ffn(const float* img, const float* x1, const float* xn2, int64_t R, float* out, DropArg drop, int out_bf16);
+                              SegMerge mg, const float* n1g = nullptr, const float* n1b = nullptr);
+__global__ void k_ffn6(const float* img, const float* x1, const float* xn2, int64_t R, float* out, DropArg drop, const float* n2g = nullptr,
+                       const float* n2b = nullptr);
+__global__ void k_ffn(const float* img, const float* x1, const float* xn2, int64_t R, float* out, DropArg drop, int out_bf16,
+                      const float* n2g = nullptr, const float* n2b = nullptr);
 template <int NQ, bool SPLITKV = false>
 __global__ void k_node_proj(const float* img, const float* x, int64_t R, float* xn_out, float* p0, float* p1, float* p2);
 __global__ void k_mode_proj(const float* norm_g, const float* proj_g, const float* x, int64_t N, float* out);
diff --git a/trajsde_amd/csrc/stages.hip b/trajsde_amd/csrc/stages.hip
--- a/trajsde_amd/csrc/stages.hip
+++ b/trajsde_amd/csrc/stages.hip
@@ -91,21 +91,34 @@
   return v;
 }
 
+static bool node_twins() { static const bool v = []() { const char* e = getenv("TRAJSDE_NODE_TWINS"); return e && atoi(e) != 0; }(); return v; }
+static int node_grid(int64_t ntiles, int threads, int lds_bytes) {
+  static const int cap = []() { const char* e = getenv("TRAJSDE_NODE_GRID_CAP"); return e ? atoi(e) : 0; }();
+  const int g = tile_grid(ntiles, threads, lds_bytes);
+  return cap > 0 && g > cap ? cap : g;
+}
+
 struct NodeImgs {
   const float *upd, *ffn, *upd6, *ffn6;
 };
 static int update_ffn(const NodeImgs& im, const float* agg, const float* xn, const float* x, int64_t R, float* x1, float* xn2, float* out,
-                      hipStream_t st, const DropArg& drop = no_drop(), bool out_bf16 = false, const SegMerge& mg = no_merge()) {
+                      hipStream_t st, const DropArg& drop = no_drop(), bool out_bf16 = false, const SegMerge& mg = no_merge(),
+                      const float* n1 = nullptr) {
   const int64_t ntiles = (R + 15) / 16;
   TS_REQUIRE(!(out_bf16 && node_x6()), "bf16 state storage needs the one-pass FFN kernel (default fp16x3 build, TRAJSDE_NODE_FP32 unset)");
+  TS_REQUIRE(xn != nullptr || n1 != nullptr, "update_ffn: neither the norm1 rows nor their affine");
+  const float* n1b = n1 ? n1 + 64 : nullptr;
+  const int tn = threads_node();
   if (node_x6()) {
-    TS_LAUNCH(k_node_update<true>, tile_grid(ntiles, threads_node(), UpdL6::SIZE * 4), threads_node(), UpdL6::SIZE * 4, st, im.upd6, agg, xn, x,
-              R, x1, xn2, drop, mg);
-    TS_LAUNCH(k_ffn6, tile_grid(ntiles, threads_node(), FfnL6::HALF * 4), threads_node(), FfnL6::HALF * 4, st, im.ffn6, x1, xn2, R, out, drop);
+    const int lu = node_update_lds(true);
+    TS_LAUNCH(k_node_update<true>, node_grid(ntiles, tn, lu), tn, lu, st, im.upd6, agg, xn, x, R, x1, xn2, drop, mg, n1, n1b);
+    TS_LAUNCH(k_ffn6, node_grid(ntiles, tn, FfnL6::HALF * 4), tn, FfnL6::HALF * 4, st, im.ffn6, x1, xn2, R, out, drop,
+              im.upd6 + UpdL6::N2G, im.upd6 + UpdL6::N2B);
   } else {
-    TS_LAUNCH(k_node_update<false>, tile_grid(ntiles, threads_node(), UpdL::SIZE * 4), threads_node(), UpdL::SIZE * 4, st, im.upd, agg, xn, x, R,
-              x1, xn2, drop, mg);
-    TS_LAUNCH(k_ffn, tile_grid(ntiles, threads_node(), FfnL::SIZE * 4), threads_node(), FfnL::SIZE * 4, st, im.ffn, x1, xn2, R, out, drop, out_bf16 ? 1 : 0);
+    const int lu = node_update_lds(false), lf = ffn_lds();
+    TS_LAUNCH(k_node_update<false>, node_grid(ntiles, tn, lu), tn, lu, st, im.upd, agg, xn, x, R, x1, xn2, drop, mg, n1, n1b);
+    TS_LAUNCH(k_ffn, node_grid(ntiles, tn, lf), tn, lf, st, im.ffn, x1, xn2, R, out, drop, out_bf16 ? 1 : 0, im.upd + UpdL::N2G,
+              im.upd + UpdL::N2B);
   }
   return TRAJSDE_OK;
 }
@@ -182,15 +195,18 @@
                           hipStream_t st, int heads = 8, const DropArg& drop = no_drop()) {
   const int N = b->N, Nt = g->Nt, H = b->H;
   const int64_t R = int64_t(H) * Nt;
-  TS_LAUNCH(k_aa_center, tile_grid((R + 15) / 16, 512, AaCenterL::SIZE * 4), 512, AaCenterL::SIZE * 4, st, blob + EncBlob::AA_CENTER,
-            b->x, g->x_fake, rot, b->bos_mask, g->orig, N, Nt, H, w.center, w.cn, w.q);
+  const bool twins = node_twins() || !attn_fused();
+  float *cn = twins ? w.cn : nullptr, *xn2 = twins ? w.xn2 : nullptr;
+  TS_LAUNCH(k_aa_center, node_grid((R + 15) / 16, 512, AaCenterL::SIZE * 4), 512, AaCenterL::SIZE * 4, st, blob + EncBlob::AA_CENTER,
+            b->x, g->x_fake, rot, b->bos_mask, g->orig, N, Nt, H, w.center, cn, w.q);
   const NodeImgs im{blob + EncBlob::AA_UPD, blob + EncBlob::AA_FFN, blob + EncBlob::AA_UPD6, blob + EncBlob::AA_FFN6};
   if (attn_fused()) {
     SegMerge mg = no_merge();
     if (int rc = fused_edge_attention("k_edge_kv[aa]", true, blob + EncBlob::AA_EDGE6F, g->aa_geom, g->aa_dst, w.q, count_of(g, 1, g->E_aa), g->aa_segptr, R,
                                       w.rec, w.agg, heads, st, drop, nullptr, nullptr, &mg))
       return rc;
-    return update_ffn(im, w.agg, w.cn, w.center, R, w.x1, w.xn2, aa_out, st, drop, state_bf16(), mg);
+    return update_ffn(im, w.agg, cn, w.center, R, w.x1, xn2, aa_out, st, drop, state_bf16(), mg,
+                      blob + EncBlob::AA_CENTER + AaCenterL::N1G);
   }
   if (g->E_aa > 0) {
     if (edge_x6() && edge_pair())
@@ -257,15 +273,17 @@
 static int run_al_encoder(const trajsde_batch* b, const trajsde_graph* g, const float* blob, EncWs& w, const float* lat,
                           float* local_embed, hipStream_t st, int heads = 8, const DropArg& drop = no_drop()) {
   const int N = b->N;
-  TS_LAUNCH(k_node_proj<1>, tile_grid((int64_t(N) + 15) / 16, 512, NodeProjL<1>::SIZE * 4), 512, NodeProjL<1>::SIZE * 4, st,
-            blob + EncBlob::AL_Q, lat, int64_t(N), w.al_xn, w.al_q, nullptr, nullptr);
+  const bool twins = node_twins() || !attn_fused();
+  float *xn = twins ? w.al_xn : nullptr, *xn2 = twins ? w.al_xn2 : nullptr;
+  TS_LAUNCH(k_node_proj<1>, node_grid((int64_t(N) + 15) / 16, 512, NodeProjL<1>::SIZE * 4), 512, NodeProjL<1>::SIZE * 4, st,
+            blob + EncBlob::AL_Q, lat, int64_t(N), xn, w.al_q, nullptr, nullptr);
   const NodeImgs im{blob + EncBlob::AL_UPD, blob + EncBlob::AL_FFN, blob + EncBlob::AL_UPD6, blob + EncBlob::AL_FFN6};
   if (attn_fused()) {
     SegMerge mg = no_merge();
     if (int rc = fused_edge_attention("k_edge_kv[al]", false, blob + EncBlob::AL_EDGE6F, g->la_geom, g->la_dst, w.al_q, count_of(g, 3, g->E_la), g->la_segptr,
                                       int64_t(N), w.al_rec, w.al_agg, heads, st, drop, nullptr, nullptr, &mg))
       return rc;
-    return update_ffn(im, w.al_agg, w.al_xn, lat, N, w.al_x1, w.al_xn2, local_embed, st, drop, false, mg);
+    return update_ffn(im, w.al_agg, xn, lat, N, w.al_x1, xn2, local_embed, st, drop, false, mg, blob + EncBlob::AL_Q + NodeProjL<1>::N1G);
   }
   if (g->E_la > 0) {
     if (edge_x6() && edge_pair())
@@ -390,7 +408,7 @@
     const DropArg dl = drop_of(DROP_TEMPORAL_BLOCK0 + l);
     if (int rc = launch_tr_attention(num_heads, q, k, v, N, o, dl, st)) return rc;
     TS_LAUNCH(k_tr_outproj, tile_grid(rtiles, 512, TrOutL::SIZE * 4), 512, TrOutL::SIZE * 4, st, lb + TrLayerL::OUT, o, x, R, x1, xn2, dl);
-    TS_LAUNCH(k_ffn, tile_grid(rtiles, 512, FfnL::SIZE * 4), 512, FfnL::SIZE * 4, st, lb + TrLayerL::FFN, x1, xn2, R, nx, dl, 0);
+    TS_LAUNCH(k_ffn, tile_grid(rtiles, 512, ffn_lds()), 512, ffn_lds(), st, lb + TrLayerL::FFN, x1, xn2, R, nx, dl, 0);
     float* t = x; x = nx; nx = t;
   }
   TS_LAUNCH(k_tr_final, tile_grid((int64_t(N) + 15) / 16, 256, 0), 256, 0, st, blob + EncGridBlob::norm(num_temporal_layers), x, N, tout);
@@ -485,15 +503,17 @@
   float* bufs[2] = {w.xa, w.xb};
   for (int i = 0; i < num_layers; ++i) {
     const float* lb = blob + AggBlob::layer(i);
+    const bool fused = global_fused_env() || num_heads != 8;
+    const bool twins = node_twins() || !fused;
+    float *xn = twins ? w.xn : nullptr, *xn2 = twins ? w.xn2 : nullptr;
     if (split)
-      TS_LAUNCH((k_node_proj<3, true>), tile_grid(ntiles, 512, NodeProjL<3>::SIZE * 4), 512, NodeProjL<3>::SIZE * 4, st, lb + AggLayerL::QKV, x, N,
-                w.xn, w.q, w.kn, w.vn);
+      TS_LAUNCH((k_node_proj<3, true>), node_grid(ntiles, 512, NodeProjL<3>::SIZE * 4), 512, NodeProjL<3>::SIZE * 4, st, lb + AggLayerL::QKV, x, N,
+                xn, w.q, w.kn, w.vn);
     else
-      TS_LAUNCH(k_node_proj<3>, tile_grid(ntiles, 512, NodeProjL<3>::SIZE * 4), 512, NodeProjL<3>::SIZE * 4, st, lb + AggLayerL::QKV, x, N,
-                w.xn, w.q, w.kn, w.vn);
+      TS_LAUNCH(k_node_proj<3>, node_grid(ntiles, 512, NodeProjL<3>::SIZE * 4), 512, NodeProjL<3>::SIZE * 4, st, lb + AggLayerL::QKV, x, N,
+                xn, w.q, w.kn, w.vn);
     float* out = bufs[i & 1];
     const NodeImgs im{lb + AggLayerL::UPD, lb + AggLayerL::FFN, lb + AggLayerL::UPD6, lb + AggLayerL::FFN6};
-    const bool fused = global_fused_env() || num_heads != 8;
     const DropArg drop = dropout ? make_drop(dropout->p, dropout->seed, 2 + i) : no_drop();
     TS_REQUIRE(fused || drop.p == 0.f, "aggregator_forward: dropout needs the fused global attention (unset TRAJSDE_GLOBAL_UNFUSED)");
     TS_REQUIRE(fused || !state_bf16(), "aggregator_forward: bf16 state storage needs the fused global attention");
@@ -513,7 +533,7 @@
       } else {
         TS_GLOBAL_ATTN(num_heads, state_bf16(), drop, xcd_grid(cdiv(N, 4)), 256, 0, st, lb + AggLayerL::ATTN, g->g_segptr, g->g_src, w.rel, w.q, w.kn, w.vn, N, w.agg, static_cast<float*>(nullptr));
       }
-      if (int rc = update_ffn(im, w.agg, w.xn, x, N, w.x1, w.xn2, out, st, drop)) return rc;
+      if (int rc = update_ffn(im, w.agg, xn, x, N, w.x1, xn2, out, st, drop, false, no_merge(), lb + AggLayerL::QKV + NodeProjL<3>::N1G)) return rc;
       x = out;
       continue;
     }
```

After: 16800 (median of 6 runs). About the same (+0.7%).
